# bdina9/qat-vit

Hardware: AMD Instinct MI355X
Metric: images/sec QAT student step (fwd+bwd+allreduce) (higher is better)
Workload: dtype f32 (emulated: int8 MFMA for grid x grid products; forward float operands as fp16 hi+lo pairs; backward gradients as ONE fp16 plane scaled per tensor - 2^-12 per element, <= 4e-4 relative L2 per stage against the fp32 reference, bf16-pair fallback on overflow; fp32 / exact-integer accumulate)

## Files before the change

### include/qatvit.h

```cpp
#ifndef QATVIT_H
#define QATVIT_H

#include <stdint.h>

#ifdef __cplusplus
extern "C" {
#endif
#if defined(__GNUC__) || defined(__clang__)
#pragma GCC visibility push(default)
#endif

#define QATVIT_ABI_VERSION 4

int qatvit_abi_version(void);
const char* qatvit_last_error(void);
const char* qatvit_target_arch(void);

int64_t qatvit_fq_workspace_bytes(int64_t channels);
int qatvit_fq_forward(const float* x, float* y, uint8_t* mask_bits,
                      float* running_min, float* running_max, float* scale, int32_t* zero_point,
                      const int64_t* observer_on, const int64_t* fake_quant_on,
                      float averaging_const, int32_t qmin, int32_t qmax,
                      int64_t channels, int64_t inner, int32_t per_channel, int32_t symmetric,
                      void* workspace, void* stream);

int qatvit_fq_backward(const float* dy, const uint8_t* mask_bits, float* dx, int64_t n, void* stream);

int qatvit_ln_forward(const float* x, const float* gamma, const float* beta, float* y,
                      float* mean, float* rstd, int64_t rows, int64_t dim, float eps, void* stream);
int qatvit_ln_backward(const float* dy, const float* x, const float* gamma, const float* mean,
                       const float* rstd, float* dx, float* dgamma, float* dbeta,
                       int64_t rows, int64_t dim, void* stream);

int qatvit_kd_ce_loss(const float* student, const float* teacher, const int64_t* labels,
                      int64_t batch, int64_t classes, float kd_temp, float kd_alpha,
                      float label_smoothing, float* out3, float* dlogits, void* stream);

int qatvit_kd_ce_loss_table(const float* student, const float* table, int64_t table_rows,
                            const int64_t* index, const int64_t* labels, int64_t batch,
                            int64_t classes, float kd_temp, float kd_alpha, float label_smoothing,
                            float* out3, float* dlogits, void* stream);


int qatvit_gemm_nt(const void* A_hi, const void* A_lo, const void* B, float* C, int32_t M, int32_t N, int32_t K,
                   int32_t lda, int32_t ldb, int32_t ldc, const float* s1, const float* s2, const float* col_scale,
                   const float* bias, uint32_t* stats, void* stream);

int qatvit_gemm_nt_f16(const void* A16_hi, const void* A16_lo, const void* B16, float* C, int32_t M, int32_t N, int32_t K, int32_t lda, int32_t ldb,
                       int32_t ldc, const float* s1, const float* s2, const float* col_scale, const float* bias, uint32_t* stats, void* stream);

int qatvit_gemm_nt_i8_minmax(const void* A8, const void* B8, const int32_t* wsum, const float* a_qp, int32_t center, int32_t M, int32_t N, int32_t K,
                             int32_t lda, int32_t ldb, const float* s1, const float* s2, const float* col_scale, const float* bias, uint32_t* stats,
                             void* stream);

int qatvit_w8_fragment_order(const void* B8, void* B8f, int32_t N, int32_t K, void* stream);

int qatvit_i8_strip(int32_t mode, const void* A8, const void* B8f, const int32_t* wsum, const float* a_qp, int32_t center, int32_t M, int32_t N, int32_t K,
                    int32_t lda, const float* s1, const float* s2, const float* col_scale, const float* bias, uint32_t* stats, const float* out_qp,
                    int32_t qmin, int32_t qmax, void* out8, void* out8_mask, int32_t code_T, uint32_t* lut_out, uint32_t* lutq_out,
                    float* out16_scale, void* stream);

int qatvit_gemm_nt_codes(const void* A8, const uint32_t* lut, const void* B16, float* C, int32_t M, int32_t N, int32_t K, int32_t lda, int32_t ldb,
                         int32_t ldc, const float* s1, const float* s2, const float* col_scale, const float* bias, uint32_t* stats, void* stream);

int qatvit_gemm_nt_i8(const void* A8, const void* B8, const int32_t* wsum, const float* a_qp, int32_t center, float* C, int32_t M,
                      int32_t N, int32_t K, int32_t lda, int32_t ldb, int32_t ldc, const float* s1, const float* s2,
                      const float* col_scale, const float* bias, uint32_t* stats, void* stream);

int64_t qatvit_gemm_tn_scratch_bytes(void);
int qatvit_gemm_tn_codes(const void* P_hi, const void* P_lo, const void* Qc, const uint32_t* lutQ, float* C, int32_t M, int32_t N, int32_t Kw, int32_t ldp,
                         int32_t ldq, int32_t ldc, const float* s1, const float* W, const float* w_scale, const int32_t* w_zp, int32_t w_per_channel,
                         int32_t w_qmin, int32_t w_qmax, float* dbias, const float* row_div, float* scratch, int64_t scratch_bytes, void* stream);
int qatvit_gemm_tn(const void* P_hi, const void* P_lo, const void* Q_hi, const void* Q_lo, float* C, int32_t M, int32_t N,
                   int32_t Kw, int32_t ldp, int32_t ldq, int32_t ldc, const float* s1, const float* W, const float* w_scale,
                   const int32_t* w_zp, int32_t w_per_channel, int32_t w_qmin, int32_t w_qmax, float* dbias,
                   const float* row_div, float* scratch, int64_t scratch_bytes, void* stream);

int qatvit_gemm_nt_dy16(const void* A16, const void* B16, float* C, int32_t M, int32_t N, int32_t K, int32_t lda, int32_t ldb, int32_t ldc, const float* s1,
                        const float* s2, void* stream);
int qatvit_gemm_tn_dy16(const void* P16, const void* Q_hi, const void* Q_lo, const void* Qc, const uint32_t* lutQ16, float* C, int32_t M, int32_t N, int32_t Kw,
                        int32_t ldp, int32_t ldq, int32_t ldc, const float* s1, const float* s2, const float* W, const float* w_scale, const int32_t* w_zp,
                        int32_t w_per_channel, int32_t w_qmin, int32_t w_qmax, float* dbias, const float* row_div, float* scratch, int64_t scratch_bytes,
                        void* stream);
int qatvit_gemm_tn_q8_dy16(const void* P16, const void* Q8, const float* a_qp, int32_t center, float* C, int32_t M, int32_t N, int32_t Kw, int32_t ldp, int32_t ldq,
                           int32_t ldc, const float* s2, const float* W, const float* w_scale, const int32_t* w_zp, int32_t w_per_channel, int32_t w_qmin,
                           int32_t w_qmax, float* dbias, const float* row_div, float* scratch, int64_t scratch_bytes, void* stream);

struct qatvit_tn_item {
    const void* P; const void* Q; const uint32_t* lut; const float* s1; const float* s2; float* C; const float* W; const float* w_scale; const int32_t* w_zp; float* dbias;
    const float* row_div; int32_t N, Kw, ldp, ldq, ldc;
};
int64_t qatvit_gemm_tn_stream_scratch_bytes(void);
int qatvit_gemm_tn_stream_dy16(int32_t mode, const struct qatvit_tn_item* items, int32_t n, int32_t M, int32_t center, int32_t w_per_channel, int32_t w_qmin, int32_t w_qmax,
                               float* scratch, int64_t scratch_bytes, void* stream);

int32_t qatvit_attn_padded_tokens(int32_t T);
int qatvit_attn_forward(const float* qkv, const float* qp, int32_t qmin, int32_t qmax, int32_t B, int32_t T, int32_t H,
                        int32_t D, void* O_hi, void* O_lo, float* lse, void* stream);
int qatvit_attn_forward_f16(const float* qkv, const float* qp, int32_t qmin, int32_t qmax, int32_t B, int32_t T, int32_t H,
                            int32_t D, void* O_hi, void* O_lo, float* lse, void* O16_hi, void* O16_lo, float* o16_scale, void* qkv_codes,
                            void* qkv_mask, void* stream);
int qatvit_attn_backward(const float* qkv, const float* qp, int32_t qmin, int32_t qmax, int32_t B, int32_t T, int32_t H,
                         int32_t D, const void* O_hi, const void* O_lo, const float* lse, float* delta, const float* dO,
                         void* dqkv_hi, void* dqkv_lo, const float* col_scale, const void* qkv_codes, const void* qkv_mask, void* stream);

typedef struct qatvit_cfg {
    int32_t batch, img_size, patch_size, in_chans;
    int32_t embed_dim, depth, num_heads, mlp_hidden, num_classes;
    int32_t act_qmin, act_qmax;
    int32_t w_qmin, w_qmax;
    int32_t w_per_channel;
    float averaging_const;
    float ln_eps;
} qatvit_cfg;

typedef struct qatvit_fq {
    float* min_val;
    float* max_val;
    float* scale;
    int32_t* zero_point;
    const int64_t* observer_on;
    const int64_t* fake_quant_on;
} qatvit_fq;

int32_t qatvit_student_num_params(const qatvit_cfg* cfg);
int32_t qatvit_student_num_act_fq(const qatvit_cfg* cfg);
int32_t qatvit_student_num_weight_fq(const qatvit_cfg* cfg);
int64_t qatvit_student_workspace_bytes(const qatvit_cfg* cfg);
int qatvit_student_init(const qatvit_cfg* cfg, void* workspace, void* stream);
int qatvit_student_forward(const qatvit_cfg* cfg, void* const* params, const qatvit_fq* act_fq, const qatvit_fq* weight_fq,
                           const float* images, float* logits, void* workspace, void* stream);
int qatvit_student_backward(const qatvit_cfg* cfg, void* const* params, const qatvit_fq* act_fq, const qatvit_fq* weight_fq,
                            const float* dlogits, void* const* grads, void* workspace, int32_t stage_from, int32_t stage_to,
                            void* stream);
#define QATVIT_STAGE_INJECT 1
#define QATVIT_FWD_X16 2
#define QATVIT_BWD_DY16 2
#define QATVIT_BWD_CALIBRATE 4
int32_t qatvit_student_dy16_supported(const qatvit_cfg* cfg);
int qatvit_student_dy16_set_mirror(const qatvit_cfg* cfg, void* workspace, void* host_pinned, void* stream);
int qatvit_student_dy16_to_pair(const qatvit_cfg* cfg, void* workspace, void* stream);
int qatvit_student_forward_stages(const qatvit_cfg* cfg, void* const* params, const qatvit_fq* act_fq, const qatvit_fq* weight_fq,
                                  const float* images, float* logits, void* workspace, int32_t stage_from, int32_t stage_to, int32_t flags,
                                  void* stream);
int qatvit_student_forward_part(const qatvit_cfg* cfg, void* const* params, const qatvit_fq* act_fq, const qatvit_fq* weight_fq, void* workspace,
                                int32_t block, int32_t part, int32_t flags, void* stream);
int qatvit_student_backward_stages(const qatvit_cfg* cfg, void* const* params, const qatvit_fq* act_fq, const qatvit_fq* weight_fq,
                                   const float* dlogits, void* const* grads, void* workspace, int32_t stage_from, int32_t stage_to, int32_t flags,
                                   void* stream);
int64_t qatvit_teacher_workspace_bytes(const qatvit_cfg* cfg);
int qatvit_teacher_forward(const qatvit_cfg* cfg, void* const* params, void* const* w_hi, void* const* w_lo,
                           const float* images, float* logits, void* workspace, void* stream);
int qatvit_teacher_forward_f16(const qatvit_cfg* cfg, void* const* params, void* const* w16, int32_t passes,
                               const float* images, float* logits, void* workspace, void* stream);

int64_t qatvit_float_student_workspace_bytes(const qatvit_cfg* cfg);
int qatvit_float_student_init(const qatvit_cfg* cfg, void* workspace, void* stream);
int qatvit_float_student_forward(const qatvit_cfg* cfg, void* const* params, const float* images, float* logits, void* workspace, void* stream);
int qatvit_float_student_backward(const qatvit_cfg* cfg, void* const* params, const float* dlogits, void* const* grads, void* workspace,
                                  void* stream);
int64_t qatvit_float_student_observe_bytes(const qatvit_cfg* cfg);
int qatvit_float_student_observe_init(const qatvit_cfg* cfg, const qatvit_fq* act_fq, const qatvit_fq* weight_fq, void* observe, void* stream);
int qatvit_float_student_forward_observe(const qatvit_cfg* cfg, void* const* params, const float* images, float* logits, void* workspace, void* observe,
                                         void* stream);
int64_t qatvit_float_student_amp_workspace_bytes(const qatvit_cfg* cfg);
int qatvit_float_student_amp_init(const qatvit_cfg* cfg, void* workspace, void* stream);
int qatvit_float_student_amp_forward(const qatvit_cfg* cfg, void* const* params, const float* images, void* logits_f16, void* workspace, void* stream);
int qatvit_float_student_amp_backward(const qatvit_cfg* cfg, void* const* params, const void* dlogits_f16, void* const* grads, void* workspace,
                                      void* stream);
int qatvit_float_student_amp_attn_backward(const float* qkv, const void* O16, const float* lse, const float* dO, int32_t B, int32_t T, int32_t H,
                                           int32_t D, void* dqkv16, void* stream);
int64_t qatvit_float_student_bf16_workspace_bytes(const qatvit_cfg* cfg);
int qatvit_float_student_bf16_init(const qatvit_cfg* cfg, void* workspace, void* stream);
int qatvit_float_student_bf16_forward(const qatvit_cfg* cfg, void* const* params, const float* images, void* logits_bf16, void* workspace, void* stream);
int qatvit_float_student_bf16_backward(const qatvit_cfg* cfg, void* const* params, const void* dlogits_bf16, void* const* grads, void* workspace,
                                       void* stream);
int qatvit_float_student_bf16_attn_backward(const float* qkv, const void* O16, const float* lse, const float* dO, int32_t B, int32_t T, int32_t H,
                                            int32_t D, void* dqkv16, void* stream);

int64_t qatvit_infer_workspace_bytes(const qatvit_cfg* cfg);
int qatvit_infer_prepare(const qatvit_cfg* cfg, const void* const* w8, const float* act_scale, const int32_t* act_zero_point, void* workspace,
                         void* stream);
int qatvit_infer_forward(const qatvit_cfg* cfg, void* const* params, const void* const* w8, const float* const* w_scale, const float* images,
                         float* logits, void* workspace, void* stream);

int qatvit_optim_grad_norm(const void* grad_ptrs, const int64_t* numel, const int32_t* chunk_tensor, const int32_t* chunk_index,
                           int32_t n_chunks, int64_t chunk_elems, float max_norm, float* partials, float* out2, void* stream);
int qatvit_optim_adamw(const void* param_ptrs, const void* grad_ptrs, const void* exp_avg_ptrs, const void* exp_avg_sq_ptrs,
                       const int64_t* numel, const int32_t* chunk_tensor, const int32_t* chunk_index, int32_t n_chunks,
                       int64_t chunk_elems, double lr, double beta1, double beta2, double eps, double weight_decay, int64_t step,
                       const float* clip_out2, void* stream);

int qatvit_image_resize_coeffs(int32_t src, int32_t dst, int32_t* xmin_host, int32_t* ntaps_host, int32_t* coef_host);
int qatvit_image_table(const float* mean_host, const float* std_host, float* table_host);
int qatvit_image_batch(const uint8_t* data, const int64_t* index, int32_t B, int32_t N, int32_t S, int32_t D, const int32_t* coeffs,
                       const float* table, float* out, void* stream);

int qatvit_profile_start(const void* workspace, int32_t kind, int32_t max_launches);
int qatvit_profile_stop(const void* workspace, double* total_ms, int64_t* launches, double* flops);
int64_t qatvit_student_tensor_offset(const qatvit_cfg* cfg, const char* name, int32_t block);

#if defined(__GNUC__) || defined(__clang__)
#pragma GCC visibility pop
#endif
#ifdef __cplusplus
}
#endif
#endif
```

### qat-vit_amd/csrc/capi.hip

```cpp
#include <stdarg.h>
#include <stdlib.h>
#include <string.h>

#include "../../include/qatvit.h"
#include "qv_common.h"
#include "qv_kernels.h"

namespace qv {
static thread_local char g_err[512] = "";
void set_error(const char* fmt, ...) {
    va_list ap;
    va_start(ap, fmt);
    vsnprintf(g_err, sizeof(g_err), fmt, ap);
    va_end(ap);
}

static bool knob(const char* name) {
    const char* v = getenv(name);
    return !v || atoi(v) != 0;
}
const Knobs& knobs() {
    static const Knobs k{knob("QATVIT_I8"), knob("QATVIT_F16"), knob("QATVIT_FC2_CODES"), knob("QATVIT_FC1_BITS"), knob("QATVIT_FC2W_CODES"),
                         knob("QATVIT_WBATCH"), knob("QATVIT_ATTN_CODES"), knob("QATVIT_QKV_2PASS"), knob("QATVIT_LNB_FUSE"), knob("QATVIT_QP_LATE"),
                         knob("QATVIT_TN_STREAM"), knob("QATVIT_TN_Q8"), knob("QATVIT_ATTN_BWD_FUSED"), knob("QATVIT_F16_STRIP"), knob("QATVIT_I8_STRIP")};
    return k;
}
}

using namespace qv;

extern "C" {

int qatvit_abi_version(void) { return QATVIT_ABI_VERSION; }
const char* qatvit_last_error(void) { return qv::g_err; }
const char* qatvit_target_arch(void) { return "gfx950"; }

int64_t qatvit_fq_workspace_bytes(int64_t channels) {
    if (channels < 1) channels = 1;
    return channels * (2 * (int64_t)sizeof(uint32_t) + 4 * (int64_t)sizeof(float));
}

int qatvit_fq_forward(const float* x, float* y, uint8_t* mask_bits, float* running_min, float* running_max, float* scale,
                      int32_t* zero_point, const int64_t* observer_on, const int64_t* fake_quant_on, float averaging_const,
                      int32_t qmin, int32_t qmax, int64_t channels, int64_t inner, int32_t per_channel, int32_t symmetric,
                      void* workspace, void* stream) {
    QV_CHECK_ARG(x && y && running_min && running_max && scale && zero_point && observer_on && fake_quant_on && workspace,
                 "qatvit_fq_forward: null pointer argument");
    QV_CHECK_ARG(channels >= 1 && inner >= 1, "qatvit_fq_forward: empty tensor (channels=%lld inner=%lld)", (long long)channels,
                 (long long)inner);
    QV_CHECK_ARG(qmin < qmax, "qatvit_fq_forward: qmin (%d) must be < qmax (%d)", qmin, qmax);
    QV_CHECK_ARG(per_channel || channels == 1, "qatvit_fq_forward: per-tensor call must pass channels == 1");
    launch_fq_forward(x, y, mask_bits, running_min, running_max, scale, zero_point, observer_on, fake_quant_on, averaging_const, qmin,
                      qmax, channels, inner, per_channel != 0, symmetric != 0, workspace, (hipStream_t)stream);
    QV_CHECK_LAUNCH("qatvit_fq_forward");
    return 0;
}

int qatvit_fq_backward(const float* dy, const uint8_t* mask_bits, float* dx, int64_t n, void* stream) {
    QV_CHECK_ARG(dy && mask_bits && dx, "qatvit_fq_backward: null pointer argument");
    QV_CHECK_ARG(n >= 1, "qatvit_fq_backward: empty tensor");
    launch_fq_backward(dy, mask_bits, dx, n, (hipStream_t)stream);
    QV_CHECK_LAUNCH("qatvit_fq_backward");
    return 0;
}

int qatvit_ln_forward(const float* x, const float* gamma, const float* beta, float* y, float* mean, float* rstd, int64_t rows,
                      int64_t dim, float eps, void* stream) {
    QV_CHECK_ARG(x && gamma && beta && y && mean && rstd, "qatvit_ln_forward: null pointer argument");
    QV_CHECK_ARG(rows >= 1 && dim >= 1, "qatvit_ln_forward: empty tensor");
    launch_ln_forward(x, gamma, beta, y, mean, rstd, rows, dim, eps, (hipStream_t)stream);
    QV_CHECK_LAUNCH("qatvit_ln_forward");
    return 0;
}

int qatvit_ln_backward(const float* dy, const float* x, const float* gamma, const float* mean, const float* rstd, float* dx,
                       float* dgamma, float* dbeta, int64_t rows, int64_t dim, void* stream) {
    QV_CHECK_ARG(dy && x && gamma && mean && rstd && dx && dgamma && dbeta, "qatvit_ln_backward: null pointer argument");
    QV_CHECK_ARG(rows >= 1 && dim >= 1, "qatvit_ln_backward: empty tensor");
    launch_ln_backward(dy, x, gamma, mean, rstd, dx, dgamma, dbeta, rows, dim, (hipStream_t)stream);
    QV_CHECK_LAUNCH("qatvit_ln_backward");
    return 0;
}

int qatvit_kd_ce_loss(const float* student, const float* teacher, const int64_t* labels, int64_t batch, int64_t classes,
                      float kd_temp, float kd_alpha, float label_smoothing, float* out3, float* dlogits, void* stream) {
    QV_CHECK_ARG(student && labels && out3 && dlogits, "qatvit_kd_ce_loss: null pointer argument");
    QV_CHECK_ARG(batch >= 1 && classes >= 2 && classes <= 4096, "qatvit_kd_ce_loss: bad shape B=%lld C=%lld", (long long)batch,
                 (long long)classes);
    QV_CHECK_ARG(kd_temp > 0.f, "qatvit_kd_ce_loss: kd_temp must be > 0");
    launch_kd_ce_loss(student, teacher, labels, batch, classes, kd_temp, kd_alpha, label_smoothing, out3, dlogits, (hipStream_t)stream);
    QV_CHECK_LAUNCH("qatvit_kd_ce_loss");
    return 0;
}

int qatvit_kd_ce_loss_table(const float* student, const float* table, int64_t table_rows, const int64_t* index, const int64_t* labels,
                            int64_t batch, int64_t classes, float kd_temp, float kd_alpha, float label_smoothing, float* out3, float* dlogits,
                            void* stream) {
    QV_CHECK_ARG(student && table && index && labels && out3 && dlogits, "qatvit_kd_ce_loss_table: null pointer argument");
    QV_CHECK_ARG(batch >= 1 && classes >= 2 && classes <= 4096, "qatvit_kd_ce_loss_table: bad shape B=%lld C=%lld", (long long)batch,
                 (long long)classes);
    QV_CHECK_ARG(table_rows >= 1, "qatvit_kd_ce_loss_table: table_rows %lld (at least 1)", (long long)table_rows);
    QV_CHECK_ARG(kd_temp > 0.f, "qatvit_kd_ce_loss_table: kd_temp must be > 0");
    launch_kd_ce_loss_table(student, table, table_rows, index, labels, batch, classes, kd_temp, kd_alpha, label_smoothing, out3, dlogits,
                            (hipStream_t)stream);
    QV_CHECK_LAUNCH("qatvit_kd_ce_loss_table");
    return 0;
}

int qatvit_gemm_nt(const void* A_hi, const void* A_lo, const void* B, float* C, int32_t M, int32_t N, int32_t K, int32_t lda, int32_t ldb,
                   int32_t ldc, const float* s1, const float* s2, const float* col_scale, const float* bias, uint32_t* stats, void* stream) {
    QV_CHECK_ARG(A_hi && B && C, "qatvit_gemm_nt: null pointer argument");
    if (launch_gemm_nt(A_hi, A_lo, B, C, M, N, K, lda, ldb, ldc, s1, s2, col_scale, bias, stats, 1, (hipStream_t)stream)) return 1;
    QV_CHECK_LAUNCH("qatvit_gemm_nt");
    return 0;
}

int qatvit_gemm_nt_f16(const void* A16_hi, const void* A16_lo, const void* B16, float* C, int32_t M, int32_t N, int32_t K, int32_t lda, int32_t ldb,
                       int32_t ldc, const float* s1, const float* s2, const float* col_scale, const float* bias, uint32_t* stats, void* stream) {
    QV_CHECK_ARG(A16_hi && A16_lo && B16 && C, "qatvit_gemm_nt_f16: null pointer argument");
    if (launch_gemm_nt(A16_hi, A16_lo, B16, C, M, N, K, lda, ldb, ldc, s1, s2, col_scale, bias, stats, 1, (hipStream_t)stream, nullptr, nullptr, true)) return 1;
    QV_CHECK_LAUNCH("qatvit_gemm_nt_f16");
    return 0;
}

int qatvit_gemm_nt_i8_minmax(const void* A8, const void* B8, const int32_t* wsum, const float* a_qp, int32_t center, int32_t M, int32_t N, int32_t K,
                             int32_t lda, int32_t ldb, const float* s1, const float* s2, const float* col_scale, const float* bias, uint32_t* stats,
                             void* stream) {
    QV_CHECK_ARG(A8 && B8 && wsum && a_qp && stats, "qatvit_gemm_nt_i8_minmax: null pointer argument");
    NTPost post{};
    post.mode = 3;
    if (launch_gemm_nt_i8(A8, B8, wsum, a_qp, center, nullptr, M, N, K, lda, ldb, N, s1, s2, col_scale, bias, stats, 1, (hipStream_t)stream, &post)) return 1;
    QV_CHECK_LAUNCH("qatvit_gemm_nt_i8_minmax");
    return 0;
}

int qatvit_w8_fragment_order(const void* B8, void* B8f, int32_t N, int32_t K, void* stream) {
    if (launch_w8_fragment_order(B8, B8f, N, K, (hipStream_t)stream)) return 1;
    QV_CHECK_LAUNCH("qatvit_w8_fragment_order");
    return 0;
}

int qatvit_i8_strip(int32_t mode, const void* A8, const void* B8f, const int32_t* wsum, const float* a_qp, int32_t center, int32_t M, int32_t N, int32_t K,
                    int32_t lda, const float* s1, const float* s2, const float* col_scale, const float* bias, uint32_t* stats, const float* out_qp,
                    int32_t qmin, int32_t qmax, void* out8, void* out8_mask, int32_t code_T, uint32_t* lut_out, uint32_t* lutq_out,
                    float* out16_scale, void* stream) {
    QV_CHECK_ARG(A8 && B8f && wsum && a_qp && s1, "qatvit_i8_strip: null pointer argument");
    QV_CHECK_ARG(mode == 3 || mode == 4 || mode == 7, "qatvit_i8_strip: mode %d (3 = statistics, 7 = qkv codes, 4 = fc1 codes)", mode);
    NTPost post{};
    post.mode = mode;
    post.qp = out_qp; post.qmin = qmin; post.qmax = qmax; post.out8 = out8; post.out8_mask = out8_mask; post.code_T = code_T; post.code_hd = 64;
    post.lut_out = lut_out; post.lutq_out = lutq_out; post.out16_scale = out16_scale;
    if (!launch_i8_strip(A8, B8f, wsum, a_qp, center, M, N, K, lda, N, s1, s2, col_scale, bias, stats, 1, (hipStream_t)stream, &post, true)) {
        set_error("qatvit_i8_strip: unsupported arguments (mode %d M=%d N=%d K=%d lda=%d: need K = 384 with N %% 1152 == 0 or N %% 1536 == 0, or K = 768 with "
                  "N = 2304 or 3072; lda %% 16 == 0, M < 2^22, the mode's output pointers, qmax - qmin < 256; mode 7: (N / 3) %% 384 == 0, 0 < code_T < 1024)",
                  mode, M, N, K, lda);
        return 1;
    }
    QV_CHECK_LAUNCH("qatvit_i8_strip");
    return 0;
}

int qatvit_gemm_nt_codes(const void* A8, const uint32_t* lut, const void* B16, float* C, int32_t M, int32_t N, int32_t K, int32_t lda, int32_t ldb,
                         int32_t ldc, const float* s1, const float* s2, const float* col_scale, const float* bias, uint32_t* stats, void* stream) {
    QV_CHECK_ARG(A8 && lut && B16 && C, "qatvit_gemm_nt_codes: null pointer argument");
    if (launch_gemm_nt_codes(A8, lut, B16, C, M, N, K, lda, ldb, ldc, s1, s2, col_scale, bias, stats, 1, (hipStream_t)stream)) return 1;
    QV_CHECK_LAUNCH("qatvit_gemm_nt_codes");
    return 0;
}

int qatvit_gemm_nt_i8(const void* A8, const void* B8, const int32_t* wsum, const float* a_qp, int32_t center, float* C, int32_t M, int32_t N,
                      int32_t K, int32_t lda, int32_t ldb, int32_t ldc, const float* s1, const float* s2, const float* col_scale, const float* bias,
                      uint32_t* stats, void* stream) {
    QV_CHECK_ARG(A8 && B8 && wsum && a_qp && C, "qatvit_gemm_nt_i8: null pointer argument");
    if (launch_gemm_nt_i8(A8, B8, wsum, a_qp, center, C, M, N, K, lda, ldb, ldc, s1, s2, col_scale, bias, stats, 1, (hipStream_t)stream)) return 1;
    QV_CHECK_LAUNCH("qatvit_gemm_nt_i8");
    return 0;
}

int qatvit_gemm_tn(const void* P_hi, const void* P_lo, const void* Q_hi, const void* Q_lo, float* C, int32_t M, int32_t N, int32_t Kw, int32_t ldp,
                   int32_t ldq, int32_t ldc, const float* s1, const float* W, const float* w_scale, const int32_t* w_zp, int32_t w_per_channel,
                   int32_t w_qmin, int32_t w_qmax, float* dbias, const float* row_div, float* scratch, int64_t scratch_bytes, void* stream) {
    QV_CHECK_ARG(P_hi && P_lo && Q_hi && C, "qatvit_gemm_tn: null pointer argument");
    QV_CHECK_ARG(!W || (w_scale && w_zp), "qatvit_gemm_tn: weight mask needs w_scale and w_zp");
    if (launch_gemm_tn(P_hi, P_lo, Q_hi, Q_lo, C, M, N, Kw, ldp, ldq, ldc, s1, W, w_scale, w_zp, w_per_channel, w_qmin, w_qmax, dbias, row_div,
                       (hipStream_t)stream, scratch, scratch_bytes))
        return 1;
    QV_CHECK_LAUNCH("qatvit_gemm_tn");
    return 0;
}

int qatvit_gemm_nt_dy16(const void* A16, const void* B16, float* C, int32_t M, int32_t N, int32_t K, int32_t lda, int32_t ldb, int32_t ldc, const float* s1,
                        const float* s2, void* stream) {
    QV_CHECK_ARG(A16 && B16 && C, "qatvit_gemm_nt_dy16: null pointer argument");
    if (launch_gemm_nt_dy16(A16, B16, C, M, N, K, lda, ldb, ldc, s1, s2, (hipStream_t)stream)) return 1;
    QV_CHECK_LAUNCH("qatvit_gemm_nt_dy16");
    return 0;
}

int qatvit_gemm_tn_dy16(const void* P16, const void* Q_hi, const void* Q_lo, const void* Qc, const uint32_t* lutQ16, float* C, int32_t M, int32_t N, int32_t Kw,
                        int32_t ldp, int32_t ldq, int32_t ldc, const float* s1, const float* s2, const float* W, const float* w_scale, const int32_t* w_zp,
                        int32_t w_per_channel, int32_t w_qmin, int32_t w_qmax, float* dbias, const float* row_div, float* scratch, int64_t scratch_bytes,
                        void* stream) {
    QV_CHECK_ARG(P16 && C && ((Q_hi && !Qc) || (Qc && lutQ16 && !Q_hi && !Q_lo)), "qatvit_gemm_tn_dy16: Q is either planes (Q_hi, optional Q_lo) or codes + table");
    QV_CHECK_ARG(!W || (w_scale && w_zp), "qatvit_gemm_tn_dy16: weight mask needs w_scale and w_zp");
    const int rc = Qc ? launch_gemm_tn_codes_dy16(P16, Qc, lutQ16, C, M, N, Kw, ldp, ldq, ldc, s1, s2, W, w_scale, w_zp, w_per_channel, w_qmin, w_qmax, dbias, row_div,
                                                  (hipStream_t)stream, scratch, scratch_bytes)
                      : launch_gemm_tn_dy16(P16, Q_hi, Q_lo, C, M, N, Kw, ldp, ldq, ldc, s1, s2, W, w_scale, w_zp, w_per_channel, w_qmin, w_qmax, dbias, row_div,
                                            (hipStream_t)stream, scratch, scratch_bytes);
    if (rc) return 1;
    QV_CHECK_LAUNCH("qatvit_gemm_tn_dy16");
    return 0;
}

int qatvit_gemm_tn_q8_dy16(const void* P16, const void* Q8, const float* a_qp, int32_t center, float* C, int32_t M, int32_t N, int32_t Kw, int32_t ldp, int32_t ldq,
                           int32_t ldc, const float* s2, const float* W, const float* w_scale, const int32_t* w_zp, int32_t w_per_channel, int32_t w_qmin,
                           int32_t w_qmax, float* dbias, const float* row_div, float* scratch, int64_t scratch_bytes, void* stream) {
    QV_CHECK_ARG(P16 && Q8 && a_qp && C, "qatvit_gemm_tn_q8_dy16: null pointer argument");
    QV_CHECK_ARG(!W || (w_scale && w_zp), "qatvit_gemm_tn_q8_dy16: weight mask needs w_scale and w_zp");
    if (launch_gemm_tn_q8_dy16(P16, Q8, a_qp, center, C, M, N, Kw, ldp, ldq, ldc, s2, W, w_scale, w_zp, w_per_channel, w_qmin, w_qmax, dbias, row_div,
                               (hipStream_t)stream, scratch, scratch_bytes))
        return 1;
    QV_CHECK_LAUNCH("qatvit_gemm_tn_q8_dy16");
    return 0;
}

int64_t qatvit_gemm_tn_stream_scratch_bytes(void) { return tn_stream_scratch_bytes(); }
int qatvit_gemm_tn_stream_dy16(int32_t mode, const struct qatvit_tn_item* items, int32_t n, int32_t M, int32_t center, int32_t w_per_channel, int32_t w_qmin, int32_t w_qmax,
                               float* scratch, int64_t scratch_bytes, void* stream) {
    QV_CHECK_ARG(items && scratch && n >= 1, "qatvit_gemm_tn_stream_dy16: null / empty argument");
    static_assert(sizeof(qatvit_tn_item) == sizeof(TNStreamGemm), "qatvit_tn_item mirrors TNStreamGemm");
    if (launch_tn_stream(mode, reinterpret_cast<const TNStreamGemm*>(items), n, M, center, w_per_channel, w_qmin, w_qmax, scratch, scratch_bytes, (hipStream_t)stream)) return 1;
    QV_CHECK_LAUNCH("qatvit_gemm_tn_stream_dy16");
    return 0;
}

int qatvit_gemm_tn_codes(const void* P_hi, const void* P_lo, const void* Qc, const uint32_t* lutQ, float* C, int32_t M, int32_t N, int32_t Kw, int32_t ldp,
                         int32_t ldq, int32_t ldc, const float* s1, const float* W, const float* w_scale, const int32_t* w_zp, int32_t w_per_channel,
                         int32_t w_qmin, int32_t w_qmax, float* dbias, const float* row_div, float* scratch, int64_t scratch_bytes, void* stream) {
    QV_CHECK_ARG(P_hi && P_lo && Qc && lutQ && C, "qatvit_gemm_tn_codes: null pointer argument");
    QV_CHECK_ARG(!W || (w_scale && w_zp), "qatvit_gemm_tn_codes: weight mask needs w_scale and w_zp");
    if (launch_gemm_tn_codes(P_hi, P_lo, Qc, lutQ, C, M, N, Kw, ldp, ldq, ldc, s1, W, w_scale, w_zp, w_per_channel, w_qmin, w_qmax, dbias, row_div,
                             (hipStream_t)stream, scratch, scratch_bytes))
        return 1;
    QV_CHECK_LAUNCH("qatvit_gemm_tn_codes");
    return 0;
}

int64_t qatvit_gemm_tn_scratch_bytes(void) { return kTnScratchBytes; }

int32_t qatvit_attn_padded_tokens(int32_t T) { return attn_padded_tokens(T); }

int qatvit_attn_forward(const float* qkv, const float* qp, int32_t qmin, int32_t qmax, int32_t B, int32_t T, int32_t H, int32_t D, void* O_hi,
                        void* O_lo, float* lse, void* stream) {
    QV_CHECK_ARG(qkv && qp && O_hi && O_lo && lse, "qatvit_attn_forward: null pointer argument");
    QV_CHECK_ARG(B >= 1 && T >= 1 && H >= 1, "qatvit_attn_forward: empty shape");
    if (launch_attn_fwd(qkv, qp, qmin, qmax, B, T, H, D, O_hi, O_lo, lse, (hipStream_t)stream)) return 1;
    QV_CHECK_LAUNCH("qatvit_attn_forward");
    return 0;
}

int qatvit_attn_forward_f16(const float* qkv, const float* qp, int32_t qmin, int32_t qmax, int32_t B, int32_t T, int32_t H, int32_t D, void* O_hi,
                            void* O_lo, float* lse, void* O16_hi, void* O16_lo, float* o16_scale, void* qkv_codes, void* qkv_mask, void* stream) {
    QV_CHECK_ARG((qkv || qkv_codes) && qp && O_hi && O_lo && lse && O16_hi && O16_lo && o16_scale, "qatvit_attn_forward_f16: null pointer argument");
    QV_CHECK_ARG(B >= 1 && T >= 1 && H >= 1, "qatvit_attn_forward_f16: empty shape");
    if (launch_attn_fwd(qkv, qp, qmin, qmax, B, T, H, D, O_hi, O_lo, lse, (hipStream_t)stream, O16_hi, O16_lo, o16_scale, qkv_codes, qkv_mask)) return 1;
    QV_CHECK_LAUNCH("qatvit_attn_forward_f16");
    return 0;
}

int qatvit_attn_backward(const float* qkv, const float* qp, int32_t qmin, int32_t qmax, int32_t B, int32_t T, int32_t H, int32_t D,
                         const void* O_hi, const void* O_lo, const float* lse, float* delta, const float* dO, void* dqkv_hi, void* dqkv_lo,
                         const float* col_scale, const void* qkv_codes, const void* qkv_mask, void* stream) {
    QV_CHECK_ARG((qkv || qkv_codes) && qp && O_hi && O_lo && lse && delta && dO && dqkv_hi && dqkv_lo, "qatvit_attn_backward: null pointer argument");
    if (launch_attn_bwd(qkv, qp, qmin, qmax, B, T, H, D, O_hi, O_lo, lse, delta, dO, dqkv_hi, dqkv_lo, col_scale, (hipStream_t)stream, qkv_codes, qkv_mask))
        return 1;
    QV_CHECK_LAUNCH("qatvit_attn_backward");
    return 0;
}

static int image_shape_ok(const char* who, int32_t S, int32_t D) {
    QV_CHECK_ARG(S >= 8 && S <= D, "%s: source size %d is outside 8 .. output size %d (downscaling is not supported)", who, S, D);
    QV_CHECK_ARG(D % 4 == 0 && D <= kImgMaxD, "%s: output size %d must be a multiple of 4, at most %d", who, D, kImgMaxD);
    return 0;
}

int qatvit_image_resize_coeffs(int32_t src, int32_t dst, int32_t* xmin_host, int32_t* ntaps_host, int32_t* coef_host) {
    QV_CHECK_ARG(xmin_host && ntaps_host && coef_host, "qatvit_image_resize_coeffs: null pointer argument");
    if (image_shape_ok("qatvit_image_resize_coeffs", src, dst)) return 1;
    return image_resize_coeffs(src, dst, xmin_host, ntaps_host, coef_host);
}

int qatvit_image_table(const float* mean_host, const float* std_host, float* table_host) {
    QV_CHECK_ARG(mean_host && std_host && table_host, "qatvit_image_table: null pointer argument");
    for (int c = 0; c < 3; ++c) QV_CHECK_ARG(std_host[c] != 0.0f, "qatvit_image_table: std[%d] is zero", c);
    image_table(mean_host, std_host, table_host);
    return 0;
}

int qatvit_image_batch(const uint8_t* data, const int64_t* index, int32_t B, int32_t N, int32_t S, int32_t D, const int32_t* coeffs,
                       const float* table, float* out, void* stream) {
    QV_CHECK_ARG(data && coeffs && table && out, "qatvit_image_batch: null pointer argument");
    if (image_shape_ok("qatvit_image_batch", S, D)) return 1;
    QV_CHECK_ARG(B >= 1 && B <= 65535 && N >= 1, "qatvit_image_batch: batch %d must be 1 .. 65535 and the data set (%d images) not empty", B, N);
    QV_CHECK_ARG(index || B <= N, "qatvit_image_batch: batch %d of a data set of %d images needs an index", B, N);
    QV_CHECK_ARG(((uintptr_t)out & 15) == 0 && ((uintptr_t)coeffs & 3) == 0 && ((uintptr_t)table & 3) == 0, "qatvit_image_batch: misaligned pointer");
    launch_image_batch(data, index, B, N, S, D, coeffs, table, out, (hipStream_t)stream);
    QV_CHECK_LAUNCH("qatvit_image_batch");
    return 0;
}

}
```

### qat-vit_amd/csrc/engine.hip

```cpp
#include <string.h>

#include <memory>
#include <mutex>
#include <unordered_map>
#include <vector>

#include "../../include/qatvit.h"
#include <stdlib.h>

#include "qv_common.h"
#include "qv_kernels.h"

namespace qv {

enum { P_PE_W = 0, P_PE_B, P_CLS, P_POS, P_BLOCK0 };
enum { B_N1W = 0, B_N1B, B_QKVW, B_QKVB, B_PROJW, B_PROJB, B_N2W, B_N2B, B_FC1W, B_FC1B, B_FC2W, B_FC2B, B_COUNT };
enum { A_IN = 0, A_PE, A_BLOCK0 };
enum { AB_N1 = 0, AB_QKV, AB_PROJ, AB_N2, AB_FC1, AB_FC2, AB_COUNT };
enum { WB_QKV = 0, WB_PROJ, WB_FC1, WB_FC2, WB_COUNT };

struct Dims {
    int B, T, np, D, H, Hd, C, depth, Kpe, img, patch, chans;
    int64_t M;
    int n_act, n_w;
};

static Dims dims_of(const qatvit_cfg& c) {
    Dims d;
    d.B = c.batch; d.img = c.img_size; d.patch = c.patch_size; d.chans = c.in_chans;
    d.np = (c.img_size / c.patch_size) * (c.img_size / c.patch_size);
    d.T = d.np + 1; d.D = c.embed_dim; d.H = c.num_heads; d.Hd = c.mlp_hidden; d.C = c.num_classes; d.depth = c.depth;
    d.Kpe = c.in_chans * c.patch_size * c.patch_size;
    d.M = (int64_t)d.B * d.T;
    d.n_act = 2 + AB_COUNT * d.depth + 2;
    d.n_w = 1 + WB_COUNT * d.depth + 1;
    return d;
}

static void wshape(const Dims& d, int wi, int* N, int* K) {
    if (wi == 0) { *N = d.D; *K = d.Kpe; return; }
    if (wi == d.n_w - 1) { *N = d.C; *K = d.D; return; }
    switch ((wi - 1) % WB_COUNT) {
        case WB_QKV: *N = 3 * d.D; *K = d.D; break;
        case WB_PROJ: *N = d.D; *K = d.D; break;
        case WB_FC1: *N = d.Hd; *K = d.D; break;
        default: *N = d.D; *K = d.Hd; break;
    }
}
static int wparam(const Dims& d, int wi) {
    if (wi == 0) return P_PE_W;
    if (wi == d.n_w - 1) return P_BLOCK0 + B_COUNT * d.depth + 2;
    const int blk = (wi - 1) / WB_COUNT, k = (wi - 1) % WB_COUNT;
    static const int map[WB_COUNT] = {B_QKVW, B_PROJW, B_FC1W, B_FC2W};
    return P_BLOCK0 + B_COUNT * blk + map[k];
}

struct Forms {
    bool i8;
    bool w_batched;
    bool late;
    bool f16_proj, f16_fc2;
    bool fc2_codes;
    bool fc1_code_bits;
    bool fc2w_codes;
    bool attn_codes;
    bool qkv_2pass;
    bool attn_bwd_fused;
    bool lnb;
    bool x_plane_from_q8;
    bool tn_stream;
    bool dy16;
};
static Forms forms_of(const qatvit_cfg& c, const Dims& d) {
    const Knobs& k = knobs();
    const bool byte_codes = c.act_qmax - c.act_qmin <= 255;
    Forms f{};
    f.i8 = k.i8;
    f.w_batched = k.wbatch && d.n_w <= kMaxW;
    f.late = k.qp_late && d.n_act <= kMaxActFq;
    f.f16_proj = k.f16 && f.w_batched && d.D % 384 == 0;
    f.f16_fc2 = f.f16_proj && d.Hd % 32 == 0;
    f.fc2_codes = f.f16_fc2 && k.fc2_codes && d.Hd % 64 == 0 && byte_codes;
    f.fc1_code_bits = f.fc2_codes && k.fc1_bits && f.i8 && d.Hd % 384 == 0;
    f.fc2w_codes = f.fc1_code_bits && k.fc2w_codes;
    f.attn_codes = k.attn_codes && byte_codes;
    f.qkv_2pass = k.qkv_2pass && f.attn_codes && f.i8 && (3 * d.D) % 384 == 0 && d.D % 64 == 0 && (d.D / d.H) % 32 == 0;
    f.attn_bwd_fused = attn_bwd_is_fused(d.T, d.H, d.D, f.attn_codes);
    f.lnb = k.lnb_fuse && d.D == 384;
    f.x_plane_from_q8 = f.i8 && k.tn_q8 && d.D % 384 == 0;
    f.tn_stream = k.tn_stream && d.D % 384 == 0 && d.Hd % 384 == 0;
    f.dy16 = f.i8 && f.w_batched && d.D % 384 == 0 && d.Hd % 384 == 0 && f.qkv_2pass && f.attn_bwd_fused && f.f16_proj && f.fc2w_codes;
    return f;
}

struct Plan {
    Forms form;
    int64_t stats, qp_act, qp_w, imgq, Y0, meanF, rstdF, hq, logits_pre;
    int64_t x_in, x_mid, mean1, rstd1, mean2, rstd2, h1q, qkv, O_hi, O_lo, lse, Yproj, h2q, Y1, G_hi, G_lo, Y2, mproj, m2, qkv8, qkvm, G8, glut, Y1m, glutq;
    int64_t blk_stride;
    int64_t wq, wqT;
    int64_t w_off[64 * 4 + 8], wT_off[64 * 4 + 8], w_stats[64 * 4 + 8], w_qp[64 * 4 + 8];
    int64_t w8_off[64 * 4 + 8], wsum_off[64 * 4 + 8], wsum_base, wsum_bytes, imgq8, h1q8, h2q8;
    int64_t w8f_off[64 * 4 + 8];
    int64_t w16_off[64 * 4 + 8], O16_hi, O16_lo, G16_hi, G16_lo, scal16;
    int64_t dxA, dxB, dYs_hi, dYs_lo, dG, dY1_hi, dY1_lo, dH, dO, dqkv_hi, dqkv_lo, delta, dh, dY0_hi, dY0_lo, tn_scratch;
    int64_t dyp, dyp_stride, dyp_p, dyp_h, dyp_q, tn_stream;
    int64_t qp_staged;
    int64_t dy16;
    int64_t total, stats_words;
    int TP;
};
enum { DS_FC2 = 0, DS_FC1, DS_PROJ, DS_QKV, DS_COUNT };

static int64_t al(int64_t x) { return (x + 255) & ~(int64_t)255; }

static int make_plan(const qatvit_cfg& c, Plan* p) {
    const Dims d = dims_of(c);
    if (d.depth > 64) { set_error("engine: depth %d > 64", d.depth); return 1; }
    p->form = forms_of(c, d);
    int64_t o = 0;
    auto take = [&](int64_t bytes) { int64_t r = o; o += al(bytes); return r; };
    const int64_t M = d.M, D = d.D, Hd = d.Hd;
    p->TP = attn_padded_tokens(d.T);
    int64_t wstat_words = 0, wqp_floats = 0;
    for (int wi = 0; wi < d.n_w; ++wi) {
        int N, K; wshape(d, wi, &N, &K);
        const int ch = c.w_per_channel ? N : 1;
        p->w_stats[wi] = (int64_t)d.n_act * kStatSlots * kStatStride + wstat_words;
        wstat_words += c.w_per_channel ? 2 * ch : kStatSlots * kStatStride;
        p->w_qp[wi] = wqp_floats; wqp_floats += 4 * ch;
    }
    p->stats_words = (int64_t)d.n_act * kStatSlots * kStatStride + wstat_words;
    p->stats = take(p->stats_words * 4);
    p->qp_staged = take((int64_t)d.n_act * kQpStagedWords * 4);
    p->dy16 = take(dy16_state_bytes(DS_COUNT * d.depth));
    p->qp_act = take((int64_t)d.n_act * 4 * 4);
    p->qp_w = take(wqp_floats * 4);
    p->imgq = take((int64_t)d.B * d.np * d.Kpe * 2);
    p->Y0 = take((int64_t)d.B * d.np * D * 4);
    p->meanF = take(M * 4); p->rstdF = take(M * 4);
    p->hq = take((int64_t)d.B * D * 4);
    p->logits_pre = take((int64_t)d.B * d.C * 4);
    const int64_t b0 = o;
    p->x_in = take(M * D * 4);
    p->x_mid = take(M * D * 4);
    p->mean1 = take(M * 4); p->rstd1 = take(M * 4); p->mean2 = take(M * 4); p->rstd2 = take(M * 4);
    p->h1q = take(M * D * 2);
    p->qkv = take(M * 3 * D * 4);
    p->O_hi = take(M * D * 2); p->O_lo = take(M * D * 2);
    p->lse = take((int64_t)d.B * d.H * p->TP * 4);
    p->Yproj = take(M * D * 4);
    p->h2q = take(M * D * 2);
    p->Y1 = take(M * Hd * 2);
    p->G_hi = take(M * Hd * 2); p->G_lo = take(M * Hd * 2);
    p->Y2 = take(M * D * 4);
    p->h1q8 = take(M * D); p->h2q8 = take(M * D);
    p->mproj = take(ln_maskbits_bytes(M, (int)D)); p->m2 = take(ln_maskbits_bytes(M, (int)D));
    p->qkv8 = take(M * 3 * D); p->qkvm = take(M * 3 * D / 8);
    p->O16_hi = take(M * D * 2); p->O16_lo = take(M * D * 2); p->scal16 = take(2 * sizeof(float));
    p->G8 = take(M * Hd); p->glut = take(256 * 4); p->Y1m = take(M * Hd / 8); p->glutq = take(256 * 4);
    p->blk_stride = o - b0;
    o = b0 + p->blk_stride * d.depth;
    const int64_t xfinal = take(M * D * 4);
    (void)xfinal;
    for (int wi = 0; wi < d.n_w; ++wi) {
        int N, K; wshape(d, wi, &N, &K);
        p->w_off[wi] = take((int64_t)N * K * 2);
        p->wT_off[wi] = take((int64_t)N * K * 2);
        (void)take((int64_t)N * K * 2);
        (void)take((int64_t)N * K * 2);
        p->w8_off[wi] = take((int64_t)N * K);
        const int kind = (wi == 0 || wi == d.n_w - 1) ? -1 : (wi - 1) % WB_COUNT;
        p->w16_off[wi] = (kind == WB_PROJ || kind == WB_FC2) ? take((int64_t)N * K * 2) : -1;
        p->w8f_off[wi] = ((kind == WB_QKV || kind == WB_FC1) && (K == 384 || K == 768) && N % 48 == 0) ? take((int64_t)N * K) : -1;
    }
    p->G16_hi = take(M * Hd * 2); p->G16_lo = take(M * Hd * 2);
    p->imgq8 = take((int64_t)d.B * d.np * d.Kpe);
    p->wsum_base = o;
    for (int wi = 0; wi < d.n_w; ++wi) {
        int N, K; wshape(d, wi, &N, &K);
        p->wsum_off[wi] = take((int64_t)N * 4);
    }
    p->wsum_bytes = o - p->wsum_base;
    p->dxA = take(M * D * 4); p->dxB = take(M * D * 4);
    p->dYs_hi = take(M * D * 2); p->dYs_lo = take(M * D * 2);
    p->dG = take(M * Hd * 4);
    p->dY1_hi = take(M * Hd * 2); p->dY1_lo = take(M * Hd * 2);
    p->dH = take(M * D * 4); p->dO = take(M * D * 4);
    p->dqkv_hi = take(M * 3 * D * 2); p->dqkv_lo = take(M * 3 * D * 2);
    p->delta = take((int64_t)d.B * d.H * p->TP * 4);
    p->dh = take((int64_t)d.B * D * 4);
    p->dY0_hi = take((int64_t)d.B * d.np * D * 2); p->dY0_lo = take((int64_t)d.B * d.np * D * 2);
    p->tn_scratch = take(kTnScratchBytes);
    p->dyp = p->tn_stream = -1; p->dyp_stride = 0;
    if (p->form.tn_stream) {
        p->dyp_p = al(M * D * 2); p->dyp_h = p->dyp_p + al(M * D * 2); p->dyp_q = p->dyp_h + al(M * Hd * 2);
        p->dyp_stride = p->dyp_q + al(M * 3 * D * 2);
        p->dyp = take(p->dyp_stride * d.depth);
        p->tn_stream = take(tn_stream_scratch_bytes());
    }
    p->total = o;
    return 0;
}

static int check_cfg(const qatvit_cfg& c) {
    if (c.batch < 1 || c.depth < 1 || c.embed_dim % 128 != 0 || c.mlp_hidden % 128 != 0 || c.embed_dim % c.num_heads != 0 ||
        c.img_size % c.patch_size != 0 || (c.in_chans * c.patch_size * c.patch_size) % 128 != 0 || c.embed_dim > 768) {
        set_error("engine: unsupported config (batch %d depth %d dim %d hidden %d heads %d img %d patch %d)", c.batch, c.depth, c.embed_dim,
                  c.mlp_hidden, c.num_heads, c.img_size, c.patch_size);
        return 1;
    }
    return 0;
}

struct Prof {
    int kind = 0;
    std::vector<hipEvent_t> ev;
    size_t used = 0;
    double flops = 0.0;
    bool closed = false;
    std::mutex mu;
    ~Prof() { for (hipEvent_t e : ev) if (e) (void)hipEventDestroy(e); }
};
static std::mutex g_prof_mu;
static std::unordered_map<const void*, std::shared_ptr<Prof>> g_profs;
static std::shared_ptr<Prof> prof_of(const void* workspace) {
    std::lock_guard<std::mutex> lk(g_prof_mu);
    auto it = g_profs.find(workspace);
    return it == g_profs.end() ? nullptr : it->second;
}
struct ProfScope {
    Prof* pr;
    hipStream_t st;
    size_t slot = 0;
    bool on = false;
    ProfScope(const std::shared_ptr<Prof>& p, int kind, double flops, hipStream_t s) : pr(p.get()), st(s) {
        if (!pr || pr->kind != kind) return;
        std::lock_guard<std::mutex> lk(pr->mu);
        if (pr->closed || pr->used + 2 > pr->ev.size()) return;
        slot = pr->used;
        pr->used += 2;
        pr->flops += flops;
        on = true;
        (void)hipEventRecord(pr->ev[slot], st);
    }
    ~ProfScope() {
        if (on) (void)hipEventRecord(pr->ev[slot + 1], st);
    }
};

struct Ctx {
    const qatvit_cfg& c;
    Dims d;
    Plan p;
    char* ws;
    void* const* params;
    const qatvit_fq* act;
    const qatvit_fq* wfq;
    hipStream_t st;
    std::shared_ptr<Prof> prof;
    int flags = 0;
    uint32_t* dy_slot(int i, int k) const { return at<uint32_t>(p.dy16) + kDyHdrWords + (int64_t)(DS_COUNT * i + k) * kDySlotWords; }
    const float* dy_mul(int i, int k) const { return reinterpret_cast<const float*>(dy_slot(i, k) + 1); }
    const float* dy_inv(int i, int k) const { return reinterpret_cast<const float*>(dy_slot(i, k) + 2); }
    void* wT16(int wi) const { int N, K; wshape(d, wi, &N, &K); return ws + p.wT_off[wi] + wT16_gap_bytes(N, K); }
    void* wT16f(int wi) const { int N, K; wshape(d, wi, &N, &K); return ws + p.wT_off[wi] + 2 * wT16_gap_bytes(N, K); }
    bool wT16f_ok(int wi) const {
        int N, K; wshape(d, wi, &N, &K);
        return wi >= 1 && wi < d.n_w - 1 && (wi - 1) % WB_COUNT == WB_FC2 && N == 384 && K == 1536;
    }
    template <typename T> T* at(int64_t off) const { return reinterpret_cast<T*>(ws + off); }
    template <typename T> T* blk(int64_t off, int i) const { return reinterpret_cast<T*>(ws + off + p.blk_stride * i); }
    const float* prm(int i) const { return reinterpret_cast<const float*>(params[i]); }
    const float* bprm(int blk_i, int k) const { return prm(P_BLOCK0 + B_COUNT * blk_i + k); }
    uint32_t* act_stats(int ai) const { return at<uint32_t>(p.stats) + (int64_t)ai * kStatSlots * kStatStride; }
    float* act_qp(int ai) const { return at<float>(p.qp_act) + 4 * ai; }
    float* w_qp(int wi) const { return at<float>(p.qp_w) + p.w_qp[wi]; }
    int aidx(int blk_i, int k) const { return A_BLOCK0 + AB_COUNT * blk_i + k; }
    int a_norm() const { return A_BLOCK0 + AB_COUNT * d.depth; }
    int a_head() const { return a_norm() + 1; }
    int widx(int blk_i, int k) const { return 1 + WB_COUNT * blk_i + k; }
    bool late_kind(int ai) const {
        if (!p.form.late || ai < A_BLOCK0 || ai >= A_BLOCK0 + AB_COUNT * d.depth) return false;
        const int k = (ai - A_BLOCK0) % AB_COUNT;
        return k == AB_N1 || k == AB_N2 || k == AB_PROJ || k == AB_FC2;
    }
    QpLate late(int ai) const {
        const qatvit_fq& f = act[ai];
        return QpLate{act_stats(ai), f.min_val, f.max_val, f.scale, f.zero_point, f.observer_on, f.fake_quant_on, c.averaging_const, c.act_qmin, c.act_qmax,
                      act_qp(ai), at<float>(p.qp_staged) + (int64_t)ai * kQpStagedWords};
    }
    int commit_late() const {
        if (!p.form.late) return 0;
        QpCommitTab t{};
        t.n = d.n_act; t.staged = at<float>(p.qp_staged); t.stats = at<uint32_t>(p.stats);
        for (int ai = 0; ai < d.n_act; ++ai) { t.rmin[ai] = act[ai].min_val; t.rmax[ai] = act[ai].max_val; t.scale[ai] = act[ai].scale; t.zp[ai] = act[ai].zero_point; }
        return launch_qp_commit(t, st);
    }
    void qparams_after(int ai, bool produced_stats, bool deferred = false) const {
        if (produced_stats && !deferred && !late_kind(ai)) qparams_act(ai);
    }
    int resid_lnstats(int mode, const float* x_prev, const float* Y, int ai_Y, const float* cls, const float* pos, float* x_new, float* mean,
                      float* rstd, const float* gamma, const float* beta, int ai_stats, void* maskbits = nullptr) const {
        const bool lt = ai_Y >= 0 && late_kind(ai_Y);
        const QpLate L = lt ? late(ai_Y) : QpLate{};
        if (launch_resid_fq_lnstats(mode, x_prev, Y, act_qp(ai_Y >= 0 ? ai_Y : 0), c.act_qmin, c.act_qmax, cls, pos, x_new, mean, rstd, gamma, beta, c.ln_eps,
                                    act_stats(ai_stats), kStatSlots, d.M, d.D, d.T, st, maskbits, lt ? &L : nullptr))
            return 1;
        qparams_after(ai_stats, true);
        return 0;
    }
    int ln_apply(const float* xrow, const float* mean, const float* rstd, const float* gamma, const float* beta, int ai, void* out16, void* out8) const {
        const bool lt = late_kind(ai);
        const QpLate L = lt ? late(ai) : QpLate{};
        const bool x16 = (flags & QATVIT_FWD_X16) != 0;
        return launch_ln_apply_quant(xrow, mean, rstd, gamma, beta, act_qp(ai), c.act_qmin, c.act_qmax, x16 && p.form.x_plane_from_q8 ? nullptr : out16, d.M, d.D,
                                     st, p.form.i8 ? out8 : nullptr, center(), x16, lt ? &L : nullptr);
    }
    void qparams_act(int ai) const {
        const qatvit_fq& f = act[ai];
        launch_qparams(act_stats(ai), f.min_val, f.max_val, f.scale, f.zero_point, f.observer_on, f.fake_quant_on, c.averaging_const,
                       c.act_qmin, c.act_qmax, 1, 0, act_qp(ai), 1, kStatSlots, st);
    }
    int linear_fwd(const void* A_hi, const void* A_lo, int M, int wi, const float* s_act, const float* bias, float* C, int ai_out,
                   const NTPost* post = nullptr, bool with_stats = true) const {
        int N, K; wshape(d, wi, &N, &K);
        const qatvit_fq& f = wfq[wi];
        {
            ProfScope ps(prof, A_lo ? 1 : 2, (post && post->mode == 3) ? 0.0 : 2.0 * M * N * K, st);
            if (launch_gemm_nt(A_hi, A_lo, at<void>(p.w_off[wi]), C, M, N, K, K, K, N, s_act, c.w_per_channel ? nullptr : f.scale,
                               c.w_per_channel ? f.scale : nullptr, bias, with_stats ? act_stats(ai_out) : nullptr, kStatSlots, st, nullptr, post, false))
                return 1;
        }
        qparams_after(ai_out, with_stats);
        return 0;
    }
    int linear_fwd_f16(const void* A16_hi, const void* A16_lo, const float* pair_scale, int M, int wi, const float* bias, float* C, int ai_out) const {
        int N, K; wshape(d, wi, &N, &K);
        const qatvit_fq& f = wfq[wi];
        {
            ProfScope ps(prof, 1, 2.0 * M * N * K, st);
            if (launch_gemm_nt(A16_hi, A16_lo, at<void>(p.w16_off[wi]), C, M, N, K, K, K, N, pair_scale, c.w_per_channel ? nullptr : f.scale,
                               c.w_per_channel ? f.scale : nullptr, bias, act_stats(ai_out), kStatSlots, st, nullptr, nullptr, true))
                return 1;
        }
        qparams_after(ai_out, true);
        return 0;
    }
    int linear_fwd_codes(const void* A8, const uint32_t* lut, const float* pair_scale, int M, int wi, const float* bias, float* C, int ai_out) const {
        int N, K; wshape(d, wi, &N, &K);
        const qatvit_fq& f = wfq[wi];
        {
            ProfScope ps(prof, 1, 2.0 * M * N * K, st);
            if (launch_gemm_nt_codes(A8, lut, at<void>(p.w16_off[wi]), C, M, N, K, K, K, N, pair_scale, c.w_per_channel ? nullptr : f.scale,
                                     c.w_per_channel ? f.scale : nullptr, bias, act_stats(ai_out), kStatSlots, st))
                return 1;
        }
        qparams_after(ai_out, true);
        return 0;
    }
    int center() const { return (c.act_qmin + c.act_qmax + 1) / 2; }
    int linear_fwd_grid(const void* A16, const void* A8, int M, int wi, const float* a_qp, const float* bias, float* C, int ai_out,
                        const NTPost* post = nullptr, bool with_stats = true, bool late_strip = false) const {
        int N, K; wshape(d, wi, &N, &K);
        if (!p.form.i8 || N % 384 != 0 || K % 64 != 0) return linear_fwd(A16, nullptr, M, wi, a_qp, bias, C, ai_out, post, with_stats);
        const qatvit_fq& f = wfq[wi];
        {
            ProfScope ps(prof, !post ? 2 : post->mode == 3 ? 7 : post->mode == 4 ? 8 : post->mode == 7 ? 9 : 2, (post && post->mode == 3) ? 0.0 : 2.0 * M * N * K, st);
            const bool code_pass = late_strip && post && post->mode != 3;
            const QpLate L = code_pass ? late(ai_out) : QpLate{};
            if (launch_gemm_nt_i8(A8, at<void>(p.w8_off[wi]), at<int32_t>(p.wsum_off[wi]), a_qp, center(), C, M, N, K, K, K, N, a_qp,
                                  c.w_per_channel ? nullptr : f.scale, c.w_per_channel ? f.scale : nullptr, bias,
                                  with_stats ? act_stats(ai_out) : nullptr, kStatSlots, st, post, w8f(wi), code_pass ? &L : nullptr))
                return 1;
        }
        qparams_after(ai_out, with_stats, late_strip);
        return 0;
    }
    void* w8f(int wi) const { return p.form.i8 && p.form.w_batched && p.w8f_off[wi] >= 0 ? at<void>(p.w8f_off[wi]) : nullptr; }
    bool late_in_strip(int M, int wi, const NTPost* post2) const {
        int N, K; wshape(d, wi, &N, &K);
        return p.form.late && i8_strip_covers(w8f(wi), M, N, K, K, N, post2);
    }
    const float* dy_colscale(int wi) const { return c.w_per_channel ? wfq[wi].scale : nullptr; }
    int linear_dgrad(const void* dY_hi, const void* dY_lo, int M, int wi, float* dX, const NTPost* post = nullptr) const {
        int N, K; wshape(d, wi, &N, &K);
        const qatvit_fq& f = wfq[wi];
        ProfScope ps(prof, !post ? 1 : post->mode == 8 ? 4 : 5, 2.0 * M * N * K, st);
        return launch_gemm_nt(dY_hi, dY_lo, at<void>(p.wT_off[wi]), dX, M, K, N, N, N, K, c.w_per_channel ? nullptr : f.scale, nullptr, nullptr,
                              nullptr, nullptr, 1, st, nullptr, post);
    }
    int linear_wgrad_codes(const void* dY_hi, const void* dY_lo, int M, int wi, const void* X8, const uint32_t* lutq, float* dW, float* db) const {
        int N, K; wshape(d, wi, &N, &K);
        const qatvit_fq& f = wfq[wi];
        ProfScope ps(prof, 6, 2.0 * M * N * K, st);
        return launch_gemm_tn_codes(dY_hi, dY_lo, X8, lutq, dW, M, N, K, N, K, K, nullptr, prm(wparam(d, wi)), f.scale, f.zero_point, c.w_per_channel, c.w_qmin,
                                    c.w_qmax, db, c.w_per_channel ? f.scale : nullptr, st, at<float>(p.tn_scratch), kTnScratchBytes);
    }
    int linear_wgrad(const void* dY_hi, const void* dY_lo, int M, int wi, const void* X_hi, const void* X_lo, const float* s_x, float* dW, float* db,
                     bool dy_scaled = true) const {
        int N, K; wshape(d, wi, &N, &K);
        const qatvit_fq& f = wfq[wi];
        ProfScope ps(prof, X_lo ? 6 : 3, 2.0 * M * N * K, st);
        return launch_gemm_tn(dY_hi, dY_lo, X_hi, X_lo, dW, M, N, K, N, K, K, s_x, prm(wparam(d, wi)), f.scale, f.zero_point, c.w_per_channel,
                              c.w_qmin, c.w_qmax, db, (c.w_per_channel && dy_scaled) ? f.scale : nullptr, st, at<float>(p.tn_scratch), kTnScratchBytes);
    }
};

static int fwd_block(const Ctx& x, int i, int parts, bool qkv_injected = false) {
    const Dims& d = x.d;
    const Plan& p = x.p;
    const Forms& F = p.form;
    const qatvit_cfg& c = x.c;
    hipStream_t st = x.st;
    const int qa = c.act_qmin, qb = c.act_qmax;
    const int M = (int)d.M;
    {
        float* xin = x.blk<float>(p.x_in, i);
        float* xmid = x.blk<float>(p.x_mid, i);
        if (parts & 1) {
        x.ln_apply(xin, x.blk<float>(p.mean1, i), x.blk<float>(p.rstd1, i), x.bprm(i, B_N1W), x.bprm(i, B_N1B), x.aidx(i, AB_N1), x.blk<void>(p.h1q, i),
                   x.blk<void>(p.h1q8, i));
        if (F.qkv_2pass) {
            NTPost p2{};
            p2.mode = 7; p2.qp = x.act_qp(x.aidx(i, AB_QKV)); p2.qmin = qa; p2.qmax = qb;
            p2.out8 = x.blk<void>(p.qkv8, i); p2.out8_mask = x.blk<void>(p.qkvm, i); p2.code_T = (int)d.T; p2.code_hd = (int)(d.D / d.H);
            const bool lt = x.late_in_strip(M, x.widx(i, WB_QKV), &p2);
            const NTPost p1{nullptr, nullptr, 0, 0, nullptr, nullptr, nullptr, 3, nullptr};
            if (x.linear_fwd_grid(x.blk<void>(p.h1q, i), x.blk<void>(p.h1q8, i), M, x.widx(i, WB_QKV), x.act_qp(x.aidx(i, AB_N1)), x.bprm(i, B_QKVB), nullptr,
                                  x.aidx(i, AB_QKV), &p1, true, lt))
                return 1;
            if (x.linear_fwd_grid(x.blk<void>(p.h1q, i), x.blk<void>(p.h1q8, i), M, x.widx(i, WB_QKV), x.act_qp(x.aidx(i, AB_N1)), x.bprm(i, B_QKVB), nullptr,
                                  x.aidx(i, AB_QKV), &p2, false, lt))
                return 1;
        } else if (x.linear_fwd_grid(x.blk<void>(p.h1q, i), x.blk<void>(p.h1q8, i), M, x.widx(i, WB_QKV), x.act_qp(x.aidx(i, AB_N1)), x.bprm(i, B_QKVB),
                                     x.blk<float>(p.qkv, i), x.aidx(i, AB_QKV)))
            return 1;
        }
        float* const scal16 = x.blk<float>(p.scal16, i);
        if (parts & 2) {
        const bool from_codes = F.qkv_2pass && !qkv_injected;
        if (launch_attn_fwd(from_codes ? nullptr : x.blk<float>(p.qkv, i), x.act_qp(x.aidx(i, AB_QKV)), qa, qb, d.B, d.T, d.H, d.D, x.blk<void>(p.O_hi, i),
                            x.blk<void>(p.O_lo, i), x.blk<float>(p.lse, i), st, F.f16_proj ? x.blk<void>(p.O16_hi, i) : nullptr,
                            F.f16_proj ? x.blk<void>(p.O16_lo, i) : nullptr, F.f16_proj ? scal16 : nullptr, F.attn_codes ? x.blk<void>(p.qkv8, i) : nullptr,
                            F.attn_codes ? x.blk<void>(p.qkvm, i) : nullptr))
            return 1;
        if (F.f16_proj) {
            if (x.linear_fwd_f16(x.blk<void>(p.O16_hi, i), x.blk<void>(p.O16_lo, i), scal16, M, x.widx(i, WB_PROJ), x.bprm(i, B_PROJB), x.blk<float>(p.Yproj, i),
                                 x.aidx(i, AB_PROJ)))
                return 1;
        } else if (x.linear_fwd(x.blk<void>(p.O_hi, i), x.blk<void>(p.O_lo, i), M, x.widx(i, WB_PROJ), nullptr, x.bprm(i, B_PROJB),
                                x.blk<float>(p.Yproj, i), x.aidx(i, AB_PROJ)))
            return 1;
        if (x.resid_lnstats(1, xin, x.blk<float>(p.Yproj, i), x.aidx(i, AB_PROJ), nullptr, nullptr, xmid, x.blk<float>(p.mean2, i),
                            x.blk<float>(p.rstd2, i), x.bprm(i, B_N2W), x.bprm(i, B_N2B), x.aidx(i, AB_N2), x.blk<void>(p.mproj, i)))
            return 1;
        }
        if (parts & 4) {
        x.ln_apply(xmid, x.blk<float>(p.mean2, i), x.blk<float>(p.rstd2, i), x.bprm(i, B_N2W), x.bprm(i, B_N2B), x.aidx(i, AB_N2), x.blk<void>(p.h2q, i),
                   x.blk<void>(p.h2q8, i));
        {
            NTPost p2{nullptr, x.act_qp(x.aidx(i, AB_FC1)), qa, qb, nullptr, x.blk<void>(p.G_hi, i), x.blk<void>(p.G_lo, i), 4,
                      x.blk<void>(p.Y1, i)};
            if (F.fc2_codes) { p2.out8 = x.blk<void>(p.G8, i); p2.lut_out = x.blk<uint32_t>(p.glut, i); p2.out16_scale = scal16 + 1; }
            if (F.fc1_code_bits) { p2.code = nullptr; p2.out8_mask = x.blk<void>(p.Y1m, i); }
            if (F.fc2w_codes) { p2.out_hi = p2.out_lo = nullptr; p2.lutq_out = x.blk<uint32_t>(p.glutq, i); }
            else if (F.f16_fc2) { p2.out16_hi = x.at<void>(p.G16_hi); p2.out16_lo = x.at<void>(p.G16_lo); p2.out16_scale = scal16 + 1; }
            const bool lt = x.late_in_strip(M, x.widx(i, WB_FC1), &p2);
            const NTPost p1{nullptr, nullptr, 0, 0, nullptr, nullptr, nullptr, 3, nullptr};
            if (x.linear_fwd_grid(x.blk<void>(p.h2q, i), x.blk<void>(p.h2q8, i), M, x.widx(i, WB_FC1), x.act_qp(x.aidx(i, AB_N2)), x.bprm(i, B_FC1B), nullptr,
                             x.aidx(i, AB_FC1), &p1, true, lt))
                return 1;
            if (x.linear_fwd_grid(x.blk<void>(p.h2q, i), x.blk<void>(p.h2q8, i), M, x.widx(i, WB_FC1), x.act_qp(x.aidx(i, AB_N2)), x.bprm(i, B_FC1B), nullptr,
                             x.aidx(i, AB_FC1), &p2, false, lt))
                return 1;
        }
        }
        if (parts & 8) {
        if (F.fc2_codes) {
            if (x.linear_fwd_codes(x.blk<void>(p.G8, i), x.blk<uint32_t>(p.glut, i), scal16 + 1, M, x.widx(i, WB_FC2), x.bprm(i, B_FC2B), x.blk<float>(p.Y2, i),
                                   x.aidx(i, AB_FC2)))
                return 1;
        } else if (F.f16_fc2) {
            if (x.linear_fwd_f16(x.at<void>(p.G16_hi), x.at<void>(p.G16_lo), scal16 + 1, M, x.widx(i, WB_FC2), x.bprm(i, B_FC2B), x.blk<float>(p.Y2, i),
                                 x.aidx(i, AB_FC2)))
                return 1;
        } else if (x.linear_fwd(x.blk<void>(p.G_hi, i), x.blk<void>(p.G_lo, i), M, x.widx(i, WB_FC2), nullptr, x.bprm(i, B_FC2B), x.blk<float>(p.Y2, i),
                                x.aidx(i, AB_FC2)))
            return 1;
        const bool last = (i + 1 == d.depth);
        const float* g = last ? x.prm(P_BLOCK0 + B_COUNT * d.depth) : x.bprm(i + 1, B_N1W);
        const float* bt = last ? x.prm(P_BLOCK0 + B_COUNT * d.depth + 1) : x.bprm(i + 1, B_N1B);
        float* mean = last ? x.at<float>(p.meanF) : x.blk<float>(p.mean1, i + 1);
        float* rstd = last ? x.at<float>(p.rstdF) : x.blk<float>(p.rstd1, i + 1);
        if (x.resid_lnstats(1, xmid, x.blk<float>(p.Y2, i), x.aidx(i, AB_FC2), nullptr, nullptr, x.blk<float>(p.x_in, i + 1), mean, rstd, g, bt,
                            last ? x.a_norm() : x.aidx(i + 1, AB_N1), x.blk<void>(p.m2, i)))
            return 1;
        }
        return 0;
    }
}

static int inject_ln_stats_of(const Ctx& x, const float* tensor, const float* g, const float* bt, float* mean, float* rstd, int ai) {
    launch_ws_init(x.act_stats(ai), kStatSlots * kStatStride / 2, x.st);
    return x.resid_lnstats(2, tensor, nullptr, -1, nullptr, nullptr, nullptr, mean, rstd, g, bt, ai);
}
static int inject_ln_stats(const Ctx& x, int i) {
    const Dims& d = x.d;
    const Plan& p = x.p;
    const bool last = (i == d.depth);
    const float* g = last ? x.prm(P_BLOCK0 + B_COUNT * d.depth) : x.bprm(i, B_N1W);
    const float* bt = last ? x.prm(P_BLOCK0 + B_COUNT * d.depth + 1) : x.bprm(i, B_N1B);
    float* mean = last ? x.at<float>(p.meanF) : x.blk<float>(p.mean1, i);
    float* rstd = last ? x.at<float>(p.rstdF) : x.blk<float>(p.rstd1, i);
    return inject_ln_stats_of(x, x.blk<float>(p.x_in, i), g, bt, mean, rstd, last ? x.a_norm() : x.aidx(i, AB_N1));
}
static int fwd_part(const Ctx& x, int block, int part, bool inject) {
    const Dims& d = x.d;
    const Plan& p = x.p;
    if (inject) {
        if (part == 0) {
            if (inject_ln_stats(x, block)) return 1;
        } else if (part == 1) {
            const int ai = x.aidx(block, AB_QKV);
            launch_ws_init(x.act_stats(ai), kStatSlots * kStatStride / 2, x.st);
            launch_minmax(x.blk<float>(p.qkv, block), 1, d.M * 3 * d.D, 0, x.act_stats(ai), kStatSlots, x.st);
            x.qparams_act(ai);
        } else if (part == 2) {
            if (inject_ln_stats_of(x, x.blk<float>(p.x_mid, block), x.bprm(block, B_N2W), x.bprm(block, B_N2B), x.blk<float>(p.mean2, block),
                                   x.blk<float>(p.rstd2, block), x.aidx(block, AB_N2)))
                return 1;
        }
    }
    return fwd_block(x, block, 1 << part, inject && part == 1);
}

static int fwd(const Ctx& x, const float* images, float* logits, int s_from, int s_to, bool inject) {
    const Dims& d = x.d;
    const Plan& p = x.p;
    const Forms& F = p.form;
    const qatvit_cfg& c = x.c;
    hipStream_t st = x.st;
    const int qa = c.act_qmin, qb = c.act_qmax;
    if (inject && s_from >= 1 && inject_ln_stats(x, s_from - 1)) return 1;
    if (s_from == 0) {
    if (F.late) launch_ws_init(x.at<uint32_t>(p.stats), (int64_t)d.n_act * kStatSlots * kStatStride / 2, st);
    if (F.w_batched) {
        WObsTab to{};
        WQpTab tq{};
        WQuantTab tw{};
        to.n = tq.n = tw.n = d.n_w;
        tw.wT16 = 1;
        for (int wi = 0; wi < d.n_w && wi < 64; ++wi)
            if (x.wT16f_ok(wi)) tw.wT16f_mask |= 1ull << wi;
        to.per_channel = tq.per_channel = tw.per_channel = c.w_per_channel;
        to.nslots = tq.nslots = kStatSlots;
        tq.qmin = tw.qmin = c.w_qmin; tq.qmax = tw.qmax = c.w_qmax; tq.c = c.averaging_const;
        for (int wi = 0; wi < d.n_w; ++wi) {
            int N, K; wshape(d, wi, &N, &K);
            const qatvit_fq& f = x.wfq[wi];
            uint32_t* ws = x.at<uint32_t>(p.stats) + p.w_stats[wi];
            to.W[wi] = tw.W[wi] = x.prm(wparam(d, wi));
            to.ws[wi] = tq.ws[wi] = ws;
            to.N[wi] = tq.N[wi] = tw.N[wi] = N;
            to.K[wi] = tw.K[wi] = K;
            tq.rmin[wi] = f.min_val; tq.rmax[wi] = f.max_val; tq.scale[wi] = f.scale; tq.zp[wi] = f.zero_point;
            tq.obs_on[wi] = f.observer_on; tq.fq_on[wi] = f.fake_quant_on;
            tq.qp[wi] = x.w_qp(wi); tw.qp[wi] = x.w_qp(wi);
            tw.wq[wi] = x.at<void>(p.w_off[wi]); tw.wqT[wi] = x.at<void>(p.wT_off[wi]);
            tw.w8[wi] = F.i8 ? x.at<void>(p.w8_off[wi]) : nullptr;
            const bool w16 = p.w16_off[wi] >= 0 && ((wi - 1) % WB_COUNT == WB_PROJ ? F.f16_proj : F.f16_fc2);
            tw.w16[wi] = w16 ? x.at<void>(p.w16_off[wi]) : nullptr;
            tw.w8f[wi] = x.w8f(wi);
            tw.wsum[wi] = F.i8 ? x.at<int32_t>(p.wsum_off[wi]) : nullptr;
        }
        if (F.i8) launch_zero_i32(x.at<int32_t>(p.wsum_base), p.wsum_bytes / 4, st);
        launch_w_observe_all(to, st);
        launch_w_qparams_all(tq, st);
        launch_w_quant_all(tw, st);
    } else {
        for (int wi = 0; wi < d.n_w; ++wi) {
            int N, K; wshape(d, wi, &N, &K);
            const qatvit_fq& f = x.wfq[wi];
            const float* W = x.prm(wparam(d, wi));
            uint32_t* ws = x.at<uint32_t>(p.stats) + p.w_stats[wi];
            launch_minmax(W, c.w_per_channel ? N : 1, c.w_per_channel ? K : (int64_t)N * K, c.w_per_channel, ws, kStatSlots, st);
            launch_qparams(ws, f.min_val, f.max_val, f.scale, f.zero_point, f.observer_on, f.fake_quant_on, c.averaging_const, c.w_qmin, c.w_qmax,
                           c.w_per_channel ? N : 1, 1, x.w_qp(wi), 1, c.w_per_channel ? 1 : kStatSlots, st);
            launch_wquant(W, x.w_qp(wi), c.w_per_channel, c.w_qmin, c.w_qmax, x.at<void>(p.w_off[wi]), x.at<void>(p.wT_off[wi]), N, K, st);
        }
    }
    launch_minmax(images, 1, (int64_t)d.B * d.chans * d.img * d.img, 0, x.act_stats(A_IN), kStatSlots, st);
    x.qparams_act(A_IN);
    if (launch_img_patches(images, x.at<void>(p.imgq), x.act_qp(A_IN), qa, qb, d.B, d.chans, d.img, d.img, d.patch, st,
                           F.i8 ? x.at<void>(p.imgq8) : nullptr, x.center()))
        return 1;
    if (x.linear_fwd_grid(x.at<void>(p.imgq), x.at<void>(p.imgq8), d.B * d.np, 0, x.act_qp(A_IN), x.prm(P_PE_B), x.at<float>(p.Y0), A_PE)) return 1;
    if (x.resid_lnstats(0, nullptr, x.at<float>(p.Y0), A_PE, x.prm(P_CLS), x.prm(P_POS), x.blk<float>(p.x_in, 0), x.blk<float>(p.mean1, 0),
                        x.blk<float>(p.rstd1, 0), x.bprm(0, B_N1W), x.bprm(0, B_N1B), x.aidx(0, AB_N1)))
        return 1;
    }
    for (int i = (s_from < 1 ? 0 : s_from - 1); i < d.depth && i + 1 <= s_to; ++i)
        if (fwd_block(x, i, 15)) return 1;
    if (s_to < d.depth + 1) return 0;
    const int base = P_BLOCK0 + B_COUNT * d.depth;
    const int wh = d.n_w - 1;
    launch_head_fwd(x.blk<float>(p.x_in, d.depth), x.at<float>(p.meanF), x.at<float>(p.rstdF), x.prm(base), x.prm(base + 1), x.act_qp(x.a_norm()),
                    qa, qb, x.at<void>(p.w_off[wh]), x.wfq[wh].scale, c.w_per_channel, x.prm(base + 3), x.at<float>(p.hq), x.at<float>(p.logits_pre),
                    x.act_stats(x.a_head()), kStatSlots, d.B, d.D, d.T, d.C, st);
    x.qparams_act(x.a_head());
    launch_logits_fq(x.at<float>(p.logits_pre), x.act_qp(x.a_head()), qa, qb, logits, d.B * d.C, st);
    return 0;
}

struct Bwd {
    const Ctx& x;
    void* const* grads;
    bool dy, cal;
    bool stream;
    float* dxA;
    float* dxB;
    std::vector<TNStreamGemm> sg[3];
    double sflops[3] = {0.0, 0.0, 0.0};

// ... 191 lines not shown
    }
    if (i > 0) calib(dYh, d.M * d.D, i - 1, DS_FC2);
    return 0;
}

int Bwd::embed() {
    const Dims& d = x.d;
    const Plan& p = x.p;
    launch_embed_bwd(dxA, x.at<float>(p.Y0), x.act_qp(A_PE), x.c.act_qmin, x.c.act_qmax, G(P_POS), G(P_CLS), x.at<void>(p.dY0_hi), x.at<void>(p.dY0_lo), d.B,
                     d.T, d.D, x.st);
    return x.linear_wgrad(x.at<void>(p.dY0_hi), x.at<void>(p.dY0_lo), d.B * d.np, 0, x.at<void>(p.imgq), nullptr, x.act_qp(A_IN), G(P_PE_W), G(P_PE_B), false);
}

int Bwd::flush() {
    const qatvit_cfg& c = x.c;
    for (int m = 0; m < 3; ++m) {
        for (size_t o = 0; o < sg[m].size(); o += 24) {
            const int n = (int)std::min<size_t>(24, sg[m].size() - o);
            ProfScope ps(x.prof, m == 0 ? 3 : 6, sflops[m] * n / (double)sg[m].size(), x.st);
            if (launch_tn_stream(m, sg[m].data() + o, n, (int)x.d.M, x.center(), c.w_per_channel, c.w_qmin, c.w_qmax, x.at<float>(x.p.tn_stream),
                                 tn_stream_scratch_bytes(), x.st))
                return 1;
        }
    }
    return 0;
}

static int bwd(const Ctx& x, const float* dlogits, void* const* grads, int stage_from, int stage_to, bool inject) {
    const Dims& d = x.d;
    const Forms& F = x.p.form;
    const bool dy = (x.flags & QATVIT_BWD_DY16) != 0, cal = (x.flags & QATVIT_BWD_CALIBRATE) != 0;
    if (dy && cal) { set_error("student backward: QATVIT_BWD_DY16 and QATVIT_BWD_CALIBRATE exclude each other"); return 1; }
    if ((dy || cal) && !F.dy16) { set_error("student backward: the one-plane form does not cover this configuration (qatvit_student_dy16_supported)"); return 1; }
    Bwd b{x, grads, dy, cal, dy && F.tn_stream && F.x_plane_from_q8, x.at<float>(x.p.dxA), x.at<float>(x.p.dxB)};
    uint32_t* const dystate = x.at<uint32_t>(x.p.dy16);
    const int nslots = DS_COUNT * d.depth;
    if ((dy || cal) && (stage_from == 0 || inject)) launch_dy16_begin(dystate, nslots, stage_from == 0 ? dlogits : nullptr, d.B * d.C, x.st);
    for (int s = stage_from; s <= stage_to; ++s) {
        const bool injected = inject && s == stage_from;
        if (s == 0 ? b.head(dlogits) : s > d.depth ? b.embed() : dy ? b.block_one_plane(d.depth - s, injected) : b.block_pair(d.depth - s, injected)) return 1;
    }
    if (dy || cal) launch_dy16_end(dystate, nslots, dy ? 1 : 0, x.st);
    return b.flush();
}

}

using namespace qv;

extern "C" {

int64_t qatvit_student_workspace_bytes(const qatvit_cfg* cfg) {
    if (!cfg || check_cfg(*cfg)) return -1;
    Plan p;
    if (make_plan(*cfg, &p)) return -1;
    return p.total;
}

int32_t qatvit_student_num_params(const qatvit_cfg* cfg) { return cfg ? P_BLOCK0 + B_COUNT * cfg->depth + 4 : -1; }
int32_t qatvit_student_num_act_fq(const qatvit_cfg* cfg) { return cfg ? 2 + AB_COUNT * cfg->depth + 2 : -1; }
int32_t qatvit_student_num_weight_fq(const qatvit_cfg* cfg) { return cfg ? 1 + WB_COUNT * cfg->depth + 1 : -1; }

int qatvit_student_init(const qatvit_cfg* cfg, void* workspace, void* stream) {
    QV_CHECK_ARG(cfg && workspace, "qatvit_student_init: null argument");
    if (check_cfg(*cfg)) return 1;
    Plan p;
    if (make_plan(*cfg, &p)) return 1;
    {
        std::lock_guard<std::mutex> lk(g_prof_mu);
        auto it = g_profs.find(workspace);
        if (it != g_profs.end()) { std::lock_guard<std::mutex> l2(it->second->mu); it->second->closed = true; }
        g_profs.erase(workspace);
    }
    launch_ws_init(reinterpret_cast<uint32_t*>(reinterpret_cast<char*>(workspace) + p.stats), p.stats_words / 2, (hipStream_t)stream);
    launch_zero_i32(reinterpret_cast<int32_t*>(reinterpret_cast<char*>(workspace) + p.dy16), dy16_state_bytes(DS_COUNT * cfg->depth) / 4, (hipStream_t)stream);
    launch_zero_i32(reinterpret_cast<int32_t*>(reinterpret_cast<char*>(workspace) + p.qp_staged), (int64_t)dims_of(*cfg).n_act * kQpStagedWords, (hipStream_t)stream);
    QV_CHECK_LAUNCH("qatvit_student_init");
    return 0;
}

static int run_forward(const qatvit_cfg* cfg, void* const* params, const qatvit_fq* act_fq, const qatvit_fq* weight_fq, const float* images,
                       float* logits, void* workspace, int32_t stage_from, int32_t stage_to, int32_t flags, void* stream, const char* who) {
    QV_CHECK_ARG(cfg && params && act_fq && weight_fq && workspace, "%s: null argument", who);
    if (check_cfg(*cfg)) return 1;
    QV_CHECK_ARG(stage_from >= 0 && stage_to <= cfg->depth + 1 && stage_from <= stage_to, "%s: bad stage range [%d,%d]", who, stage_from, stage_to);
    QV_CHECK_ARG(stage_from > 0 || images, "%s: stage 0 needs the images", who);
    QV_CHECK_ARG(stage_to <= cfg->depth || logits, "%s: the last stage needs the logits buffer", who);
    QV_CHECK_ARG((flags & ~(QATVIT_STAGE_INJECT | QATVIT_FWD_X16)) == 0 && !((flags & QATVIT_STAGE_INJECT) && stage_from == 0), "%s: bad flags %d", who, flags);
    Ctx x{*cfg, dims_of(*cfg), Plan(), reinterpret_cast<char*>(workspace), params, act_fq, weight_fq, (hipStream_t)stream, prof_of(workspace)};
    if (make_plan(*cfg, &x.p)) return 1;
    x.flags = flags & QATVIT_FWD_X16;
    QV_CHECK_ARG(!x.flags || x.p.form.dy16, "%s: QATVIT_FWD_X16 needs a configuration the one-plane backward covers (qatvit_student_dy16_supported)", who);
    if (fwd(x, images, logits, stage_from, stage_to, (flags & QATVIT_STAGE_INJECT) != 0)) return 1;
    if (x.commit_late()) return 1;
    QV_CHECK_LAUNCH(who);
    return 0;
}

int qatvit_student_forward(const qatvit_cfg* cfg, void* const* params, const qatvit_fq* act_fq, const qatvit_fq* weight_fq, const float* images,
                           float* logits, void* workspace, void* stream) {
    QV_CHECK_ARG(cfg && images && logits, "qatvit_student_forward: null argument");
    return run_forward(cfg, params, act_fq, weight_fq, images, logits, workspace, 0, cfg->depth + 1, 0, stream, "qatvit_student_forward");
}

int qatvit_student_forward_stages(const qatvit_cfg* cfg, void* const* params, const qatvit_fq* act_fq, const qatvit_fq* weight_fq,
                                  const float* images, float* logits, void* workspace, int32_t stage_from, int32_t stage_to, int32_t flags,
                                  void* stream) {
    return run_forward(cfg, params, act_fq, weight_fq, images, logits, workspace, stage_from, stage_to, flags, stream, "qatvit_student_forward_stages");
}

int qatvit_student_forward_part(const qatvit_cfg* cfg, void* const* params, const qatvit_fq* act_fq, const qatvit_fq* weight_fq, void* workspace,
                                int32_t block, int32_t part, int32_t flags, void* stream) {
    QV_CHECK_ARG(cfg && params && act_fq && weight_fq && workspace, "qatvit_student_forward_part: null argument");
    if (check_cfg(*cfg)) return 1;
    QV_CHECK_ARG(block >= 0 && block < cfg->depth && part >= 0 && part <= 3 && (flags & ~(QATVIT_STAGE_INJECT | QATVIT_FWD_X16)) == 0,
                 "qatvit_student_forward_part: bad block %d / part %d / flags %d", block, part, flags);
    Ctx x{*cfg, dims_of(*cfg), Plan(), reinterpret_cast<char*>(workspace), params, act_fq, weight_fq, (hipStream_t)stream, prof_of(workspace)};
    if (make_plan(*cfg, &x.p)) return 1;
    x.flags = flags & QATVIT_FWD_X16;
    QV_CHECK_ARG(!x.flags || x.p.form.dy16, "qatvit_student_forward_part: QATVIT_FWD_X16 needs a configuration the one-plane backward covers");
    if (fwd_part(x, block, part, (flags & QATVIT_STAGE_INJECT) != 0)) return 1;
    if (x.commit_late()) return 1;
    QV_CHECK_LAUNCH("qatvit_student_forward_part");
    return 0;
}

static int run_backward(const qatvit_cfg* cfg, void* const* params, const qatvit_fq* act_fq, const qatvit_fq* weight_fq, const float* dlogits,
                        void* const* grads, void* workspace, int32_t stage_from, int32_t stage_to, int32_t flags, void* stream, const char* who) {
    QV_CHECK_ARG(cfg && params && act_fq && weight_fq && grads && workspace, "%s: null argument", who);
    if (check_cfg(*cfg)) return 1;
    QV_CHECK_ARG(stage_from >= 0 && stage_to <= cfg->depth + 1 && stage_from <= stage_to, "%s: bad stage range [%d,%d]", who, stage_from, stage_to);
    QV_CHECK_ARG(stage_from > 0 || dlogits, "%s: stage 0 needs dlogits", who);
    QV_CHECK_ARG((flags & ~(QATVIT_STAGE_INJECT | QATVIT_BWD_DY16 | QATVIT_BWD_CALIBRATE)) == 0 && !((flags & QATVIT_STAGE_INJECT) && stage_from == 0),
                 "%s: bad flags %d", who, flags);
    Ctx x{*cfg, dims_of(*cfg), Plan(), reinterpret_cast<char*>(workspace), params, act_fq, weight_fq, (hipStream_t)stream, prof_of(workspace)};
    if (make_plan(*cfg, &x.p)) return 1;
    x.flags = flags & (QATVIT_BWD_DY16 | QATVIT_BWD_CALIBRATE);
    if (bwd(x, dlogits, grads, stage_from, stage_to, (flags & QATVIT_STAGE_INJECT) != 0)) return 1;
    QV_CHECK_LAUNCH(who);
    return 0;
}

int qatvit_student_backward(const qatvit_cfg* cfg, void* const* params, const qatvit_fq* act_fq, const qatvit_fq* weight_fq, const float* dlogits,
                            void* const* grads, void* workspace, int32_t stage_from, int32_t stage_to, void* stream) {
    return run_backward(cfg, params, act_fq, weight_fq, dlogits, grads, workspace, stage_from, stage_to, 0, stream, "qatvit_student_backward");
}

int qatvit_student_backward_stages(const qatvit_cfg* cfg, void* const* params, const qatvit_fq* act_fq, const qatvit_fq* weight_fq,
                                   const float* dlogits, void* const* grads, void* workspace, int32_t stage_from, int32_t stage_to, int32_t flags,
                                   void* stream) {
    return run_backward(cfg, params, act_fq, weight_fq, dlogits, grads, workspace, stage_from, stage_to, flags, stream, "qatvit_student_backward_stages");
}

int32_t qatvit_student_dy16_supported(const qatvit_cfg* cfg) {
    if (!cfg || check_cfg(*cfg)) return 0;
    Plan p;
    if (make_plan(*cfg, &p)) return 0;
    return p.form.dy16 ? 1 : 0;
}

int qatvit_student_dy16_set_mirror(const qatvit_cfg* cfg, void* workspace, void* host_pinned, void* stream) {
    QV_CHECK_ARG(cfg && workspace, "qatvit_student_dy16_set_mirror: null argument");
    if (check_cfg(*cfg)) return 1;
    Plan p;
    if (make_plan(*cfg, &p)) return 1;
    if (launch_dy16_set_mirror(reinterpret_cast<uint32_t*>(reinterpret_cast<char*>(workspace) + p.dy16), host_pinned, (hipStream_t)stream)) return 1;
    QV_CHECK_LAUNCH("qatvit_student_dy16_set_mirror");
    return 0;
}

int qatvit_student_dy16_to_pair(const qatvit_cfg* cfg, void* workspace, void* stream) {
    QV_CHECK_ARG(cfg && workspace, "qatvit_student_dy16_to_pair: null argument");
    if (check_cfg(*cfg)) return 1;
    Ctx x{*cfg, dims_of(*cfg), Plan(), reinterpret_cast<char*>(workspace), nullptr, nullptr, nullptr, (hipStream_t)stream, nullptr};
    if (make_plan(*cfg, &x.p)) return 1;
    for (int i = 0; i < x.d.depth; ++i) {
        if (x.p.form.x_plane_from_q8) {
            if (launch_q8_to_bf16int(x.blk<void>(x.p.h1q8, i), x.act_qp(x.aidx(i, AB_N1)), x.center(), x.blk<void>(x.p.h1q, i), x.d.M * x.d.D, x.st)) return 1;
            if (launch_q8_to_bf16int(x.blk<void>(x.p.h2q8, i), x.act_qp(x.aidx(i, AB_N2)), x.center(), x.blk<void>(x.p.h2q, i), x.d.M * x.d.D, x.st)) return 1;
            continue;
        }
        if (launch_f16int_to_bf16int(x.blk<void>(x.p.h1q, i), x.d.M * x.d.D, x.st)) return 1;
        if (launch_f16int_to_bf16int(x.blk<void>(x.p.h2q, i), x.d.M * x.d.D, x.st)) return 1;
    }
    QV_CHECK_LAUNCH("qatvit_student_dy16_to_pair");
    return 0;
}

int qatvit_profile_start(const void* workspace, int32_t kind, int32_t max_launches) {
    QV_CHECK_ARG(workspace && kind >= 1 && kind <= 9 && max_launches > 0, "qatvit_profile_start: bad arguments");
    auto pr = std::make_shared<Prof>();
    pr->ev.assign((size_t)max_launches * 2, nullptr);
    for (auto& e : pr->ev)
        if (hipEventCreate(&e) != hipSuccess) {
            set_error("qatvit_profile_start: hipEventCreate failed");
            return 2;
        }
    pr->kind = kind;
    std::lock_guard<std::mutex> lk(g_prof_mu);
    auto it = g_profs.find(workspace);
    if (it != g_profs.end()) {
        std::lock_guard<std::mutex> l2(it->second->mu);
        it->second->closed = true;
    }
    g_profs[workspace] = pr;
    return 0;
}

int qatvit_profile_stop(const void* workspace, double* total_ms, int64_t* launches, double* flops) {
    QV_CHECK_ARG(workspace && total_ms && launches && flops, "qatvit_profile_stop: null argument");
    std::shared_ptr<Prof> pr;
    {
        std::lock_guard<std::mutex> lk(g_prof_mu);
        auto it = g_profs.find(workspace);
        if (it != g_profs.end()) { pr = it->second; g_profs.erase(it); }
    }
    QV_CHECK_ARG(pr, "qatvit_profile_stop: no profile is active for this workspace");
    size_t used;
    {
        std::lock_guard<std::mutex> lk(pr->mu);
        pr->closed = true;
        used = pr->used;
        *flops = pr->flops;
    }
    double ms = 0.0;
    for (size_t i = 0; i + 1 < used; i += 2) {
        if (hipEventSynchronize(pr->ev[i + 1]) != hipSuccess) continue;
        float t = 0.f;
        if (hipEventElapsedTime(&t, pr->ev[i], pr->ev[i + 1]) == hipSuccess) ms += t;
    }
    *total_ms = ms;
    *launches = (int64_t)(used / 2);
    return 0;
}

int64_t qatvit_student_tensor_offset(const qatvit_cfg* cfg, const char* name, int32_t block) {
    if (!cfg || !name || check_cfg(*cfg)) return -1;
    Plan p;
    if (make_plan(*cfg, &p)) return -1;
    struct { const char* n; int64_t off; bool per_block; } tab[] = {
        {"Y0", p.Y0, false}, {"imgq", p.imgq, false}, {"hq", p.hq, false}, {"logits_pre", p.logits_pre, false}, {"x_in", p.x_in, true},
        {"x_mid", p.x_mid, true}, {"h1q", p.h1q, true}, {"qkv", p.qkv, true}, {"O_hi", p.O_hi, true}, {"O_lo", p.O_lo, true}, {"Yproj", p.Yproj, true}, {"h2q", p.h2q, true},
        {"Y1", p.Y1, true}, {"G_hi", p.G_hi, true}, {"G_lo", p.G_lo, true}, {"Y2", p.Y2, true}, {"dxA", p.dxA, false}, {"dqkv_hi", p.dqkv_hi, false},
        {"dqkv_lo", p.dqkv_lo, false}, {"dO", p.dO, false},
        {"dH", p.dH, false}, {"lse", p.lse, true}, {"O16_hi", p.O16_hi, true}, {"O16_lo", p.O16_lo, true}, {"G16_hi", p.G16_hi, false},
        {"G16_lo", p.G16_lo, false}, {"scal16", p.scal16, true}, {"dy16", p.dy16, false}, {"dYs_hi", p.dYs_hi, false}, {"dY1_hi", p.dY1_hi, false}, {"G8", p.G8, true}, {"glut", p.glut, true}, {"Y1m", p.Y1m, true}, {"glutq", p.glutq, true}, {"qkv8", p.qkv8, true}, {"qkvm", p.qkvm, true},
    };
    for (auto& t : tab)
        if (strcmp(t.n, name) == 0) return t.off + (t.per_block ? p.blk_stride * block : 0);
    return -1;
}

}
```

### qat-vit_amd/csrc/i8strip.hip

```cpp
#include <stdlib.h>

#include <type_traits>

#include "qv_common.h"
#include "qv_kernels.h"
#include "qv_qparams.h"

namespace qv {

typedef int i32x4 __attribute__((ext_vector_type(4)));
typedef __attribute__((address_space(3))) void lds_void;

struct I8StripArgs {
    const int8_t* A;
    const i32x4* Bf;
    int M, N, lda;
    const float* s1;
    const float* s2;
    const float* col_scale;
    const float* bias;
    const int32_t* wsum;
    const float* aqp;
    int center;
    uint32_t* stats;
    int stat_slots;
    const float* qp;
    int qmin, qmax;
    uint8_t* out8;
    uint8_t* out8_mask;
    int ldc;
    int code_T, D;
    uint32_t* lut_out;
    uint32_t* lutq_out;
    float* out16_scale;
    unsigned long long* dbg;
    QpLate late;
};

__device__ inline int strip_off(int row, int chunk) {
    const int R = row >> 1;
    return R * 128 + (((((row & 1) << 2) | chunk) ^ (R & 7)) << 4);
}
__device__ inline void strip_lds_barrier() { asm volatile("s_waitcnt lgkmcnt(0)\n\ts_barrier" ::: "memory"); }

#ifdef QV_STRIP_EXPERIMENTS
#define QV_STAMP() stamp()
#else
#define QV_STAMP() ((void)0)
#endif

template <int MODE, int NTL, int NWV = 8, bool R255 = false, int TM_ = 13, int KT_ = 6>
__global__ __launch_bounds__(NWV * 64, NWV / 4) void k_i8_strip(const I8StripArgs p) {
    constexpr int TM = TM_, TNT = 24 / NWV, WC = 16 * TNT, BM = 16 * TM, BN = 384, KT = KT_, PF = 3, NT_ = NWV * 64;
    static_assert(TM <= 2 * NWV, "the strip's 1-KiB DMA pieces are dealt in two rounds");
    static_assert(NWV == 8 || NWV == 12, "8 waves x 48 columns or 12 waves x 32 columns");
    constexpr int IMGA = BM * 64, LA = KT * IMGA;
    constexpr int NC = NTL * BN;
    constexpr int CH = 4;
    constexpr int WSTG = 16 * CH * WC + 16 * CH * 16;
    extern __shared__ __attribute__((aligned(16))) char smem[];
    char* sA = smem;
    int* sCorr = reinterpret_cast<int*>(smem + LA);
    float* sCa = reinterpret_cast<float*>(sCorr + NC);
    float* sCb = sCa + NC;
    char* sStage = smem + LA + 3 * NC * 4;
    const int tid = threadIdx.x, lane = tid & 63;
    const int wave = __builtin_amdgcn_readfirstlane(tid >> 6);
    const int r = lane & 15, g = lane >> 4;
    const int m0 = blockIdx.x * BM, nbase = blockIdx.y * NTL * BN;
#ifdef QV_STRIP_EXPERIMENTS
    int nstamp = 0;
    auto stamp = [&]() {
        if (p.dbg && (blockIdx.x == 0 || blockIdx.x == 100) && blockIdx.y == 0) {
            const unsigned long long t = __builtin_amdgcn_s_memtime();
            if (lane == 0 && nstamp < 32) p.dbg[((blockIdx.x ? 1 : 0) * 8 + (wave & 7)) * 32 + nstamp] = t;
            ++nstamp;
        }
    };
#endif
    QV_STAMP();

    {
        const int64_t abytes = (int64_t)p.M * p.lda;
        const __amdgpu_buffer_rsrc_t rA = __builtin_amdgcn_make_buffer_rsrc(const_cast<int8_t*>(p.A), 0, abytes > 0xffffffffll ? 0xffffffffu : (uint32_t)abytes, 0x00020000);
        const int lR = lane >> 3, lL = (lane & 7) ^ lR;
        const int prow = 2 * lR + (lL >> 2), pk = lL & 3;
#pragma unroll
        for (int kt = 0; kt < KT; ++kt)
#pragma unroll
            for (int c = 0; c < 2; ++c) {
                const int q = c * NWV + wave;
                if (q < TM) {
                    const uint32_t off = (uint32_t)((int64_t)(m0 + q * 16 + prow) * p.lda + kt * 64 + pk * 16);
                    __builtin_amdgcn_raw_ptr_buffer_load_lds(rA, (lds_void*)(sA + kt * IMGA + q * 1024), 16, off, 0, 0, 0);
                }
            }
    }
    const __amdgpu_buffer_rsrc_t rB = __builtin_amdgcn_make_buffer_rsrc(const_cast<i32x4*>(p.Bf), 0, (uint32_t)((int64_t)p.N * (KT * 64)), 0x00020000);
    const int f0 = nbase / 16 + wave * TNT;
    auto load_b = [&](int nt, int kt, i32x4 (&b)[TNT]) {
#pragma unroll
        for (int j = 0; j < TNT; ++j) {
            const int f = f0 + nt * 24 + j;
            const auto v = __builtin_amdgcn_raw_buffer_load_b128(rB, lane * 16, (((f / 3) * KT + kt) * 3 + f % 3) * 1024, 0);
            b[j] = __builtin_bit_cast(i32x4, v);
        }
    };
    i32x4 bb[2][TNT];
    load_b(0, 0, bb[0]);

    {
        const float alpha = *p.s1 * (p.s2 ? *p.s2 : 1.0f);
        const int zc = p.center - (int)p.aqp[2];
        for (int c = tid; c < NC; c += NT_) {
            sCorr[c] = zc * p.wsum[nbase + c];
            sCa[c] = alpha * (p.col_scale ? p.col_scale[nbase + c] : 1.0f);
            sCb[c] = p.bias ? p.bias[nbase + c] : 0.0f;
        }
    }
    struct Consts { float4 ca, cb; };
    auto consts_of = [&](int nt, int j, int g) {
        const int c = nt * BN + wave * WC + 16 * j + 4 * g;
        return Consts{*reinterpret_cast<const float4*>(sCa + c), *reinterpret_cast<const float4*>(sCb + c)};
    };

    float* sQp = reinterpret_cast<float*>(sStage + (MODE == 3 ? 512 : NWV * WSTG));
    if constexpr (MODE != 3) {
        if (p.late.stats) qp_late_compute(p.late, sQp);
        else if (tid == 0) { sQp[0] = p.qp[0]; sQp[1] = p.qp[1]; sQp[2] = p.qp[2]; }
    }

    asm volatile("s_waitcnt vmcnt(0) lgkmcnt(0)" ::: "memory");
    QV_STAMP();
    __builtin_amdgcn_s_barrier();
    asm volatile("" ::: "memory");
    QV_STAMP();
    const float qp_s = MODE != 3 ? sQp[0] : 0.f, qp_inv = MODE != 3 ? sQp[1] : 0.f, qp_zp = MODE != 3 ? sQp[2] : 0.f;
    if constexpr (MODE == 4) {
        if (blockIdx.x == 0 && blockIdx.y == 0 && tid < 256) {
            const float ga = fabsf(((float)p.qmin - qp_zp) * qp_s), gb = fabsf(((float)p.qmax - qp_zp) * qp_s);
            int ex;
            (void)frexpf(fmaxf(ga, gb), &ex);
            const float gs = ldexpf(1.0f, 14 - ex);
            if (p.out16_scale && tid == 0) *p.out16_scale = ldexpf(1.0f, ex - 14);
            uint32_t wq = 0u, wh = 0u;
            if (tid <= p.qmax - p.qmin) {
                const float gv = gelu_fwd(((float)(tid + p.qmin) - qp_zp) * qp_s);
                const __bf16 gh = (__bf16)gv;
                const __bf16 gl = (__bf16)(gv - (float)gh);
                wq = (uint32_t)__builtin_bit_cast(uint16_t, gh) | ((uint32_t)__builtin_bit_cast(uint16_t, gl) << 16);
                const float g16 = gv * gs;
                const _Float16 hh = (_Float16)g16;
                const _Float16 hl = (_Float16)(g16 - (float)hh);
                wh = (uint32_t)__builtin_bit_cast(uint16_t, hh) | ((uint32_t)__builtin_bit_cast(uint16_t, hl) << 16);
            }
            if (p.lut_out) p.lut_out[tid] = wh;
            if (p.lutq_out) p.lutq_out[tid] = wq;
        }
    }

    float mn = INFINITY, mx = -INFINITY;
    const bool ragged = m0 + BM > p.M;

    i32x4 acc[TM][TNT];
#pragma clang loop unroll(disable)
    for (int nt = 0; nt < NTL; ++nt) {
        i32x4 cinit[TNT];
#pragma unroll
        for (int j = 0; j < TNT; ++j) {
            const int4 c = *reinterpret_cast<const int4*>(sCorr + nt * BN + wave * WC + 16 * j + 4 * g);
            cinit[j] = i32x4{c.x, c.y, c.z, c.w};
        }
        auto kstep = [&](int kt, const i32x4 (&bc)[TNT]) {
            __builtin_amdgcn_sched_barrier(0);
            int opaque = 0;
            asm volatile("" : "+v"(opaque));
            const char* st = sA + opaque + kt * IMGA + strip_off(r, g);
            i32x4 af[PF];
#pragma unroll
            for (int i = 0; i < PF - 1; ++i) af[i] = *reinterpret_cast<const i32x4*>(st + 1024 * i);
#pragma unroll
            for (int i = 0; i < TM; ++i) {
                __builtin_amdgcn_sched_barrier(0);
                if (i + PF - 1 < TM) af[(i + PF - 1) % PF] = *reinterpret_cast<const i32x4*>(st + 1024 * (i + PF - 1));
#pragma unroll
                for (int j = 0; j < TNT; ++j)
                    acc[i][j] = __builtin_amdgcn_mfma_i32_16x16x64_i8(bc[j], af[i % PF], kt == 0 ? cinit[j] : acc[i][j], 0, 0, 0);
            }
        };
        if constexpr (MODE != 3) __builtin_amdgcn_s_setprio(2);
#pragma unroll
        for (int kt = 0; kt < KT; ++kt) {
            if (kt + 1 < KT) load_b(nt, kt + 1, bb[(kt + 1) & 1]);
            else if (nt + 1 < NTL) load_b(nt + 1, 0, bb[0]);
            kstep(kt, bb[kt & 1]);
        }
        __builtin_amdgcn_sched_barrier(0);
        if constexpr (MODE != 3) {
            if (((wave >> 2) + nt) % (NWV / 4) == 0) __builtin_amdgcn_s_setprio(1); else __builtin_amdgcn_s_setprio(0);
        }
        QV_STAMP();

        if constexpr (MODE == 3) {
            int tid3 = threadIdx.x;
            asm volatile("" : "+v"(tid3));
            const int r3 = tid3 & 15, g3 = (tid3 & 63) >> 4;
#pragma unroll
            for (int j = 0; j < TNT; ++j) {
                int lo[4], hi[4];
#pragma unroll
                for (int e = 0; e < 4; ++e) {
                    lo[e] = 0x7fffffff;
                    hi[e] = (int)0x80000000;
                    if (!ragged) {
#pragma unroll
                        for (int i = 0; i < TM; ++i) { lo[e] = min(lo[e], acc[i][j][e]); hi[e] = max(hi[e], acc[i][j][e]); }
                    } else {
#pragma unroll
                        for (int i = 0; i < TM; ++i) {
                            const bool ok = m0 + 16 * i + r3 < p.M;
                            lo[e] = min(lo[e], ok ? acc[i][j][e] : 0x7fffffff);
                            hi[e] = max(hi[e], ok ? acc[i][j][e] : (int)0x80000000);
                        }
                    }
                }
                const Consts k = consts_of(nt, j, g3);
                const float ka[4] = {k.ca.x, k.ca.y, k.ca.z, k.ca.w}, kb[4] = {k.cb.x, k.cb.y, k.cb.z, k.cb.w};
#pragma unroll
                for (int e = 0; e < 4; ++e)
                    if (lo[e] <= hi[e]) {
                        mn = fminf(mn, (float)lo[e] * ka[e] + kb[e]);
                        mx = fmaxf(mx, (float)hi[e] * ka[e] + kb[e]);
                    }
            }
        } else {
            const float qinv = qp_inv, zoff = qp_zp - (float)p.qmin, frange = (float)(p.qmax - p.qmin);
            const uint32_t range_bits = __builtin_bit_cast(uint32_t, frange);
            const int tilebase = nbase + nt * BN;
            int tid2 = threadIdx.x;
            asm volatile("" : "+v"(tid2));
            const int lane2 = tid2 & 63, r2 = lane2 & 15, g2 = lane2 >> 4;
            char* sW = sStage + wave * WSTG;
            char* sWm = sW + 16 * CH * WC;
            const int which = MODE == 7 ? tilebase / p.D : 0, cm0 = MODE == 7 ? tilebase % p.D + wave * WC : 0, Hh = MODE == 7 ? p.D >> 6 : 0;
            const float invT = MODE == 7 ? 1.0f / (float)p.code_T : 0.f;
#pragma unroll
            for (int c0 = 0; c0 < TM; c0 += CH) {
                const int nf = TM - c0 < CH ? TM - c0 : CH;
#pragma unroll
                for (int j = 0; j < TNT; ++j) {
                    const Consts k = consts_of(nt, j, g2);
                    const float ka[4] = {k.ca.x, k.ca.y, k.ca.z, k.ca.w}, kb[4] = {k.cb.x, k.cb.y, k.cb.z, k.cb.w};
#pragma unroll
                    for (int ii = 0; ii < CH; ++ii) {
                        if (ii >= nf) continue;
                        const int i = c0 + ii, rl = 16 * ii + r2;
                        uint32_t pk = 0, mk = 0;
#pragma unroll
                        for (int e = 3; e >= 0; --e) {
                            const float v = (float)acc[i][j][e] * ka[e] + kb[e];
                            const float u = rintf(v * qinv) + zoff;
                            pk = __builtin_amdgcn_cvt_pk_u8_f32(R255 ? u : fminf(u, frange), e, pk);
                            const unsigned long long inr = __builtin_amdgcn_uicmp(__builtin_bit_cast(uint32_t, u), range_bits, 37 );
                            asm("v_addc_co_u32 %0, vcc, %0, %0, %1" : "+v"(mk) : "s"(inr) : "vcc");
                        }
                        *reinterpret_cast<uint32_t*>(sW + rl * WC + 16 * j + 4 * g2) = pk;
                        reinterpret_cast<uint8_t*>(sWm)[rl * 16 + 4 * j + g2] = (uint8_t)mk;
                    }
                }
                asm volatile("s_waitcnt lgkmcnt(0)" ::: "memory");
                const int row0 = m0 + 16 * c0;
#pragma unroll
                for (int k3 = 0; k3 < TNT; ++k3) {
                    if (k3 * 64 >= nf * 16 * TNT) continue;
                    const int pc = lane2 + 64 * k3;
                    const int rl = pc / TNT, c = pc - TNT * rl, row = row0 + rl;
                    const bool ok = pc < nf * 16 * TNT && row < p.M;
                    const uint4 v = *reinterpret_cast<const uint4*>(sW + 16 * pc);
                    uint32_t mx4 = *reinterpret_cast<const uint32_t*>(sWm + rl * 16 + 4 * c) & 0x0f0f0f0fu;
                    mx4 = (mx4 | (mx4 >> 4)) & 0x00ff00ffu;
                    const uint16_t mv = (uint16_t)((mx4 | (mx4 >> 8)) & 0xffffu);
                    if constexpr (MODE == 4) {
                        const uint32_t eo = __umul24((uint32_t)row, (uint32_t)p.ldc) + (uint32_t)(tilebase + wave * WC + 16 * c);
                        if (ok) {
                            *reinterpret_cast<uint4*>(p.out8 + eo) = v;
                            *reinterpret_cast<uint16_t*>(p.out8_mask + (eo >> 3)) = mv;
                        }
                    } else {
                        const int cm = cm0 + 16 * c, hh = cm >> 6, d = cm & 63;
                        const int bb_ = (int)(((float)row + 0.5f) * invT), tt = row - (int)__umul24((uint32_t)bb_, (uint32_t)p.code_T);
                        const uint32_t eo = ((__umul24(__umul24((uint32_t)(bb_ * Hh + hh), 3u) + (uint32_t)which, (uint32_t)p.code_T) + (uint32_t)tt) << 6) + (uint32_t)d;
                        if (ok) {
                            *reinterpret_cast<uint4*>(p.out8 + eo) = v;
                            *reinterpret_cast<uint16_t*>(p.out8_mask + (eo >> 3)) = mv;
                        }
                    }
                }
                asm volatile("" ::: "memory");
            }
            QV_STAMP();
        }
    }

    QV_STAMP();
    if constexpr (MODE == 3) {
        float* sRed = reinterpret_cast<float*>(sStage);
        mn = wave_min(mn);
        mx = wave_max(mx);
        if (lane == 0) { sRed[wave] = mn; sRed[16 + wave] = mx; }
        strip_lds_barrier();
        if (tid == 0) {
#pragma unroll
            for (int w = 1; w < NWV; ++w) { mn = fminf(mn, sRed[w]); mx = fmaxf(mx, sRed[16 + w]); }
        }
        if (tid == 0) stat_atomic(p.stats, p.stat_slots, mn, mx);
    }
}

template <int MODE, int NTL, int NWV, bool R255, int TM, int KT>
static void strip_launch_r(const I8StripArgs& a, hipStream_t st) {
    constexpr int kLds = KT * 16 * TM * 64 + 3 * NTL * 384 * 4 + (MODE == 3 ? 512 : NWV * (64 * (384 / NWV) + 64 * 16)) + 16;
    static_assert(kLds <= 160 * 1024, "strip + constants + staging patches exceed the LDS");
    static bool once = ((void)hipFuncSetAttribute(reinterpret_cast<const void*>(k_i8_strip<MODE, NTL, NWV, R255, TM, KT>), hipFuncAttributeMaxDynamicSharedMemorySize, kLds), true);
    (void)once;
    k_i8_strip<MODE, NTL, NWV, R255, TM, KT><<<dim3(cdiv(a.M, 16 * TM), a.N / (NTL * 384)), NWV * 64, kLds, st>>>(a);
}
template <int MODE, int NTL, int NWV, int TM, int KT>
static void strip_launch_w(const I8StripArgs& a, hipStream_t st) {
    if (MODE != 3 && a.qmax - a.qmin == 255) strip_launch_r<MODE, NTL, NWV, true, TM, KT>(a, st);
    else strip_launch_r<MODE, NTL, NWV, false, TM, KT>(a, st);
}
template <int MODE, int NTL, int TM = 13, int KT = 6>
static void strip_launch(const I8StripArgs& a0, hipStream_t st) {
    I8StripArgs a = a0;
#ifdef QV_STRIP_EXPERIMENTS
    const char* d = getenv("QATVIT_STRIP_DBG");
    a.dbg = d ? reinterpret_cast<unsigned long long*>(strtoull(d, nullptr, 0)) : nullptr;
#endif
    if constexpr (MODE == 3) strip_launch_w<MODE, NTL, 8, TM, KT>(a, st);
    else strip_launch_w<MODE, NTL, 12, TM, KT>(a, st);
}

static int strip_ntl(int N, int K) {
    return K == 384 ? (N % (4 * 384) == 0 ? 4 : N % (3 * 384) == 0 ? 3 : 0) : (N == 6 * 384 ? 6 : N == 8 * 384 ? 8 : 0);
}
static bool strip_addressable(int M, int N, int lda, int ldc, int mode) {
    if ((int64_t)M * lda >= (1ll << 32) || M >= (1 << 22) || (int64_t)M * N >= (1ll << 32) || N >= (1 << 24)) return false;
    if (mode == 4 && (ldc >= (1 << 24) || (int64_t)M * ldc >= (1ll << 32))) return false;
    if (mode == 7 && M >= (1 << 20)) return false;
    return true;
}
bool i8_strip_covers(const void* B8f, int M, int N, int K, int lda, int ldc, const NTPost* post) {
    if (!knobs().i8_strip || !B8f || !post || (K != 384 && K != 768) || lda % 16 != 0 || !strip_addressable(M, N, lda, ldc, post->mode) || !strip_ntl(N, K)) return false;
    if (post->mode == 3) return true;
    if (!post->out8 || !post->out8_mask || post->qmax - post->qmin >= 256) return false;
    if (post->mode == 7) return post->code_hd == 64 && (N / 3) % 384 == 0 && post->code_T >= 1 && post->code_T < 1024;
    if (post->mode == 4) return !(post->out_hi || post->out_lo || post->code || post->out16_hi || post->out16_lo || !post->lut_out || !post->lutq_out || ldc % 128 != 0);
    return false;
}

bool launch_i8_strip(const void* A8, const void* B8f, const int32_t* wsum, const float* a_qp, int center, int M, int N, int K, int lda, int ldc,
                     const float* s1, const float* s2, const float* col_scale, const float* bias, uint32_t* stats, int stat_slots, hipStream_t st,
                     const NTPost* post, bool force, const QpLate* late) {
    if ((!knobs().i8_strip && !force) || !B8f || !post || (K != 384 && K != 768) || lda % 16 != 0 || !s1 || !strip_addressable(M, N, lda, ldc, post->mode)) return false;
    const int ntl = strip_ntl(N, K);
    if (!ntl) return false;
    const bool wide = K == 768;
    I8StripArgs a{};
    a.A = reinterpret_cast<const int8_t*>(A8); a.Bf = reinterpret_cast<const i32x4*>(B8f); a.M = M; a.N = N; a.lda = lda;
    a.s1 = s1; a.s2 = s2; a.col_scale = col_scale; a.bias = bias; a.wsum = wsum; a.aqp = a_qp; a.center = center;
    if (post->mode == 3) {
        if (!stats) return false;
        a.stats = stats; a.stat_slots = stat_slots < 1 ? 1 : stat_slots;
        if (wide) { if (ntl == 8) strip_launch<3, 8, 7, 12>(a, st); else strip_launch<3, 6, 7, 12>(a, st); }
        else if (ntl == 4) strip_launch<3, 4>(a, st); else strip_launch<3, 3>(a, st);
        return true;
    }
    a.qp = post->qp; a.qmin = post->qmin; a.qmax = post->qmax;
    if (late) a.late = *late;
    a.out8 = reinterpret_cast<uint8_t*>(post->out8); a.out8_mask = reinterpret_cast<uint8_t*>(post->out8_mask);
    if ((!a.qp && !a.late.stats) || !a.out8 || !a.out8_mask || a.qmax - a.qmin >= 256) return false;
    if (post->mode == 7) {
        const int D = N / 3;
        if (post->code_hd != 64 || D % 384 != 0 || post->code_T < 1 || post->code_T >= 1024) return false;
        a.code_T = post->code_T; a.D = D;
        if (wide) { if (ntl == 8) strip_launch<7, 8, 7, 12>(a, st); else strip_launch<7, 6, 7, 12>(a, st); }
        else if (ntl == 4) strip_launch<7, 4>(a, st); else strip_launch<7, 3>(a, st);
        return true;
    }
    if (post->mode == 4) {
        if (post->out_hi || post->out_lo || post->code || post->out16_hi || post->out16_lo || !post->lut_out || !post->lutq_out || ldc % 128 != 0) return false;
        a.ldc = ldc; a.lut_out = post->lut_out; a.lutq_out = post->lutq_out; a.out16_scale = post->out16_scale;
        if (wide) { if (ntl == 8) strip_launch<4, 8, 7, 12>(a, st); else strip_launch<4, 6, 7, 12>(a, st); }
        else if (ntl == 4) strip_launch<4, 4>(a, st); else strip_launch<4, 3>(a, st);
        return true;
    }
    return false;
}

}
```

### qat-vit_amd/csrc/qv_common.h

```cpp
#pragma once
#include <hip/hip_runtime.h>
#include <stdint.h>
#include <stdio.h>

namespace qv {

constexpr int kWave = 64;

void set_error(const char* fmt, ...);

struct Knobs {
    bool i8;
    bool f16;
    bool fc2_codes;
    bool fc1_bits;
    bool fc2w_codes;
    bool wbatch;
    bool attn_codes;
    bool qkv_2pass;
    bool lnb_fuse;
    bool qp_late;
    bool tn_stream;
    bool tn_q8;
    bool attn_bwd_fused;
    bool f16_strip;
    bool i8_strip;
};
const Knobs& knobs();

#define QV_CHECK_ARG(cond, ...)                 \
    do {                                        \
        if (!(cond)) {                          \
            qv::set_error(__VA_ARGS__);         \
            return 1;                           \
        }                                       \
    } while (0)

#define QV_CHECK_LAUNCH(name)                                                     \
    do {                                                                          \
        hipError_t e_ = hipGetLastError();                                        \
        if (e_ != hipSuccess) {                                                   \
            qv::set_error("%s: launch failed: %s", name, hipGetErrorString(e_));  \
            return 2;                                                             \
        }                                                                         \
    } while (0)

__host__ __device__ inline uint32_t f2ord(float f) {
    uint32_t u = __builtin_bit_cast(uint32_t, f);
    return (u & 0x80000000u) ? ~u : (u | 0x80000000u);
}
__host__ __device__ inline float ord2f(uint32_t k) {
    uint32_t u = (k & 0x80000000u) ? (k & 0x7fffffffu) : ~k;
    return __builtin_bit_cast(float, u);
}
constexpr uint32_t kOrdPosInf = 0xff800000u;
constexpr uint32_t kOrdNegInf = 0x007fffffu;

constexpr int kStatSlots = 32;
constexpr int kStatStride = 32;
__device__ inline void stat_atomic(uint32_t* stats, int nslots, float mn, float mx) {
    uint32_t* s = stats + (nslots > 1 ? (int)(blockIdx.x & (nslots - 1)) * kStatStride : 0);
    atomicMin(&s[0], f2ord(mn));
    atomicMax(&s[1], f2ord(mx));
}

__device__ inline float wave_min(float v) {
#pragma unroll
    for (int o = 32; o > 0; o >>= 1) v = fminf(v, __shfl_xor(v, o, 64));
    return v;
}
__device__ inline float wave_max(float v) {
#pragma unroll
    for (int o = 32; o > 0; o >>= 1) v = fmaxf(v, __shfl_xor(v, o, 64));
    return v;
}
__device__ inline float wave_sum(float v) {
#pragma unroll
    for (int o = 32; o > 0; o >>= 1) v += __shfl_xor(v, o, 64);
    return v;
}

__device__ inline float fq_one(float x, float inv_scale, float scale, float fzp, float fqmin, float fqmax, bool& in_range) {
    float q = rintf(x * inv_scale) + fzp;
    in_range = (q >= fqmin) && (q <= fqmax);
    float qc = fminf(fmaxf(q, fqmin), fqmax);
    return (qc - fzp) * scale;
}

inline int cdiv(int64_t a, int64_t b) { return (int)((a + b - 1) / b); }

__device__ inline float fast_exp(float x) { return __builtin_amdgcn_exp2f(x * 1.4426950408889634f); }

typedef float qv_f32x2 __attribute__((ext_vector_type(2)));
typedef __bf16 qv_bf16x2 __attribute__((ext_vector_type(2)));
__device__ inline uint32_t pk_bf16(float a, float b) {
    const qv_f32x2 v = {a, b};
    return __builtin_bit_cast(uint32_t, __builtin_convertvector(v, qv_bf16x2));
}
typedef _Float16 qv_f16x2 __attribute__((ext_vector_type(2)));
__device__ inline uint32_t pk_f16(float a, float b) {
    const qv_f32x2 v = {a, b};
    return __builtin_bit_cast(uint32_t, __builtin_convertvector(v, qv_f16x2));
}
__device__ inline void split_pair(float a, float b, uint32_t& hi, uint32_t& lo) {
    const qv_f32x2 v = {a, b};
    hi = __builtin_bit_cast(uint32_t, __builtin_convertvector(v, qv_bf16x2));
    const qv_f32x2 h = {__builtin_bit_cast(float, hi << 16), __builtin_bit_cast(float, hi & 0xffff0000u)};
    const qv_f32x2 r = v - h;
    lo = __builtin_bit_cast(uint32_t, __builtin_convertvector(r, qv_bf16x2));
}

__device__ inline float gelu_fwd(float x) { return 0.5f * x * (1.0f + erff(x * 0.70710678118654752f)); }
__device__ inline float gelu_fwd_fast(float x) {
    const float z = fabsf(x) * 0.70710678118654752f;
    const float t = __builtin_amdgcn_rcpf(fmaf(0.3275911f, z, 1.0f));
    float pl = fmaf(1.061405429f, t, -1.453152027f);
    pl = fmaf(pl, t, 1.421413741f);
    pl = fmaf(pl, t, -0.284496736f);
    pl = fmaf(pl, t, 0.254829592f);
    const float E = pl * t * __builtin_amdgcn_exp2f(-z * z * 1.4426950408889634f);
    return x < 0.f ? 0.5f * x * E : x * (1.0f - 0.5f * E);
}
__device__ inline float gelu_bwd(float x) {
    return 0.5f * (1.0f + erff(x * 0.70710678118654752f)) + x * 0.3989422804014327f * expf(-0.5f * x * x);
}

}
```

### qat-vit_amd/csrc/qv_kernels.h

```cpp
#pragma once
#include <hip/hip_runtime.h>
#include <stdint.h>

namespace qv {

int launch_fq_forward(const float* x, float* y, uint8_t* mask_bits, float* running_min, float* running_max, float* scale,
                      int32_t* zero_point, const int64_t* observer_on, const int64_t* fake_quant_on, float c, int qmin, int qmax,
                      int64_t channels, int64_t inner, bool per_channel, bool symmetric, void* workspace, hipStream_t st);
int launch_fq_backward(const float* dy, const uint8_t* mask_bits, float* dx, int64_t n, hipStream_t st);

int launch_ln_forward(const float* x, const float* gamma, const float* beta, float* y, float* mean, float* rstd, int64_t rows,
                      int64_t dim, float eps, hipStream_t st);
int launch_ln_backward(const float* dy, const float* x, const float* gamma, const float* mean, const float* rstd, float* dx,
                       float* dgamma, float* dbeta, int64_t rows, int64_t dim, hipStream_t st);

int launch_kd_ce_loss(const float* student, const float* teacher, const int64_t* labels, int64_t batch, int64_t classes, float kd_temp,
                      float kd_alpha, float label_smoothing, float* out3, float* dlogits, hipStream_t st);
int launch_kd_ce_loss_table(const float* student, const float* table, int64_t table_rows, const int64_t* index, const int64_t* labels, int64_t batch,
                            int64_t classes, float kd_temp, float kd_alpha, float label_smoothing, float* out3, float* dlogits, hipStream_t st);

int launch_minmax(const float* x, int64_t channels, int64_t inner, int per_channel, uint32_t* ws, int nslots, hipStream_t st);
int launch_ws_init(uint32_t* ws, int64_t slots, hipStream_t st);
int launch_qparams(uint32_t* ws, float* running_min, float* running_max, float* scale, int32_t* zero_point, const int64_t* observer_on,
                   const int64_t* fake_quant_on, float c, int qmin, int qmax, int64_t channels, int symmetric, float* qp_out, int reset_ws,
                   int nslots, hipStream_t st);

constexpr int kMaxActFq = 96;
struct QpCommitTab { float* rmin[kMaxActFq]; float* rmax[kMaxActFq]; float* scale[kMaxActFq]; int32_t* zp[kMaxActFq]; float* staged; uint32_t* stats; int n; };
int launch_qp_commit(const QpCommitTab& t, hipStream_t st);
struct QpLate {
    const uint32_t* stats;
    const float* rmin; const float* rmax; const float* scale; const int32_t* zp;
    const int64_t* obs_on; const int64_t* fq_on;
    float c; int qmin, qmax;
    float* qp_out;
    float* staged;
};
constexpr int kQpStagedWords = 8;

struct NTPost {
    const float* Y;
    const float* qp;
    int qmin, qmax;
    const float* colscale;
    void* out_hi;
    void* out_lo;
    int mode = 0;
    void* code = nullptr;
    void* out16_hi = nullptr;
    void* out16_lo = nullptr;
    float* out16_scale = nullptr;
    const float* resid = nullptr;
    int embed_np = 0;
    void* out8 = nullptr;
    int code_T = 0, code_hd = 0;
    uint32_t* lut_out = nullptr;
    uint32_t* lutq_out = nullptr;
    const void* code8 = nullptr;
    const void* code_mask = nullptr;
    void* out8_mask = nullptr;
    const float* lnb_x = nullptr;
    const float* lnb_mean = nullptr;
    const float* lnb_rstd = nullptr;
    const float* lnb_gamma = nullptr;
    const float* lnb_beta = nullptr;
    const float* lnb_dx_in = nullptr;
    float* lnb_dgamma = nullptr;
    float* lnb_dbeta = nullptr;
    const void* lnb_nmask = nullptr;
    int out_f16 = 0;
    const float* o16_mul = nullptr;
    uint32_t* o16_amax = nullptr;
};

int launch_gemm_nt(const void* A_hi, const void* A_lo, const void* B, float* C, int M, int N, int K, int lda, int ldb, int ldc, const float* s1,
                   const float* s2, const float* col_scale, const float* bias, uint32_t* stats, int stat_slots, hipStream_t st,
                   const void* B_lo = nullptr, const NTPost* post = nullptr, bool f16 = false);
int launch_gemm_nt_i8(const void* A8, const void* B8, const int32_t* wsum, const float* a_qp, int center, float* C, int M, int N, int K, int lda,
                      int ldb, int ldc, const float* s1, const float* s2, const float* col_scale, const float* bias, uint32_t* stats, int stat_slots,
                      hipStream_t st, const NTPost* post = nullptr,
                      const void* B8f = nullptr,
                      const QpLate* late = nullptr);
int launch_gemm_nt_dy16(const void* A16, const void* B16, float* C, int M, int N, int K, int lda, int ldb, int ldc, const float* s1, const float* s2,
                        hipStream_t st, const NTPost* post = nullptr, bool bf16 = false);
bool launch_f16_strip_gelu_bwd(const void* A16, const void* B16f, float* unused, int M, int N, int K, int lda, int ldc, const float* s1, const float* s2, hipStream_t st,
                               const NTPost* post);
bool launch_i8_strip(const void* A8, const void* B8f, const int32_t* wsum, const float* a_qp, int center, int M, int N, int K, int lda, int ldc,
                     const float* s1, const float* s2, const float* col_scale, const float* bias, uint32_t* stats, int stat_slots, hipStream_t st,
                     const NTPost* post, bool force = false, const QpLate* late = nullptr);
bool i8_strip_covers(const void* B8f, int M, int N, int K, int lda, int ldc, const NTPost* post);
__host__ __device__ inline int64_t w8f_offset(int n, int k, int K) {
    const int cg = n / 48, cr = n % 48, j = cr / 16, r = cr % 16, kt = k / 64, kk = k % 64;
    return ((((int64_t)cg * (K / 64) + kt) * 3 + j) * 64 + (kk / 16) * 16 + r) * 16 + (kk % 16);
}
int launch_w8_fragment_order(const void* B8, void* B8f, int N, int K, hipStream_t st);
int launch_gemm_nt_codes(const void* A8, const uint32_t* lut, const void* B16, float* C, int M, int N, int K, int lda, int ldb, int ldc, const float* s1,
                         const float* s2, const float* col_scale, const float* bias, uint32_t* stats, int stat_slots, hipStream_t st, const NTPost* post = nullptr);
constexpr int64_t kTnScratchBytes = 256ll * 128 * 384 * 4;
int launch_gemm_tn(const void* P_hi, const void* P_lo, const void* Q_hi, const void* Q_lo, float* C, int M, int N, int Kw, int ldp, int ldq, int ldc,
                   const float* s1, const float* W, const float* w_scale, const int32_t* w_zp, int w_per_channel, int w_qmin, int w_qmax,
                   float* dbias, const float* row_div, hipStream_t st, float* partial = nullptr, int64_t partial_bytes = 0);
int launch_gemm_tn_codes(const void* P_hi, const void* P_lo, const void* Qc, const uint32_t* lutQ, float* C, int M, int N, int Kw, int ldp, int ldq, int ldc,
                         const float* s1, const float* W, const float* w_scale, const int32_t* w_zp, int w_per_channel, int w_qmin, int w_qmax, float* dbias,
                         const float* row_div, hipStream_t st, float* partial = nullptr, int64_t partial_bytes = 0);
int launch_gemm_tn_dy16(const void* P16, const void* Q_hi, const void* Q_lo, float* C, int M, int N, int Kw, int ldp, int ldq, int ldc, const float* s1,
                        const float* s2, const float* W, const float* w_scale, const int32_t* w_zp, int w_per_channel, int w_qmin, int w_qmax, float* dbias,
                        const float* row_div, hipStream_t st, float* partial = nullptr, int64_t partial_bytes = 0, bool bf16 = false);
int launch_gemm_tn_codes_dy16(const void* P16, const void* Qc, const uint32_t* lutQ16, float* C, int M, int N, int Kw, int ldp, int ldq, int ldc, const float* s1,
                              const float* s2, const float* W, const float* w_scale, const int32_t* w_zp, int w_per_channel, int w_qmin, int w_qmax, float* dbias,
                              const float* row_div, hipStream_t st, float* partial = nullptr, int64_t partial_bytes = 0);
int launch_gemm_tn_q8_dy16(const void* P16, const void* Q8, const float* a_qp, int center, float* C, int M, int N, int Kw, int ldp, int ldq, int ldc, const float* s2,
                           const float* W, const float* w_scale, const int32_t* w_zp, int w_per_channel, int w_qmin, int w_qmax, float* dbias, const float* row_div,
                           hipStream_t st, float* partial = nullptr, int64_t partial_bytes = 0);
struct TNStreamGemm {
    const void* P; const void* Q; const uint32_t* lut; const float* s1; const float* s2; float* C; const float* W; const float* w_scale; const int32_t* w_zp; float* dbias;
    const float* row_div; int N, Kw, ldp, ldq, ldc;
};
int64_t tn_stream_scratch_bytes();
int launch_tn_stream(int mode, const TNStreamGemm* items, int n, int M, int center, int w_per_channel, int w_qmin, int w_qmax, float* partial, int64_t partial_bytes,
                     hipStream_t st);
int launch_img_patches(const float* img, void* out_bf16, const float* qp, int qmin, int qmax, int B, int C, int H, int W, int P, hipStream_t st,
                       void* out8 = nullptr, int center = 0);
int launch_resid_fq_lnstats(int mode, const float* x_prev, const float* Y, const float* qpY, int qmin, int qmax, const float* cls, const float* pos,
                            float* x_new, float* mean, float* rstd, const float* gamma, const float* beta, float eps, uint32_t* stats, int stat_slots,
                            int64_t M, int D, int T, hipStream_t st, void* maskbits = nullptr, const QpLate* late = nullptr);
inline int64_t ln_maskbits_bytes(int64_t M, int D) { return M * ((D + 255) / 256) * 32; }
struct LnBwdNext { const void* maskbits; const float* colscale; void* out_hi; void* out_lo; const float* o16_mul = nullptr; uint32_t* o16_amax = nullptr; };
int launch_ln_apply_quant(const float* x, const float* mean, const float* rstd, const float* gamma, const float* beta, const float* qp, int qmin,
                          int qmax, void* out_bf16, int64_t M, int D, hipStream_t st, void* out8 = nullptr, int center = 0,
                          bool out_f16 = false,
                          const QpLate* late = nullptr);
int launch_ln_quant8(const float* x, const float* gamma, const float* beta, float eps, const float* qp, int qmin, int qmax, int center, void* out8,
                     float* mean, float* rstd, int64_t nrows, int64_t row_stride, int D, hipStream_t st);
int launch_cls_rows(const float* cls, const float* pos, float* x, int B, int T, int D, hipStream_t st);
int launch_mask_bwd(int gelu_bwd, const float* d, const float* Y, const float* qp, int qmin, int qmax, const float* col_scale, int ncols,
                    void* dst_hi, void* dst_lo, int64_t n, hipStream_t st, const float* o16_mul = nullptr, uint32_t* o16_amax = nullptr);
int launch_ln_bwd_fq(int acc, const float* dH, const float* x, const float* mean, const float* rstd, const float* gamma, const float* beta,
                     const float* qp, int qmin, int qmax, const float* dx_in, float* dx_out, float* dgamma, float* dbeta, int64_t M, int D, int T,
                     int cls_only, hipStream_t st, const LnBwdNext* next = nullptr);
int launch_head_fwd(const float* x, const float* mean, const float* rstd, const float* gamma, const float* beta, const float* qp_norm, int qmin,
                    int qmax, const void* wq, const float* w_scale, int w_per_channel, const float* bias, float* hq, float* logits_pre,
                    uint32_t* stats, int stat_slots, int B, int D, int T, int C, hipStream_t st);
int launch_logits_fq(const float* pre, const float* qp, int qmin, int qmax, float* out, int n, hipStream_t st);
int launch_head_bwd(const float* dlogits, const float* logits_pre, const float* qp_logits, int qmin, int qmax, const float* hq, const float* qp_norm,
                    const void* wq, const float* W, const float* w_scale, const int32_t* w_zp, int w_per_channel, int w_qmin, int w_qmax, float* dW,
                    float* dbias, float* dh, int B, int D, int C, hipStream_t st);
int launch_embed_bwd(const float* dx0, const float* Y0, const float* qp, int qmin, int qmax, float* dpos, float* dcls, void* dY0_hi, void* dY0_lo,
                     int B, int T, int D, hipStream_t st);
constexpr int kMaxW = 52;
struct WObsTab { const float* W[kMaxW]; uint32_t* ws[kMaxW]; int N[kMaxW], K[kMaxW], blk0[kMaxW + 1]; int n, per_channel, nslots; };
struct WQpTab {
    uint32_t* ws[kMaxW]; float* rmin[kMaxW]; float* rmax[kMaxW]; float* scale[kMaxW]; int32_t* zp[kMaxW]; float* qp[kMaxW];
    const int64_t* obs_on[kMaxW]; const int64_t* fq_on[kMaxW]; int N[kMaxW], blk0[kMaxW + 1]; int n, per_channel, nslots, qmin, qmax; float c;
};
struct WQuantTab {
    const float* W[kMaxW]; const float* qp[kMaxW]; void* wq[kMaxW]; void* wqT[kMaxW]; void* w8[kMaxW]; int32_t* wsum[kMaxW];
    void* w16[kMaxW];
    void* w8f[kMaxW];
    int N[kMaxW], K[kMaxW], blk0[kMaxW + 1]; int n, per_channel, qmin, qmax;
    int wT16;
    unsigned long long wT16f_mask;
};
__host__ __device__ inline int64_t wT16_gap_bytes(int N, int K) { return ((int64_t)N * K * 2 + 255) & ~(int64_t)255; }
int launch_w_observe_all(WObsTab& t, hipStream_t st);
int launch_w_qparams_all(WQpTab& t, hipStream_t st);
int launch_w_quant_all(WQuantTab& t, hipStream_t st);
int launch_zero_i32(int32_t* p, int64_t n, hipStream_t st);
struct ObsFoldEntry {
    uint32_t* ws; float* rmin; float* rmax; float* scale; int32_t* zp; const int64_t* obs_on; const int64_t* fq_on;
    int32_t channels, nslots, symmetric, qmin, qmax, blk0;
};
int launch_obs_fold(const ObsFoldEntry* tab, int n, int nblocks, float c, hipStream_t st);
int launch_wquant(const float* W, const float* qp, int per_channel, int qmin, int qmax, void* wq, void* wqT, int N, int K, hipStream_t st);

constexpr int kDyHdrWords = 64, kDySlotWords = 256, kDyAmaxStride = 32, kDyAmaxSlots = 8;
inline int64_t dy16_state_bytes(int nslots) { return 4ll * (kDyHdrWords + (int64_t)nslots * kDySlotWords); }
int launch_dy16_begin(uint32_t* state, int nslots, const float* dlogits, int n_dlogits, hipStream_t st);
int launch_dy16_set_mirror(uint32_t* state, void* host_pinned, hipStream_t st);
int launch_dy16_end(uint32_t* state, int nslots, int check_overflow, hipStream_t st);
int launch_absmax_bf16(const void* hi, int64_t n, uint32_t* amax, hipStream_t st);
int launch_q8_to_bf16int(const void* q8, const float* qp, int center, void* plane, int64_t n, hipStream_t st);
int launch_f16int_to_bf16int(void* plane, int64_t n, hipStream_t st);

int attn_padded_tokens(int T);
int launch_attn_fwd(const float* qkv, const float* qp, int qmin, int qmax, int B, int T, int H, int D, void* O_hi, void* O_lo, float* lse,
                    hipStream_t st, void* O16_hi = nullptr, void* O16_lo = nullptr, float* o16_scale = nullptr, void* codes = nullptr,
                    void* cmask = nullptr);
int launch_attn_bwd(const float* qkv, const float* qp, int qmin, int qmax, int B, int T, int H, int D, const void* O_hi, const void* O_lo,
                    const float* lse, float* delta, const float* dO, void* dqkv_hi, void* dqkv_lo, const float* col_scale, hipStream_t st,
                    const void* codes = nullptr, const void* cmask = nullptr,
                    const float* o16_mul = nullptr, uint32_t* o16_amax = nullptr);
bool attn_bwd_is_fused(int T, int H, int D, bool codes);

int launch_attn_fwd_float(const float* qkv, int B, int T, int H, int D, void* O_hi, void* O_lo, hipStream_t st, int f16 = 0, float* lse = nullptr);
int launch_patches_split(const float* img, void* hi, void* lo, int B, int C, int H, int W, int P, hipStream_t st, int f16 = 0);
int launch_resid_ln_split_save(int mode, const float* x_prev, const float* Y, const float* cls, const float* pos, float* x_new, const float* gamma,
                               const float* beta, float eps, void* h_hi, void* h_lo, float* mean, float* rstd, int64_t M, int D, int T, hipStream_t st,
                               uint32_t* stats = nullptr, int f16 = 0);
int launch_gelu_split(const float* Y, void* hi, void* lo, int64_t n, hipStream_t st);
int launch_attn_bwd_f16(const float* qkv, const void* O16, const float* lse, const float* dO, int B, int T, int H, int D, void* dqkv16, hipStream_t st,
                        bool bf16 = false);
int launch_fa_wcast(int n, const float* const* W, void* const* w16, void* const* w16T, const int* N, const int* K, const int* blk0, hipStream_t st,
                    bool bf16 = false);
int launch_fa_head_fwd(const float* x, const float* mean, const float* rstd, const float* gamma, const float* beta, const float* W, const float* bias, float* hn,
                       void* logits16, int B, int D, int T, int C, hipStream_t st, bool bf16 = false);
int launch_fa_head_bwd(const void* dl16, const float* hn, const float* W, float* dW, float* dbias, float* dhn, int B, int D, int C, hipStream_t st,
                       bool bf16 = false);
int launch_fa_gelu(const float* Y, void* G16, int64_t n, hipStream_t st, bool bf16 = false);
int launch_fa_gelu_bwd(const float* dG, const float* Y, void* dY16, int64_t n, hipStream_t st, bool bf16 = false);
int launch_fa_embed_bwd(const float* dx, float* dpos, float* dcls, void* dY0_16, int B, int T, int D, hipStream_t st, bool bf16 = false);
int launch_fa_inf_rule(float* const* g, const int64_t* n, int count, hipStream_t st);
constexpr int kImgTaps = 4, kImgBits = 22, kImgBand = 16, kImgMaxD = 384;
int image_resize_coeffs(int src, int dst, int32_t* xmin, int32_t* ntaps, int32_t* coef);
void image_table(const float* mean, const float* stdv, float* table);
int launch_image_batch(const uint8_t* data, const int64_t* index, int B, int N, int S, int D, const int32_t* coeffs, const float* table, float* out,
                       hipStream_t st);
inline int flat_grid_fs(int64_t n) {
    int64_t b = (n + 255) / 256;
    return (int)(b < 1 ? 1 : (b > 4096 ? 4096 : b));
}

}
```

### qat-vit_amd/engine.py

```python
from __future__ import annotations

import ctypes
import os
import time
import warnings
import weakref
from typing import Callable, Dict, List, Optional, Sequence, Tuple

import torch
import torch.distributed as dist
from torch.ao.quantization.fake_quantize import FusedMovingAvgObsFakeQuantize

from . import float_engine, native

STAGE_INJECT = 1
FWD_X16 = 2
BWD_DY16 = 2
BWD_CALIBRATE = 4


def dy16_default() -> bool:
    return os.environ.get("QATVIT_DY16", "1") != "0"


# ... 76 lines not shown


def decide_fq_mode(state: FqModeState, flags: Sequence[torch.Tensor], names: Sequence[str]) -> str:
    versions = fq_versions(flags)
    if versions == state.versions:
        return state.mode
    on = (torch.stack([t.reshape(-1)[0] for t in flags]) != 0).tolist()
    state.reads += 1
    if all(on):
        mode = QAT
    elif not any(on):
        mode = OBSERVE
    else:
        def some(xs):
            return ", ".join(xs[:8]) + (f" (+{len(xs) - 8} more)" if len(xs) > 8 else "")
        en = [n for n, o in zip(names, on) if o]
        dis = [n for n, o in zip(names, on) if not o]
        raise RuntimeError(
            f"qat-vit_amd: fake-quant is enabled on {len(en)} modules ({some(en)}) and disabled on {len(dis)} ({some(dis)}); the native step supports "
            "fake_quant_enabled = 1 everywhere (QAT) or 0 everywhere (observe-only) - apply torch.ao.quantization.enable_fake_quant / disable_fake_quant "
            "to the whole model")
    state.versions, state.mode = versions, mode
    return mode


def fq_modules_and_names(wrapper: torch.nn.Module):
    _, act, wfq = collect_student(wrapper)
    names = {id(m): n for n, m in wrapper.named_modules()}
    fqs = list(act) + list(wfq)
    return fqs, [names.get(id(f), type(f).__name__) for f in fqs]


def fq_flags_and_names(wrapper: torch.nn.Module):
    fqs, names = fq_modules_and_names(wrapper)
    return [f.fake_quant_enabled for f in fqs], names



def _fq_of(mod, attr):
    fq = getattr(mod, attr, None)
    if not isinstance(fq, FusedMovingAvgObsFakeQuantize):
        raise RuntimeError(
            f"{type(mod).__name__}.{attr} is {type(fq).__name__}: the native path implements the fused moving-average "
            "fake-quant that get_default_qat_qconfig('qnnpack'|'x86'|'fbgemm') installs"
        )
    return fq


def collect_student(wrapper: torch.nn.Module):
    m = wrapper.model
    blocks = list(m.blocks)
    pe = m.patch_embed.proj
    ps = native.vit_params(m)
    act = [_fq_of(wrapper.quant, "activation_post_process"), _fq_of(pe, "activation_post_process")]
    wfq = [_fq_of(pe, "weight_fake_quant")]
    for b in blocks:
        act += [_fq_of(x, "activation_post_process") for x in (b.norm1, b.attn.qkv, b.attn.proj, b.norm2, b.mlp.fc1, b.mlp.fc2)]
        wfq += [_fq_of(x, "weight_fake_quant") for x in (b.attn.qkv, b.attn.proj, b.mlp.fc1, b.mlp.fc2)]
    act += [_fq_of(m.norm, "activation_post_process"), _fq_of(m.head, "activation_post_process")]
    wfq += [_fq_of(m.head, "weight_fake_quant")]
    return ps, act, wfq


def weight_param_indices(n_params: int) -> List[int]:
    depth = (n_params - 8) // 12
    idx = [0]
    for i in range(depth):
        idx += [4 + 12 * i + 2, 4 + 12 * i + 4, 4 + 12 * i + 8, 4 + 12 * i + 10]
    return idx + [n_params - 2]


def rehome_fq_state(params, act_fq, w_fq, device):
    sizes = []
    for f, w in [(f, None) for f in act_fq] + list(zip(w_fq, [params[i] for i in weight_param_indices(len(params))])):
        sizes.append(w.shape[0] if (w is not None and f.is_per_channel) else 1)
    tot = sum(sizes)
    arena = torch.empty(16 * tot, dtype=torch.uint8, device=device)
    f32 = arena[:12 * tot].view(torch.float32)
    i32 = arena[12 * tot:].view(torch.int32)
    o = 0
    for f, c in zip(list(act_fq) + list(w_fq), sizes):
        obs = f.activation_post_process
        per_ch = f.is_per_channel
        mn, mx, sc, zp = f32[o:o + c], f32[tot + o:tot + o + c], f32[2 * tot + o:2 * tot + o + c], i32[o:o + c]
        if obs.min_val.numel() == c:
            mn.copy_(obs.min_val.reshape(-1)); mx.copy_(obs.max_val.reshape(-1))
        else:
            mn.fill_(float("inf")); mx.fill_(float("-inf"))
        if f.scale.numel() == c:
            sc.copy_(f.scale.reshape(-1)); zp.copy_(f.zero_point.reshape(-1))
        else:
            sc.fill_(1.0); zp.fill_(0)
        obs._buffers["min_val"] = mn if per_ch else mn.view(())
        obs._buffers["max_val"] = mx if per_ch else mx.view(())
        f._buffers["scale"] = sc
        f._buffers["zero_point"] = zp
        o += c
    return f32, i32, arena, tot


@torch.no_grad()
def broadcast_fq_state(arena: torch.Tensor, pg) -> None:
    dist.broadcast(arena, src=0, group=pg)


class StudentEngine:

    def __init__(self, wrapper: torch.nn.Module, batch: int):
        m = wrapper.model
        dev = m.cls_token.device
        if dev.type != "cuda":
            raise RuntimeError("StudentEngine needs the model on an MI355X (cuda) device")
        self.device = dev
        self.lib = native.lib()
        blocks = list(m.blocks)
        ps, act, wfq = collect_student(wrapper)
        for p in ps:
            if p is None or p.dtype != torch.float32 or not p.is_contiguous():
                raise RuntimeError("every student parameter must be a contiguous fp32 tensor (bias=True everywhere)")
        self.params: List[torch.nn.Parameter] = ps
        self.act_fq, self.w_fq = act, wfq
        a0, w0 = act[0], wfq[0]
        for f in act:
            if f.is_per_channel or f.is_symmetric_quant or (f.activation_post_process.quant_min, f.activation_post_process.quant_max) != (
                    a0.activation_post_process.quant_min, a0.activation_post_process.quant_max):
                raise RuntimeError("activation fake-quant must be per-tensor affine with one common range")
        for f in wfq:
            if not f.is_symmetric_quant or f.is_per_channel != w0.is_per_channel or (f.is_per_channel and f.ch_axis != 0):
                raise RuntimeError("weight fake-quant must be symmetric, all per-tensor or all per-channel (axis 0)")
        self._fq_flags, self._fq_names = fq_flags_and_names(wrapper)
        self._fq_state = FqModeState()
        self.fq_mode: Optional[str] = None
        self.float_form = float_engine.Form(*float_engine.FP32)
        self.observe_buf: Optional[torch.Tensor] = None
        hd = blocks[0].attn.head_dim
        self._cfg_kw = dict(
            native.vit_shape(m), act_qmin=a0.activation_post_process.quant_min, act_qmax=a0.activation_post_process.quant_max,
            w_qmin=w0.activation_post_process.quant_min, w_qmax=w0.activation_post_process.quant_max, w_per_channel=int(w0.is_per_channel),
            averaging_const=float(a0.activation_post_process.averaging_constant),
        )
        self._cfgs: Dict[int, native.Cfg] = {}
        self.cfg = self.cfg_for(batch)
        if hd * self.cfg.num_heads != self.cfg.embed_dim:
            raise RuntimeError("embed_dim must equal num_heads * head_dim")
        L, cp = self.lib, ctypes.byref(self.cfg)
        assert L.qatvit_student_num_params(cp) == len(ps) and L.qatvit_student_num_act_fq(cp) == len(act) and L.qatvit_student_num_weight_fq(cp) == len(wfq)
        self._rehome_fq_state()
        self.capacity = 0
        self.workspace: Optional[torch.Tensor] = None
        self._pins = 0
        self.dy16 = dy16_default() and bool(self.lib.qatvit_student_dy16_supported(ctypes.byref(self.cfg)))
        self._dy16_calibrated = False
        self._fwd_x16 = False
        self.dy16_fallbacks = 0
        self._mirror = self._mirror_np = None
        self._mirror_on = os.environ.get("QATVIT_DY16_MIRROR", "1") != "0"
        self._gen_issued = 0
        self._agree_store, self._agree_round = None, 0
        self._reserve(batch)
        self.layout = FlatGradLayout([p.numel() for p in ps], self.cfg.depth)
        self.grad_numel = self.layout.numel
        self._ptr_params = (ctypes.c_void_p * len(ps))(*[p.data_ptr() for p in ps])
        self._param_ptrs_key = tuple(p.data_ptr() for p in ps)
        self.pg = None
        self.sync_state = True
        self.bucket_bytes = 16 << 20
        self.exposed_events: Optional[list] = None
        self.generation = 0
        self._build_fq_structs()

    def cfg_for(self, batch: int) -> native.Cfg:
        c = self._cfgs.get(batch)
        if c is None:
            c = self._cfgs[batch] = native.Cfg(batch=batch, **self._cfg_kw)
        return c

    @property
    def frozen(self) -> bool:
        return self._pins > 0

    def pin(self) -> None:
        self._pins += 1

    def unpin(self) -> None:
        self._pins = max(0, self._pins - 1)

    def _reserve(self, batch: int) -> None:
        if batch <= self.capacity:
            return
        if self.frozen:
            raise RuntimeError(f"batch {batch} exceeds the workspace ({self.capacity}) a captured hipGraph is bound to")
        L, cp = self.lib, ctypes.byref(self.cfg_for(batch))
        nbytes = L.qatvit_student_workspace_bytes(cp)
        if nbytes <= 0:
            raise RuntimeError("qatvit_student_workspace_bytes: " + L.qatvit_last_error().decode())
        self.workspace = None
        self.workspace = torch.empty(nbytes, dtype=torch.uint8, device=self.device)
        native.check(L.qatvit_student_init(cp, self.workspace.data_ptr(), native.stream_ptr()), "qatvit_student_init")
        self.capacity = batch
        self._dy16_calibrated = False
        off = L.qatvit_student_tensor_offset(cp, b"dy16", 0)
        self._dy16_flag = self.workspace[off + 8:off + 12].view(torch.int32)
        self._install_mirror(cp)

    def _install_mirror(self, cp) -> None:
        self._mirror = self._mirror_np = None
        self._gen_issued = 0
        if not (self._mirror_on and self.dy16):
            return
        try:
            m = torch.zeros(2, dtype=torch.int32).pin_memory()
        except RuntimeError:
            return
        if self.lib.qatvit_student_dy16_set_mirror(cp, self.workspace.data_ptr(), m.data_ptr(), native.stream_ptr()) != 0:
            return
        self._mirror, self._mirror_np = m, m.numpy()

    def _mirror_wait(self) -> Optional[bool]:
        m, want, t0 = self._mirror_np, self._gen_issued & 0xffffffff, time.perf_counter()
        while ((int(m[1]) - want) & 0xffffffff) >= 0x80000000:
            if time.perf_counter() - t0 > 10.0:
                return None
            time.sleep(0)
        return bool(int(m[0]))

    def _rehome_fq_state(self):
        self.fq_f32, self.fq_i32, self.fq_arena, self.fq_total = rehome_fq_state(self.params, self.act_fq, self.w_fq, self.device)

    def _build_fq_structs(self):
        def arr(fqs):
            a = (native.FQ * len(fqs))()
            for s, f in zip(a, fqs):
                obs = f.activation_post_process
                s.min_val, s.max_val, s.scale, s.zero_point = obs.min_val.data_ptr(), obs.max_val.data_ptr(), f.scale.data_ptr(), f.zero_point.data_ptr()
                s.observer_on, s.fake_quant_on = f.observer_enabled.data_ptr(), f.fake_quant_enabled.data_ptr()
            return a
        self._act_structs, self._w_structs = arr(self.act_fq), arr(self.w_fq)

    def enable_data_parallel(self, process_group=None, bucket_bytes: int = 16 << 20):
        if not dist.is_initialized():
            raise RuntimeError("torch.distributed is not initialised")
        self.pg = process_group if process_group is not None else dist.group.WORLD
        self.bucket_bytes = bucket_bytes
        for p in self.params:
            dist.broadcast(p.data, src=0, group=self.pg)
        self._agree_store, self._agree_round = None, 0
        ranks = dist.get_process_group_ranks(self.pg)
        self._dp_epoch = getattr(self, "_dp_epoch", 0) + 1
        tag = torch.tensor([id(self) & 0x7fffffff, self._dp_epoch], dtype=torch.int64, device=self.device)
        dist.broadcast(tag, src=ranks[0], group=self.pg)
        if os.environ.get("QATVIT_DY16_STORE_AGREE", "1") != "0":
            try:
                from torch.distributed.distributed_c10d import _get_default_store
                self._agree_store = dist.PrefixStore(f"qatvit_dy16/{int(tag[0].item())}.{int(tag[1].item())}/{'-'.join(map(str, ranks))}", _get_default_store())
                self._agree_store.add("probe", 0)
            except Exception:
                self._agree_store = None
        can = torch.tensor([1 if self._agree_store is not None else 0], dtype=torch.int32, device=self.device)
        dist.all_reduce(can, op=dist.ReduceOp.MIN, group=self.pg)
        if int(can.item()) == 0:
            self._agree_store = None

    def _agree_overflow(self, local: bool) -> bool:
        st, k, world = self._agree_store, self._agree_round, dist.get_world_size(self.pg)
        self._agree_round += 1
        if local:
            st.add(f"o{k}", 1)
        n = st.add(f"a{k}", 1)
        t0 = time.perf_counter()
        while n < world:
            if time.perf_counter() - t0 > 60.0:
                raise RuntimeError("one-plane backward: a rank of the data-parallel group did not report its overflow flag within 60 s")
            time.sleep(0)
            n = st.add(f"a{k}", 0)
        over = st.add(f"o{k}", 0) > 0
        if k >= 2 and dist.get_rank(self.pg) == 0:
            for key in (f"a{k - 2}", f"o{k - 2}"):
                try:
                    st.delete_key(key)
                except Exception:
                    pass
        return over

    def _broadcast_fq_state(self):
        broadcast_fq_state(self.fq_arena, self.pg)

    def _check_ptrs(self):
        if tuple(p.data_ptr() for p in self.params) != self._param_ptrs_key:
            raise RuntimeError("student parameters were re-allocated after the native engine was built (e.g. .to()); rebuild the wrapper")

    def _check_shape(self, images: torch.Tensor) -> None:
        c0 = self.cfg
        if images.dim() != 4 or images.shape[0] < 1 or tuple(images.shape[1:]) != (c0.in_chans, c0.img_size, c0.img_size) or images.dtype != torch.float32:
            raise RuntimeError(f"expected fp32 images of shape (B, {c0.in_chans}, {c0.img_size}, {c0.img_size}), got {tuple(images.shape)} {images.dtype}")
        self._check_ptrs()

    def _check_images(self, images: torch.Tensor) -> native.Cfg:
        self._check_shape(images)
        self._reserve(images.shape[0])
        return self.cfg_for(images.shape[0])

    def fq_versions(self) -> Tuple[int, ...]:
        return fq_versions(self._fq_flags)

    def decide_mode(self) -> str:
        prev = self._fq_state.mode
        mode = decide_fq_mode(self._fq_state, self._fq_flags, self._fq_names)
        if mode == QAT and prev == OBSERVE:
            self._dy16_calibrated = False
        return mode

    def forward(self, images: torch.Tensor) -> torch.Tensor:
        mode = self.decide_mode()
        self.fq_mode = mode
        if mode == OBSERVE:
            return self._forward_observe(images)
        c = self._check_images(images)
        self.cfg = c
        if self.pg is not None and self.sync_state:
            self._broadcast_fq_state()
        images = images.contiguous()
        logits = torch.empty(c.batch, c.num_classes, dtype=torch.float32, device=self.device)
        self.generation += 1
        self._fwd_x16 = self.dy16 and self._dy16_calibrated and self.sync_state
        native.check(self.lib.qatvit_student_forward_stages(ctypes.byref(c), self._ptr_params, self._act_structs, self._w_structs, images.data_ptr(),
                                                            logits.data_ptr(), self.workspace.data_ptr(), 0, c.depth + 1, FWD_X16 if self._fwd_x16 else 0,
                                                            native.stream_ptr()), "qatvit_student_forward")
        return logits

    def _reserve_observe(self, c: native.Cfg) -> None:
        L, cp = self.lib, ctypes.byref(c)
        if self.observe_buf is None:
            n = L.qatvit_float_student_observe_bytes(cp)
            if n <= 0:
                raise RuntimeError("observe-only step: " + L.qatvit_last_error().decode())
            buf = torch.empty(n, dtype=torch.uint8, device=self.device)
            native.check(L.qatvit_float_student_observe_init(cp, self._act_structs, self._w_structs, buf.data_ptr(), native.stream_ptr()),
                         "qatvit_float_student_observe_init")
            self.observe_buf = buf
        self.float_form.reserve(c, self.device)

    def _forward_observe(self, images: torch.Tensor) -> torch.Tensor:
        self._check_shape(images)
        c = self.cfg_for(images.shape[0])
        self._reserve_observe(c)
        self.cfg = c
        if self.pg is not None and self.sync_state:
            self._broadcast_fq_state()
        images = images.contiguous()
        logits = torch.empty(c.batch, c.num_classes, dtype=torch.float32, device=self.device)
        self.generation += 1
        self._fwd_x16 = False
        native.check(self.lib.qatvit_float_student_forward_observe(ctypes.byref(c), self._ptr_params, images.data_ptr(), logits.data_ptr(),
                                                                   self.float_form.workspace.data_ptr(), self.observe_buf.data_ptr(), native.stream_ptr()),
                     "qatvit_float_student_forward_observe")
        return logits

    def backward_observe(self, dlogits: torch.Tensor, c: native.Cfg) -> List[torch.Tensor]:
        flat, views, gptr = self._grad_buffers()
        self.float_form.call("backward", ctypes.byref(c), self._ptr_params, dlogits.contiguous().data_ptr(), gptr)
        if self.pg is not None:
            if dist.get_backend(self.pg) == "nccl":
                dist.all_reduce(flat, op=dist.ReduceOp.AVG, group=self.pg)
            else:
                dist.all_reduce(flat, op=dist.ReduceOp.SUM, group=self.pg)
                flat.div_(dist.get_world_size(self.pg))
        return views

    def _grad_buffers(self):
        flat = torch.zeros(self.grad_numel, dtype=torch.float32, device=self.device)
        views = self.layout.views(flat, [p.shape for p in self.params])
        gptr = (ctypes.c_void_p * len(views))(*[v.data_ptr() for v in views])
        return flat, views, gptr

    def _run_backward(self, dlogits: torch.Tensor, c: native.Cfg, flags: int):
        flat, views, gptr = self._grad_buffers()
        L, cp, st = self.lib, ctypes.byref(c), native.stream_ptr()

        def run(s0, s1):
            native.check(L.qatvit_student_backward_stages(cp, self._ptr_params, self._act_structs, self._w_structs, dlogits.data_ptr(), gptr,
                                                          self.workspace.data_ptr(), s0, s1, flags, st), "qatvit_student_backward")
            if flags & (BWD_DY16 | BWD_CALIBRATE) and not torch.cuda.is_current_stream_capturing():
                self._gen_issued += 1

        if self.pg is None:
            run(0, self.layout.last_stage)
        else:
            staged_backward_allreduce(flat, self.layout, self.bucket_bytes, self.pg, run, self.exposed_events)
        return views

    def dy16_overflowed(self) -> bool:
        flag = self._dy16_flag
        if self.pg is not None:
            flag = flag.clone()
            dist.all_reduce(flag, op=dist.ReduceOp.MAX, group=self.pg)
        over = bool(flag.item())
        if self._mirror_np is not None:
            self._gen_issued = int(self._mirror_np[1]) & 0xffffffff
        return over

    def backward(self, dlogits: torch.Tensor, cfg: Optional[native.Cfg] = None, x16: Optional[bool] = None):
        c = cfg if cfg is not None else self.cfg
        dlogits = dlogits.contiguous()
        x16 = self._fwd_x16 if x16 is None else x16
        if not self.dy16:
            return self._run_backward(dlogits, c, 0)
        if not x16:
            views = self._run_backward(dlogits, c, BWD_CALIBRATE)
            self._dy16_calibrated = True
            return views
        views = self._run_backward(dlogits, c, BWD_DY16)
        if torch.cuda.is_current_stream_capturing():
            return views
        over = None
        if self.pg is None:
            if self._mirror_np is not None:
                over = self._mirror_wait()
        elif self._agree_store is not None:
            local = self._mirror_wait() if self._mirror_np is not None else None
            over = self._agree_overflow(bool(self._dy16_flag.item()) if local is None else local)
        if over is None:
            over = self.dy16_overflowed()
        if over:
            views = self.dy16_fallback(dlogits, c)
        return views

    def dy16_fallback(self, dlogits: torch.Tensor, c: native.Cfg):
        self.dy16_fallbacks += 1
        if self.dy16_fallbacks == 1:
            warnings.warn("qat-vit_amd: a gradient outgrew its fp16 plane (scale predicted from the previous step); this backward was repeated in the "
                          "bf16-pair form. Harmless if rare (engine.dy16_fallbacks counts them); QATVIT_DY16=0 keeps the pair form throughout.",
                          RuntimeWarning, stacklevel=3)
        native.check(self.lib.qatvit_student_dy16_to_pair(ctypes.byref(c), self.workspace.data_ptr(), native.stream_ptr()), "qatvit_student_dy16_to_pair")
        self._fwd_x16 = False
        return self._run_backward(dlogits, c, BWD_CALIBRATE)

    def tensor(self, name: str, block: int, shape, dtype=torch.float32, cfg: Optional[native.Cfg] = None) -> torch.Tensor:
        c = cfg if cfg is not None else self.cfg
        off = self.lib.qatvit_student_tensor_offset(ctypes.byref(c), name.encode(), block)
        if off < 0:
            raise KeyError(name)
        n = 1
        for s in shape:
            n *= s
        return self.workspace[off:off + n * torch.empty((), dtype=dtype).element_size()].view(dtype).view(*shape)

    def forward_stages(self, images: Optional[torch.Tensor], stage_from: int, stage_to: int, inject: bool = False,
                       logits: Optional[torch.Tensor] = None, x16: bool = False) -> Optional[torch.Tensor]:
        c = self.cfg
        if stage_to == c.depth + 1 and logits is None:
            logits = torch.empty(c.batch, c.num_classes, dtype=torch.float32, device=self.device)
        self.generation += 1
        native.check(self.lib.qatvit_student_forward_stages(
            ctypes.byref(c), self._ptr_params, self._act_structs, self._w_structs, images.data_ptr() if images is not None else None,
            logits.data_ptr() if logits is not None else None, self.workspace.data_ptr(), stage_from, stage_to,
            (STAGE_INJECT if inject else 0) | (FWD_X16 if x16 else 0), native.stream_ptr()), "qatvit_student_forward_stages")
        return logits

    def forward_part(self, block: int, part: int, inject: bool = False, x16: bool = False) -> None:
        self.generation += 1
        native.check(self.lib.qatvit_student_forward_part(ctypes.byref(self.cfg), self._ptr_params, self._act_structs, self._w_structs,
                                                          self.workspace.data_ptr(), block, part, (STAGE_INJECT if inject else 0) | (FWD_X16 if x16 else 0),
                                                          native.stream_ptr()),
                     "qatvit_student_forward_part")

    def backward_stages(self, dlogits: Optional[torch.Tensor], stage_from: int, stage_to: int, inject: bool = False, mode: int = 0):
        c = self.cfg
        flat, views, gptr = self._grad_buffers()
        native.check(self.lib.qatvit_student_backward_stages(
            ctypes.byref(c), self._ptr_params, self._act_structs, self._w_structs, dlogits.contiguous().data_ptr() if dlogits is not None else None,
            gptr, self.workspace.data_ptr(), stage_from, stage_to, (STAGE_INJECT if inject else 0) | mode, native.stream_ptr()), "qatvit_student_backward_stages")
        if mode & (BWD_DY16 | BWD_CALIBRATE):
            self._gen_issued += 1
        return views


class _StudentStep(torch.autograd.Function):
# ... 50 lines not shown
```

### qat-vit_amd/native.py

```python
from __future__ import annotations

import ctypes
import os
import subprocess
from ctypes import c_char_p, c_double, c_float, c_int, c_int32, c_int64, c_void_p

_HERE = os.path.dirname(os.path.abspath(__file__))
LIB_PATH = os.path.join(_HERE, "libqatvit.so")
CSRC = os.path.join(_HERE, "csrc")
_lib = None

SIGNATURES = {
    "qatvit_abi_version": (c_int, []),
    "qatvit_last_error": (c_char_p, []),
    "qatvit_target_arch": (c_char_p, []),
    "qatvit_fq_workspace_bytes": (c_int64, [c_int64]),
    "qatvit_fq_forward": (c_int, [c_void_p] * 9 + [c_float, c_int32, c_int32, c_int64, c_int64, c_int32, c_int32, c_void_p, c_void_p]),
    "qatvit_fq_backward": (c_int, [c_void_p, c_void_p, c_void_p, c_int64, c_void_p]),
    "qatvit_ln_forward": (c_int, [c_void_p] * 6 + [c_int64, c_int64, c_float, c_void_p]),
    "qatvit_ln_backward": (c_int, [c_void_p] * 8 + [c_int64, c_int64, c_void_p]),
    "qatvit_kd_ce_loss": (c_int, [c_void_p, c_void_p, c_void_p, c_int64, c_int64, c_float, c_float, c_float, c_void_p, c_void_p, c_void_p]),
    "qatvit_kd_ce_loss_table": (c_int, [c_void_p, c_void_p, c_int64, c_void_p, c_void_p, c_int64, c_int64, c_float, c_float, c_float, c_void_p, c_void_p, c_void_p]),
    "qatvit_optim_grad_norm": (c_int, [c_void_p] * 4 + [c_int32, c_int64, c_float, c_void_p, c_void_p, c_void_p]),
    "qatvit_optim_adamw": (c_int, [c_void_p] * 7 + [c_int32, c_int64] + [c_double] * 5 + [c_int64, c_void_p, c_void_p]),
    "qatvit_gemm_nt": (c_int, [c_void_p] * 4 + [c_int32] * 6 + [c_void_p] * 6),
    "qatvit_gemm_nt_f16": (c_int, [c_void_p] * 4 + [c_int32] * 6 + [c_void_p] * 6),
    "qatvit_gemm_nt_i8_minmax": (c_int, [c_void_p] * 4 + [c_int32] * 6 + [c_void_p] * 6),
    "qatvit_w8_fragment_order": (c_int, [c_void_p, c_void_p, c_int32, c_int32, c_void_p]),
    "qatvit_i8_strip": (c_int, [c_int32] + [c_void_p] * 4 + [c_int32] * 5 + [c_void_p] * 6 + [c_int32, c_int32, c_void_p, c_void_p, c_int32] + [c_void_p] * 4),
    "qatvit_gemm_nt_codes": (c_int, [c_void_p] * 4 + [c_int32] * 6 + [c_void_p] * 6),
    "qatvit_gemm_nt_i8": (c_int, [c_void_p] * 4 + [c_int32, c_void_p] + [c_int32] * 6 + [c_void_p] * 6),
    "qatvit_gemm_tn_scratch_bytes": (c_int64, []),
    "qatvit_gemm_tn": (c_int, [c_void_p] * 5 + [c_int32] * 6 + [c_void_p] * 4 + [c_int32] * 3 + [c_void_p] * 3 + [c_int64, c_void_p]),
    "qatvit_gemm_tn_codes": (c_int, [c_void_p] * 5 + [c_int32] * 6 + [c_void_p] * 4 + [c_int32] * 3 + [c_void_p] * 3 + [c_int64, c_void_p]),
    "qatvit_gemm_nt_dy16": (c_int, [c_void_p] * 3 + [c_int32] * 6 + [c_void_p] * 3),
    "qatvit_gemm_tn_dy16": (c_int, [c_void_p] * 6 + [c_int32] * 6 + [c_void_p] * 5 + [c_int32] * 3 + [c_void_p] * 3 + [c_int64, c_void_p]),
    "qatvit_gemm_tn_q8_dy16": (c_int, [c_void_p] * 3 + [c_int32, c_void_p] + [c_int32] * 6 + [c_void_p] * 4 + [c_int32] * 3 + [c_void_p] * 3 + [c_int64, c_void_p]),
    "qatvit_gemm_tn_stream_scratch_bytes": (c_int64, []),
    "qatvit_gemm_tn_stream_dy16": (c_int, [c_int32, c_void_p, c_int32, c_int32, c_int32, c_int32, c_int32, c_int32, c_void_p, c_int64, c_void_p]),
    "qatvit_attn_padded_tokens": (c_int32, [c_int32]),
    "qatvit_attn_forward": (c_int, [c_void_p, c_void_p] + [c_int32] * 6 + [c_void_p] * 4),
    "qatvit_attn_forward_f16": (c_int, [c_void_p, c_void_p] + [c_int32] * 6 + [c_void_p] * 9),
    "qatvit_attn_backward": (c_int, [c_void_p, c_void_p] + [c_int32] * 6 + [c_void_p] * 11),
    "qatvit_student_num_params": (c_int32, [c_void_p]),
    "qatvit_student_num_act_fq": (c_int32, [c_void_p]),
    "qatvit_student_num_weight_fq": (c_int32, [c_void_p]),
    "qatvit_student_workspace_bytes": (c_int64, [c_void_p]),
    "qatvit_student_init": (c_int, [c_void_p, c_void_p, c_void_p]),
    "qatvit_student_forward": (c_int, [c_void_p] * 8),
    "qatvit_student_backward": (c_int, [c_void_p] * 7 + [c_int32, c_int32, c_void_p]),
    "qatvit_student_forward_stages": (c_int, [c_void_p] * 7 + [c_int32, c_int32, c_int32, c_void_p]),
    "qatvit_student_forward_part": (c_int, [c_void_p] * 5 + [c_int32, c_int32, c_int32, c_void_p]),
    "qatvit_student_backward_stages": (c_int, [c_void_p] * 7 + [c_int32, c_int32, c_int32, c_void_p]),
    "qatvit_student_tensor_offset": (c_int64, [c_void_p, c_char_p, c_int32]),
    "qatvit_student_dy16_supported": (c_int32, [c_void_p]),
    "qatvit_student_dy16_to_pair": (c_int, [c_void_p, c_void_p, c_void_p]),
    "qatvit_student_dy16_set_mirror": (c_int, [c_void_p, c_void_p, c_void_p, c_void_p]),
    "qatvit_teacher_workspace_bytes": (c_int64, [c_void_p]),
    "qatvit_teacher_forward": (c_int, [c_void_p] * 8),
    "qatvit_teacher_forward_f16": (c_int, [c_void_p, c_void_p, c_void_p, c_int32, c_void_p, c_void_p, c_void_p, c_void_p]),
    "qatvit_float_student_workspace_bytes": (c_int64, [c_void_p]),
    "qatvit_float_student_init": (c_int, [c_void_p] * 3),
    "qatvit_float_student_forward": (c_int, [c_void_p] * 6),
    "qatvit_float_student_backward": (c_int, [c_void_p] * 6),
    "qatvit_float_student_observe_bytes": (c_int64, [c_void_p]),
    "qatvit_float_student_observe_init": (c_int, [c_void_p] * 5),
    "qatvit_float_student_forward_observe": (c_int, [c_void_p] * 7),
    "qatvit_float_student_amp_workspace_bytes": (c_int64, [c_void_p]),
    "qatvit_float_student_amp_init": (c_int, [c_void_p] * 3),
    "qatvit_float_student_amp_forward": (c_int, [c_void_p] * 6),
    "qatvit_float_student_amp_backward": (c_int, [c_void_p] * 6),
    "qatvit_float_student_amp_attn_backward": (c_int, [c_void_p] * 4 + [c_int32] * 4 + [c_void_p] * 2),
    "qatvit_float_student_bf16_workspace_bytes": (c_int64, [c_void_p]),
    "qatvit_float_student_bf16_init": (c_int, [c_void_p] * 3),
    "qatvit_float_student_bf16_forward": (c_int, [c_void_p] * 6),
    "qatvit_float_student_bf16_backward": (c_int, [c_void_p] * 6),
    "qatvit_float_student_bf16_attn_backward": (c_int, [c_void_p] * 4 + [c_int32] * 4 + [c_void_p] * 2),
    "qatvit_infer_workspace_bytes": (c_int64, [c_void_p]),
    "qatvit_infer_prepare": (c_int, [c_void_p] * 6),
    "qatvit_infer_forward": (c_int, [c_void_p] * 8),
    "qatvit_image_resize_coeffs": (c_int, [c_int32, c_int32, c_void_p, c_void_p, c_void_p]),
    "qatvit_image_table": (c_int, [c_void_p] * 3),
    "qatvit_image_batch": (c_int, [c_void_p, c_void_p] + [c_int32] * 4 + [c_void_p] * 4),
    "qatvit_profile_start": (c_int, [c_void_p, c_int32, c_int32]),
    "qatvit_profile_stop": (c_int, [c_void_p, c_void_p, c_void_p, c_void_p]),
}


class Cfg(ctypes.Structure):
    _fields_ = [(n, c_int32) for n in ("batch", "img_size", "patch_size", "in_chans", "embed_dim", "depth", "num_heads", "mlp_hidden",
                                       "num_classes", "act_qmin", "act_qmax", "w_qmin", "w_qmax", "w_per_channel")] + \
               [("averaging_const", c_float), ("ln_eps", c_float)]


def vit_params(model) -> list:
    pe = model.patch_embed.proj
    ps = [pe.weight, pe.bias, model.cls_token, model.pos_embed]
    for b in model.blocks:
        ps += [b.norm1.weight, b.norm1.bias, b.attn.qkv.weight, b.attn.qkv.bias, b.attn.proj.weight, b.attn.proj.bias,
               b.norm2.weight, b.norm2.bias, b.mlp.fc1.weight, b.mlp.fc1.bias, b.mlp.fc2.weight, b.mlp.fc2.bias]
    return ps + [model.norm.weight, model.norm.bias, model.head.weight, model.head.bias]


def vit_shape(model) -> dict:
    b0 = model.blocks[0]
    return dict(img_size=model.patch_embed.img_size, patch_size=model.patch_embed.patch_size, in_chans=model.patch_embed.proj.weight.shape[1],
                embed_dim=model.embed_dim, depth=len(model.blocks), num_heads=b0.attn.num_heads, mlp_hidden=b0.mlp.fc1.weight.shape[0],
                num_classes=model.head.weight.shape[0], ln_eps=float(b0.norm1.eps))


class TNItem(ctypes.Structure):
    _fields_ = [(n, c_void_p) for n in ("P", "Q", "lut", "s1", "s2", "C", "W", "w_scale", "w_zp", "dbias", "row_div")] + [(n, c_int32) for n in ("N", "Kw", "ldp", "ldq", "ldc")]


class FQ(ctypes.Structure):
    _fields_ = [(n, c_void_p) for n in ("min_val", "max_val", "scale", "zero_point", "observer_on", "fake_quant_on")]


def build(verbose: bool = False) -> str:
    r = subprocess.run(["make", "-C", CSRC, "-j8"], capture_output=True, text=True)
    if r.returncode != 0:
        raise RuntimeError("building libqatvit.so failed:\n" + r.stdout[-4000:] + r.stderr[-4000:])
    if verbose:
        print(r.stdout[-2000:])
    return LIB_PATH


def lib() -> ctypes.CDLL:
    global _lib
    if _lib is None:
        if not os.path.exists(LIB_PATH):
            raise RuntimeError(
                f"{LIB_PATH} is missing: the MI355X path has no fallback. Build it with "
                "`python -c 'import __graft_entry__ as g; g.build()'` (needs hipcc)."
            )
        L = ctypes.CDLL(LIB_PATH)
        for name, (res, args) in SIGNATURES.items():
            fn = getattr(L, name)
            fn.restype, fn.argtypes = res, args
        if L.qatvit_abi_version() != 4:
            raise RuntimeError("libqatvit.so ABI version mismatch")
        _lib = L
    return _lib


def check(status: int, what: str) -> None:
    if status != 0:
        raise RuntimeError(f"{what} failed ({status}): {lib().qatvit_last_error().decode()}")


def stream_ptr() -> int:
    import torch

    return torch.cuda.current_stream().cuda_stream
```

Measured before the change: 16070.

## Fuse LayerNorm apply and int8 quantization into the int8 strip statistics pass

Measured after the change: 16290 (median of 6 runs). +1.4%, better.

```diff
diff --git a/include/qatvit.h b/include/qatvit.h
--- a/include/qatvit.h
+++ b/include/qatvit.h
@@ -59,6 +59,13 @@
                     int32_t lda, const float* s1, const float* s2, const float* col_scale, const float* bias, uint32_t* stats, const float* out_qp,
                     int32_t qmin, int32_t qmax, void* out8, void* out8_mask, int32_t code_T, uint32_t* lut_out, uint32_t* lutq_out,
                     float* out16_scale, void* stream);
+
+int qatvit_ln_apply_quant8(const float* x, const float* mean, const float* rstd, const float* gamma, const float* beta, const float* qp, int32_t qmin, int32_t qmax,
+                           void* out8, int32_t center, int64_t M, int32_t D, void* stream);
+
+int qatvit_i8_strip_ln(const float* x, const float* mean, const float* rstd, const float* gamma, const float* beta, int32_t ln_qmin, int32_t ln_qmax, void* out8,
+                       const void* B8f, const int32_t* wsum, const float* a_qp, int32_t center, int32_t M, int32_t N, int32_t K, int32_t lda, const float* s2,
+                       const float* col_scale, const float* bias, uint32_t* stats, void* stream);
 
 int qatvit_gemm_nt_codes(const void* A8, const uint32_t* lut, const void* B16, float* C, int32_t M, int32_t N, int32_t K, int32_t lda, int32_t ldb,
                          int32_t ldc, const float* s1, const float* s2, const float* col_scale, const float* bias, uint32_t* stats, void* stream);
@@ -138,6 +145,7 @@
 #define QATVIT_BWD_DY16 2
 #define QATVIT_BWD_CALIBRATE 4
 int32_t qatvit_student_dy16_supported(const qatvit_cfg* cfg);
+int32_t qatvit_student_ln_in_strip(const qatvit_cfg* cfg, int32_t flags);
 int qatvit_student_dy16_set_mirror(const qatvit_cfg* cfg, void* workspace, void* host_pinned, void* stream);
 int qatvit_student_dy16_to_pair(const qatvit_cfg* cfg, void* workspace, void* stream);
 int qatvit_student_forward_stages(const qatvit_cfg* cfg, void* const* params, const qatvit_fq* act_fq, const qatvit_fq* weight_fq,
diff --git a/qat-vit_amd/csrc/capi.hip b/qat-vit_amd/csrc/capi.hip
--- a/qat-vit_amd/csrc/capi.hip
+++ b/qat-vit_amd/csrc/capi.hip
@@ -22,7 +22,7 @@
 const Knobs& knobs() {
     static const Knobs k{knob("QATVIT_I8"), knob("QATVIT_F16"), knob("QATVIT_FC2_CODES"), knob("QATVIT_FC1_BITS"), knob("QATVIT_FC2W_CODES"),
                          knob("QATVIT_WBATCH"), knob("QATVIT_ATTN_CODES"), knob("QATVIT_QKV_2PASS"), knob("QATVIT_LNB_FUSE"), knob("QATVIT_QP_LATE"),
-                         knob("QATVIT_TN_STREAM"), knob("QATVIT_TN_Q8"), knob("QATVIT_ATTN_BWD_FUSED"), knob("QATVIT_F16_STRIP"), knob("QATVIT_I8_STRIP")};
+                         knob("QATVIT_TN_STREAM"), knob("QATVIT_TN_Q8"), knob("QATVIT_ATTN_BWD_FUSED"), knob("QATVIT_F16_STRIP"), knob("QATVIT_I8_STRIP"), knob("QATVIT_LN_STRIP")};
     return k;
 }
 }
@@ -160,6 +160,29 @@
     return 0;
 }
 
+int qatvit_ln_apply_quant8(const float* x, const float* mean, const float* rstd, const float* gamma, const float* beta, const float* qp, int32_t qmin, int32_t qmax,
+                           void* out8, int32_t center, int64_t M, int32_t D, void* stream) {
+    QV_CHECK_ARG(x && mean && rstd && gamma && beta && qp && out8, "qatvit_ln_apply_quant8: null pointer argument");
+    QV_CHECK_ARG(M >= 1 && D >= 4 && D % 4 == 0, "qatvit_ln_apply_quant8: M=%lld D=%d (D %% 4 == 0)", (long long)M, D);
+    if (launch_ln_apply_quant(x, mean, rstd, gamma, beta, qp, qmin, qmax, nullptr, M, D, (hipStream_t)stream, out8, center)) return 1;
+    QV_CHECK_LAUNCH("qatvit_ln_apply_quant8");
+    return 0;
+}
+
+int qatvit_i8_strip_ln(const float* x, const float* mean, const float* rstd, const float* gamma, const float* beta, int32_t ln_qmin, int32_t ln_qmax, void* out8,
+                       const void* B8f, const int32_t* wsum, const float* a_qp, int32_t center, int32_t M, int32_t N, int32_t K, int32_t lda, const float* s2,
+                       const float* col_scale, const float* bias, uint32_t* stats, void* stream) {
+    QV_CHECK_ARG(x && mean && rstd && gamma && beta && out8 && B8f && wsum && a_qp && stats, "qatvit_i8_strip_ln: null pointer argument");
+    if (!launch_i8_strip_ln(x, mean, rstd, gamma, beta, ln_qmin, ln_qmax, out8, B8f, wsum, a_qp, center, M, N, K, lda, s2, col_scale, bias, stats, 1,
+                            (hipStream_t)stream, true)) {
+        set_error("qatvit_i8_strip_ln: unsupported arguments (M=%d N=%d K=%d lda=%d: need K = 384 with N = 1152 or 1536, or K = 768 with N = 2304 or 3072; "
+                  "lda %% 16 == 0, lda >= K, 0 < M < 2^22)", M, N, K, lda);
+        return 1;
+    }
+    QV_CHECK_LAUNCH("qatvit_i8_strip_ln");
+    return 0;
+}
+
 int qatvit_gemm_nt_codes(const void* A8, const uint32_t* lut, const void* B16, float* C, int32_t M, int32_t N, int32_t K, int32_t lda, int32_t ldb,
                          int32_t ldc, const float* s1, const float* s2, const float* col_scale, const float* bias, uint32_t* stats, void* stream) {
     QV_CHECK_ARG(A8 && lut && B16 && C, "qatvit_gemm_nt_codes: null pointer argument");
diff --git a/qat-vit_amd/csrc/engine.hip b/qat-vit_amd/csrc/engine.hip
--- a/qat-vit_amd/csrc/engine.hip
+++ b/qat-vit_amd/csrc/engine.hip
@@ -70,6 +70,7 @@
     bool x_plane_from_q8;
     bool tn_stream;
     bool dy16;
+    bool ln_in_strip;
 };
 static Forms forms_of(const qatvit_cfg& c, const Dims& d) {
     const Knobs& k = knobs();
@@ -90,6 +91,7 @@
     f.x_plane_from_q8 = f.i8 && k.tn_q8 && d.D % 384 == 0;
     f.tn_stream = k.tn_stream && d.D % 384 == 0 && d.Hd % 384 == 0;
     f.dy16 = f.i8 && f.w_batched && d.D % 384 == 0 && d.Hd % 384 == 0 && f.qkv_2pass && f.attn_bwd_fused && f.f16_proj && f.fc2w_codes;
+    f.ln_in_strip = k.ln_strip && f.i8 && f.late && f.x_plane_from_q8;
     return f;
 }
 
@@ -203,6 +205,15 @@
     return 0;
 }
 
+static bool ln_in_strip_of(const Plan& p, const Dims& d, int flags, int kind) {
+    const Forms& F = p.form;
+    if (!F.ln_in_strip || !(flags & QATVIT_FWD_X16) || (kind == WB_QKV && !F.qkv_2pass) || d.depth < 1) return false;
+    const int wi = 1 + kind;
+    int N, K; wshape(d, wi, &N, &K);
+    if (!(F.w_batched && p.w8f_off[wi] >= 0) || K != d.D) return false;
+    return i8_strip_ln_covers(&p , (int)d.M, N, K, K);
+}
+
 static int check_cfg(const qatvit_cfg& c) {
     if (c.batch < 1 || c.depth < 1 || c.embed_dim % 128 != 0 || c.mlp_hidden % 128 != 0 || c.embed_dim % c.num_heads != 0 ||
         c.img_size % c.patch_size != 0 || (c.in_chans * c.patch_size * c.patch_size) % 128 != 0 || c.embed_dim > 768) {
@@ -317,6 +328,24 @@
         return launch_ln_apply_quant(xrow, mean, rstd, gamma, beta, act_qp(ai), c.act_qmin, c.act_qmax, x16 && p.form.x_plane_from_q8 ? nullptr : out16, d.M, d.D,
                                      st, p.form.i8 ? out8 : nullptr, center(), x16, lt ? &L : nullptr);
     }
+    struct LnRows { const float* x; const float* mean; const float* rstd; const float* gamma; const float* beta; int ai; };
+    bool ln_in_strip(int kind) const { return ln_in_strip_of(p, d, flags, kind); }
+    int linear_stats_ln(const LnRows& r, void* out8, int M, int wi, const float* bias, int ai_out, bool late_strip) const {
+        int N, K; wshape(d, wi, &N, &K);
+        const qatvit_fq& f = wfq[wi];
+        {
+            ProfScope ps(prof, 7, 0.0, st);
+            const QpLate L = late(r.ai);
+            if (!late_kind(r.ai) ||
+                !launch_i8_strip_ln(r.x, r.mean, r.rstd, r.gamma, r.beta, c.act_qmin, c.act_qmax, out8, w8f(wi), at<int32_t>(p.wsum_off[wi]), act_qp(r.ai), center(), M, N, K, K,
+                                    c.w_per_channel ? nullptr : f.scale, c.w_per_channel ? f.scale : nullptr, bias, act_stats(ai_out), kStatSlots, st, false, &L)) {
+                set_error("engine: the statistics pass with the LayerNorm prologue does not cover layer %d (M=%d N=%d K=%d)", wi, M, N, K);
+                return 1;
+            }
+        }
+        qparams_after(ai_out, true, late_strip);
+        return 0;
+    }
     void qparams_act(int ai) const {
         const qatvit_fq& f = act[ai];
         launch_qparams(act_stats(ai), f.min_val, f.max_val, f.scale, f.zero_point, f.observer_on, f.fake_quant_on, c.averaging_const,
@@ -419,16 +448,21 @@
         float* xin = x.blk<float>(p.x_in, i);
         float* xmid = x.blk<float>(p.x_mid, i);
         if (parts & 1) {
-        x.ln_apply(xin, x.blk<float>(p.mean1, i), x.blk<float>(p.rstd1, i), x.bprm(i, B_N1W), x.bprm(i, B_N1B), x.aidx(i, AB_N1), x.blk<void>(p.h1q, i),
-                   x.blk<void>(p.h1q8, i));
+        const bool ln1 = x.ln_in_strip(WB_QKV);
+        if (!ln1)
+            x.ln_apply(xin, x.blk<float>(p.mean1, i), x.blk<float>(p.rstd1, i), x.bprm(i, B_N1W), x.bprm(i, B_N1B), x.aidx(i, AB_N1), x.blk<void>(p.h1q, i),
+                       x.blk<void>(p.h1q8, i));
         if (F.qkv_2pass) {
             NTPost p2{};
             p2.mode = 7; p2.qp = x.act_qp(x.aidx(i, AB_QKV)); p2.qmin = qa; p2.qmax = qb;
             p2.out8 = x.blk<void>(p.qkv8, i); p2.out8_mask = x.blk<void>(p.qkvm, i); p2.code_T = (int)d.T; p2.code_hd = (int)(d.D / d.H);
             const bool lt = x.late_in_strip(M, x.widx(i, WB_QKV), &p2);
             const NTPost p1{nullptr, nullptr, 0, 0, nullptr, nullptr, nullptr, 3, nullptr};
-            if (x.linear_fwd_grid(x.blk<void>(p.h1q, i), x.blk<void>(p.h1q8, i), M, x.widx(i, WB_QKV), x.act_qp(x.aidx(i, AB_N1)), x.bprm(i, B_QKVB), nullptr,
-                                  x.aidx(i, AB_QKV), &p1, true, lt))
+            if (ln1) {
+                const Ctx::LnRows r{xin, x.blk<float>(p.mean1, i), x.blk<float>(p.rstd1, i), x.bprm(i, B_N1W), x.bprm(i, B_N1B), x.aidx(i, AB_N1)};
+                if (x.linear_stats_ln(r, x.blk<void>(p.h1q8, i), M, x.widx(i, WB_QKV), x.bprm(i, B_QKVB), x.aidx(i, AB_QKV), lt)) return 1;
+            } else if (x.linear_fwd_grid(x.blk<void>(p.h1q, i), x.blk<void>(p.h1q8, i), M, x.widx(i, WB_QKV), x.act_qp(x.aidx(i, AB_N1)), x.bprm(i, B_QKVB), nullptr,
+                                         x.aidx(i, AB_QKV), &p1, true, lt))
                 return 1;
             if (x.linear_fwd_grid(x.blk<void>(p.h1q, i), x.blk<void>(p.h1q8, i), M, x.widx(i, WB_QKV), x.act_qp(x.aidx(i, AB_N1)), x.bprm(i, B_QKVB), nullptr,
                                   x.aidx(i, AB_QKV), &p2, false, lt))
@@ -457,8 +491,10 @@
             return 1;
         }
         if (parts & 4) {
-        x.ln_apply(xmid, x.blk<float>(p.mean2, i), x.blk<float>(p.rstd2, i), x.bprm(i, B_N2W), x.bprm(i, B_N2B), x.aidx(i, AB_N2), x.blk<void>(p.h2q, i),
-                   x.blk<void>(p.h2q8, i));
+        const bool ln2 = x.ln_in_strip(WB_FC1);
+        if (!ln2)
+            x.ln_apply(xmid, x.blk<float>(p.mean2, i), x.blk<float>(p.rstd2, i), x.bprm(i, B_N2W), x.bprm(i, B_N2B), x.aidx(i, AB_N2), x.blk<void>(p.h2q, i),
+                       x.blk<void>(p.h2q8, i));
         {
             NTPost p2{nullptr, x.act_qp(x.aidx(i, AB_FC1)), qa, qb, nullptr, x.blk<void>(p.G_hi, i), x.blk<void>(p.G_lo, i), 4,
                       x.blk<void>(p.Y1, i)};
@@ -468,8 +504,11 @@
             else if (F.f16_fc2) { p2.out16_hi = x.at<void>(p.G16_hi); p2.out16_lo = x.at<void>(p.G16_lo); p2.out16_scale = scal16 + 1; }
             const bool lt = x.late_in_strip(M, x.widx(i, WB_FC1), &p2);
             const NTPost p1{nullptr, nullptr, 0, 0, nullptr, nullptr, nullptr, 3, nullptr};
-            if (x.linear_fwd_grid(x.blk<void>(p.h2q, i), x.blk<void>(p.h2q8, i), M, x.widx(i, WB_FC1), x.act_qp(x.aidx(i, AB_N2)), x.bprm(i, B_FC1B), nullptr,
-                             x.aidx(i, AB_FC1), &p1, true, lt))
+            if (ln2) {
+                const Ctx::LnRows r{xmid, x.blk<float>(p.mean2, i), x.blk<float>(p.rstd2, i), x.bprm(i, B_N2W), x.bprm(i, B_N2B), x.aidx(i, AB_N2)};
+                if (x.linear_stats_ln(r, x.blk<void>(p.h2q8, i), M, x.widx(i, WB_FC1), x.bprm(i, B_FC1B), x.aidx(i, AB_FC1), lt)) return 1;
+            } else if (x.linear_fwd_grid(x.blk<void>(p.h2q, i), x.blk<void>(p.h2q8, i), M, x.widx(i, WB_FC1), x.act_qp(x.aidx(i, AB_N2)), x.bprm(i, B_FC1B), nullptr,
+                                         x.aidx(i, AB_FC1), &p1, true, lt))
                 return 1;
             if (x.linear_fwd_grid(x.blk<void>(p.h2q, i), x.blk<void>(p.h2q8, i), M, x.widx(i, WB_FC1), x.act_qp(x.aidx(i, AB_N2)), x.bprm(i, B_FC1B), nullptr,
                              x.aidx(i, AB_FC1), &p2, false, lt))
@@ -967,6 +1006,14 @@
     return run_backward(cfg, params, act_fq, weight_fq, dlogits, grads, workspace, stage_from, stage_to, flags, stream, "qatvit_student_backward_stages");
 }
 
+int32_t qatvit_student_ln_in_strip(const qatvit_cfg* cfg, int32_t flags) {
+    if (!cfg || check_cfg(*cfg)) return 0;
+    Plan p;
+    if (make_plan(*cfg, &p)) return 0;
+    const Dims d = dims_of(*cfg);
+    return (ln_in_strip_of(p, d, flags, WB_QKV) ? 1 : 0) | (ln_in_strip_of(p, d, flags, WB_FC1) ? 2 : 0);
+}
+
 int32_t qatvit_student_dy16_supported(const qatvit_cfg* cfg) {
     if (!cfg || check_cfg(*cfg)) return 0;
     Plan p;
diff --git a/qat-vit_amd/csrc/i8strip.hip b/qat-vit_amd/csrc/i8strip.hip
--- a/qat-vit_amd/csrc/i8strip.hip
+++ b/qat-vit_amd/csrc/i8strip.hip
@@ -35,6 +35,14 @@
     float* out16_scale;
     unsigned long long* dbg;
     QpLate late;
+    const float* ln_x;
+    const float* ln_mean;
+    const float* ln_rstd;
+    const float* ln_gamma;
+    const float* ln_beta;
+    int8_t* ln_out8;
+    int ln_qmin, ln_qmax;
+    QpLate ln_late;
 };
 
 __device__ inline int strip_off(int row, int chunk) {
@@ -49,8 +57,9 @@
 #define QV_STAMP() ((void)0)
 #endif
 
-template <int MODE, int NTL, int NWV = 8, bool R255 = false, int TM_ = 13, int KT_ = 6>
+template <int MODE, int NTL, int NWV = 8, bool R255 = false, int TM_ = 13, int KT_ = 6, bool LN = false>
 __global__ __launch_bounds__(NWV * 64, NWV / 4) void k_i8_strip(const I8StripArgs p) {
+    static_assert(!LN || MODE == 3, "the LayerNorm prologue exists in the statistics pass only");
     constexpr int TM = TM_, TNT = 24 / NWV, WC = 16 * TNT, BM = 16 * TM, BN = 384, KT = KT_, PF = 3, NT_ = NWV * 64;
     static_assert(TM <= 2 * NWV, "the strip's 1-KiB DMA pieces are dealt in two rounds");
     static_assert(NWV == 8 || NWV == 12, "8 waves x 48 columns or 12 waves x 32 columns");
@@ -80,7 +89,7 @@
 #endif
     QV_STAMP();
 
-    {
+    if constexpr (!LN) {
         const int64_t abytes = (int64_t)p.M * p.lda;
         const __amdgpu_buffer_rsrc_t rA = __builtin_amdgcn_make_buffer_rsrc(const_cast<int8_t*>(p.A), 0, abytes > 0xffffffffll ? 0xffffffffu : (uint32_t)abytes, 0x00020000);
         const int lR = lane >> 3, lL = (lane & 7) ^ lR;
@@ -109,13 +118,76 @@
     i32x4 bb[2][TNT];
     load_b(0, 0, bb[0]);
 
+    float* sQp = reinterpret_cast<float*>(sStage + (MODE == 3 ? 512 : NWV * WSTG));
+
+    constexpr int CPR = KT * 4, RG = NT_ / CPR, NIT = (BM + RG - 1) / RG, LU = 2, LNB = (NIT + LU - 1) / LU;
+    const int kc = tid % CPR, rg = tid / CPR;
+    float4 xv[LN ? 2 : 1][LN ? LU : 1][4], lg[4], lb[4];
+    float xmu[LN ? 2 : 1][LN ? LU : 1], xrs[LN ? 2 : 1][LN ? LU : 1];
+    auto ln_load = [&](int it, float4 (&v)[4], float& mu, float& rs) {
+        const int rl = rg + RG * it;
+        const bool ok = rg < RG && rl < BM && m0 + rl < p.M;
+        const int64_t row = ok ? m0 + rl : m0;
+        const float4* src = reinterpret_cast<const float4*>(p.ln_x + row * (KT * 64) + kc * 16);
+#pragma unroll
+        for (int c = 0; c < 4; ++c) v[c] = src[c];
+        mu = p.ln_mean[row];
+        rs = p.ln_rstd[row];
+    };
+    if constexpr (LN) {
+#pragma unroll
+        for (int u = 0; u < LU; ++u) ln_load(u, xv[0][u], xmu[0][u], xrs[0][u]);
+#pragma unroll
+        for (int c = 0; c < 4; ++c) {
+            lg[c] = reinterpret_cast<const float4*>(p.ln_gamma + kc * 16)[c];
+            lb[c] = reinterpret_cast<const float4*>(p.ln_beta + kc * 16)[c];
+        }
+        if (p.ln_late.stats) qp_late_compute(p.ln_late, sQp);
+        else if (tid == 0) { sQp[0] = p.aqp[0]; sQp[1] = p.aqp[1]; sQp[2] = p.aqp[2]; }
+        strip_lds_barrier();
+        QV_STAMP();
+    }
+    const float a_s = LN ? sQp[0] : *p.s1, a_inv = LN ? sQp[1] : 0.f, a_zp = LN ? sQp[2] : p.aqp[2];
+
     {
-        const float alpha = *p.s1 * (p.s2 ? *p.s2 : 1.0f);
-        const int zc = p.center - (int)p.aqp[2];
+        const float alpha = a_s * (p.s2 ? *p.s2 : 1.0f);
+        const int zc = p.center - (int)a_zp;
         for (int c = tid; c < NC; c += NT_) {
             sCorr[c] = zc * p.wsum[nbase + c];
             sCa[c] = alpha * (p.col_scale ? p.col_scale[nbase + c] : 1.0f);
             sCb[c] = p.bias ? p.bias[nbase + c] : 0.0f;
+        }
+    }
+    if constexpr (LN) {
+        const float fqmin = (float)p.ln_qmin, fqmax = (float)p.ln_qmax, sh = a_zp - (float)p.center;
+        auto ln_code = [&](float x, float mu, float rs, float g, float b) {
+            const float y = (x - mu) * rs * g + b;
+            const float qi = fminf(fmaxf(rintf(y * a_inv) + a_zp, fqmin), fqmax) - a_zp;
+            return (uint32_t)(uint8_t)(signed char)(qi + sh);
+        };
+        auto ln_put = [&](int it, const float4 (&v)[4], float mu, float rs) {
+            const int rl = rg + RG * it;
+            const bool in_strip = rg < RG && rl < BM, ok = in_strip && m0 + rl < p.M;
+            uint32_t w[4];
+#pragma unroll
+            for (int c = 0; c < 4; ++c)
+                w[c] = ln_code(v[c].x, mu, rs, lg[c].x, lb[c].x) | (ln_code(v[c].y, mu, rs, lg[c].y, lb[c].y) << 8) |
+                       (ln_code(v[c].z, mu, rs, lg[c].z, lb[c].z) << 16) | (ln_code(v[c].w, mu, rs, lg[c].w, lb[c].w) << 24);
+            const uint4 pk = ok ? make_uint4(w[0], w[1], w[2], w[3]) : make_uint4(0u, 0u, 0u, 0u);
+            if (in_strip) *reinterpret_cast<uint4*>(sA + (kc >> 2) * IMGA + strip_off(rl, kc & 3)) = pk;
+            if (ok) *reinterpret_cast<uint4*>(p.ln_out8 + (int64_t)(m0 + rl) * p.lda + kc * 16) = pk;
+        };
+#pragma unroll
+        for (int b = 0; b < LNB; ++b) {
+            if (b + 1 < LNB) {
+#pragma unroll
+                for (int u = 0; u < LU; ++u)
+                    if ((b + 1) * LU + u < NIT) ln_load((b + 1) * LU + u, xv[(b + 1) & 1][u], xmu[(b + 1) & 1][u], xrs[(b + 1) & 1][u]);
+            }
+            __builtin_amdgcn_sched_barrier(0);
+#pragma unroll
+            for (int u = 0; u < LU; ++u)
+                if (b * LU + u < NIT) ln_put(b * LU + u, xv[b & 1][u], xmu[b & 1][u], xrs[b & 1][u]);
         }
     }
     struct Consts { float4 ca, cb; };
@@ -124,7 +196,6 @@
         return Consts{*reinterpret_cast<const float4*>(sCa + c), *reinterpret_cast<const float4*>(sCb + c)};
     };
 
-    float* sQp = reinterpret_cast<float*>(sStage + (MODE == 3 ? 512 : NWV * WSTG));
     if constexpr (MODE != 3) {
         if (p.late.stats) qp_late_compute(p.late, sQp);
         else if (tid == 0) { sQp[0] = p.qp[0]; sQp[1] = p.qp[1]; sQp[2] = p.qp[2]; }
@@ -341,6 +412,20 @@
     else strip_launch_w<MODE, NTL, 12, TM, KT>(a, st);
 }
 
+template <int NTL, int TM = 13, int KT = 6>
+static void strip_launch_ln(const I8StripArgs& a0, hipStream_t st) {
+    I8StripArgs a = a0;
+#ifdef QV_STRIP_EXPERIMENTS
+    const char* d = getenv("QATVIT_STRIP_DBG");
+    a.dbg = d ? reinterpret_cast<unsigned long long*>(strtoull(d, nullptr, 0)) : nullptr;
+#endif
+    constexpr int kLds = KT * 16 * TM * 64 + 3 * NTL * 384 * 4 + 512 + 16;
+    static_assert(kLds <= 160 * 1024, "strip + constants exceed the LDS");
+    static bool once = ((void)hipFuncSetAttribute(reinterpret_cast<const void*>(k_i8_strip<3, NTL, 8, false, TM, KT, true>), hipFuncAttributeMaxDynamicSharedMemorySize, kLds), true);
+    (void)once;
+    k_i8_strip<3, NTL, 8, false, TM, KT, true><<<dim3(cdiv(a.M, 16 * TM), 1), 8 * 64, kLds, st>>>(a);
+}
+
 static int strip_ntl(int N, int K) {
     return K == 384 ? (N % (4 * 384) == 0 ? 4 : N % (3 * 384) == 0 ? 3 : 0) : (N == 6 * 384 ? 6 : N == 8 * 384 ? 8 : 0);
 }
@@ -357,6 +442,32 @@
     if (post->mode == 7) return post->code_hd == 64 && (N / 3) % 384 == 0 && post->code_T >= 1 && post->code_T < 1024;
     if (post->mode == 4) return !(post->out_hi || post->out_lo || post->code || post->out16_hi || post->out16_lo || !post->lut_out || !post->lutq_out || ldc % 128 != 0);
     return false;
+}
+
+bool i8_strip_ln_covers(const void* B8f, int M, int N, int K, int lda) {
+    NTPost p1{};
+    p1.mode = 3;
+    return knobs().ln_strip && lda >= K && i8_strip_covers(B8f, M, N, K, lda, N, &p1) && N == strip_ntl(N, K) * 384 && (int64_t)M * K < (1ll << 31);
+}
+bool launch_i8_strip_ln(const float* x, const float* mean, const float* rstd, const float* gamma, const float* beta, int ln_qmin, int ln_qmax, void* out8,
+                        const void* B8f, const int32_t* wsum, const float* a_qp, int center, int M, int N, int K, int lda, const float* s2,
+                        const float* col_scale, const float* bias, uint32_t* stats, int stat_slots, hipStream_t st, bool force, const QpLate* ln_late) {
+    if ((!(knobs().i8_strip && knobs().ln_strip) && !force) || !x || !mean || !rstd || !gamma || !beta || !out8 || !B8f || !wsum || !stats || (K != 384 && K != 768) ||
+        lda % 16 != 0 || lda < K || M < 1 || !strip_addressable(M, N, lda, N, 3) || (int64_t)M * K >= (1ll << 31))
+        return false;
+    const int ntl = strip_ntl(N, K);
+    if (!ntl || N != ntl * 384) return false;
+    if (!(ln_late && ln_late->stats) && !a_qp) return false;
+    I8StripArgs a{};
+    a.A = reinterpret_cast<const int8_t*>(out8); a.Bf = reinterpret_cast<const i32x4*>(B8f); a.M = M; a.N = N; a.lda = lda;
+    a.s1 = nullptr; a.s2 = s2; a.col_scale = col_scale; a.bias = bias; a.wsum = wsum; a.aqp = a_qp; a.center = center;
+    a.stats = stats; a.stat_slots = stat_slots < 1 ? 1 : stat_slots;
+    a.ln_x = x; a.ln_mean = mean; a.ln_rstd = rstd; a.ln_gamma = gamma; a.ln_beta = beta; a.ln_out8 = reinterpret_cast<int8_t*>(out8);
+    a.ln_qmin = ln_qmin; a.ln_qmax = ln_qmax;
+    if (ln_late) a.ln_late = *ln_late;
+    if (K == 768) { if (ntl == 8) strip_launch_ln<8, 7, 12>(a, st); else strip_launch_ln<6, 7, 12>(a, st); }
+    else if (ntl == 4) strip_launch_ln<4>(a, st); else strip_launch_ln<3>(a, st);
+    return true;
 }
 
 bool launch_i8_strip(const void* A8, const void* B8f, const int32_t* wsum, const float* a_qp, int center, int M, int N, int K, int lda, int ldc,
diff --git a/qat-vit_amd/csrc/qv_common.h b/qat-vit_amd/csrc/qv_common.h
--- a/qat-vit_amd/csrc/qv_common.h
+++ b/qat-vit_amd/csrc/qv_common.h
@@ -25,6 +25,7 @@
     bool attn_bwd_fused;
     bool f16_strip;
     bool i8_strip;
+    bool ln_strip;
 };
 const Knobs& knobs();
 
diff --git a/qat-vit_amd/csrc/qv_kernels.h b/qat-vit_amd/csrc/qv_kernels.h
--- a/qat-vit_amd/csrc/qv_kernels.h
+++ b/qat-vit_amd/csrc/qv_kernels.h
@@ -89,6 +89,11 @@
                      const float* s1, const float* s2, const float* col_scale, const float* bias, uint32_t* stats, int stat_slots, hipStream_t st,
                      const NTPost* post, bool force = false, const QpLate* late = nullptr);
 bool i8_strip_covers(const void* B8f, int M, int N, int K, int lda, int ldc, const NTPost* post);
+bool launch_i8_strip_ln(const float* x, const float* mean, const float* rstd, const float* gamma, const float* beta, int ln_qmin, int ln_qmax, void* out8,
+                        const void* B8f, const int32_t* wsum, const float* a_qp, int center, int M, int N, int K, int lda, const float* s2,
+                        const float* col_scale, const float* bias, uint32_t* stats, int stat_slots, hipStream_t st, bool force = false,
+                        const QpLate* ln_late = nullptr);
+bool i8_strip_ln_covers(const void* B8f, int M, int N, int K, int lda);
 __host__ __device__ inline int64_t w8f_offset(int n, int k, int K) {
     const int cg = n / 48, cr = n % 48, j = cr / 16, r = cr % 16, kt = k / 64, kk = k % 64;
     return ((((int64_t)cg * (K / 64) + kt) * 3 + j) * 64 + (kk / 16) * 16 + r) * 16 + (kk % 16);
diff --git a/qat-vit_amd/engine.py b/qat-vit_amd/engine.py
--- a/qat-vit_amd/engine.py
+++ b/qat-vit_amd/engine.py
@@ -252,6 +252,7 @@
         self.dy16 = dy16_default() and bool(self.lib.qatvit_student_dy16_supported(ctypes.byref(self.cfg)))
         self._dy16_calibrated = False
         self._fwd_x16 = False
+        self.ln_in_strip = 0
         self.dy16_fallbacks = 0
         self._mirror = self._mirror_np = None
         self._mirror_on = os.environ.get("QATVIT_DY16_MIRROR", "1") != "0"
@@ -423,6 +424,7 @@
         logits = torch.empty(c.batch, c.num_classes, dtype=torch.float32, device=self.device)
         self.generation += 1
         self._fwd_x16 = self.dy16 and self._dy16_calibrated and self.sync_state
+        self.ln_in_strip = int(self.lib.qatvit_student_ln_in_strip(ctypes.byref(c), FWD_X16 if self._fwd_x16 else 0))
         native.check(self.lib.qatvit_student_forward_stages(ctypes.byref(c), self._ptr_params, self._act_structs, self._w_structs, images.data_ptr(),
                                                             logits.data_ptr(), self.workspace.data_ptr(), 0, c.depth + 1, FWD_X16 if self._fwd_x16 else 0,
                                                             native.stream_ptr()), "qatvit_student_forward")
diff --git a/qat-vit_amd/native.py b/qat-vit_amd/native.py
--- a/qat-vit_amd/native.py
+++ b/qat-vit_amd/native.py
@@ -28,6 +28,8 @@
     "qatvit_gemm_nt_i8_minmax": (c_int, [c_void_p] * 4 + [c_int32] * 6 + [c_void_p] * 6),
     "qatvit_w8_fragment_order": (c_int, [c_void_p, c_void_p, c_int32, c_int32, c_void_p]),
     "qatvit_i8_strip": (c_int, [c_int32] + [c_void_p] * 4 + [c_int32] * 5 + [c_void_p] * 6 + [c_int32, c_int32, c_void_p, c_void_p, c_int32] + [c_void_p] * 4),
+    "qatvit_ln_apply_quant8": (c_int, [c_void_p] * 6 + [c_int32, c_int32, c_void_p, c_int32, c_int64, c_int32, c_void_p]),
+    "qatvit_i8_strip_ln": (c_int, [c_void_p] * 5 + [c_int32, c_int32] + [c_void_p] * 4 + [c_int32] * 5 + [c_void_p] * 5),
     "qatvit_gemm_nt_codes": (c_int, [c_void_p] * 4 + [c_int32] * 6 + [c_void_p] * 6),
     "qatvit_gemm_nt_i8": (c_int, [c_void_p] * 4 + [c_int32, c_void_p] + [c_int32] * 6 + [c_void_p] * 6),
     "qatvit_gemm_tn_scratch_bytes": (c_int64, []),
@@ -54,6 +56,7 @@
     "qatvit_student_backward_stages": (c_int, [c_void_p] * 7 + [c_int32, c_int32, c_int32, c_void_p]),
     "qatvit_student_tensor_offset": (c_int64, [c_void_p, c_char_p, c_int32]),
     "qatvit_student_dy16_supported": (c_int32, [c_void_p]),
+    "qatvit_student_ln_in_strip": (c_int32, [c_void_p, c_int32]),
     "qatvit_student_dy16_to_pair": (c_int, [c_void_p, c_void_p, c_void_p]),
     "qatvit_student_dy16_set_mirror": (c_int, [c_void_p, c_void_p, c_void_p, c_void_p]),
     "qatvit_teacher_workspace_bytes": (c_int64, [c_void_p]),
```
